# JuliaQuantumControl/GRAPE.jl

Hardware: AMD Instinct MI355X
Metric: GRAPE gradient evals/sec (N=64, 1000 steps, 128 traj) (higher is better)
Workload: dtype f64

## Files before the change

grape.jl_amd/api.py:

```python
from __future__ import annotations

import ctypes as C
import os
import subprocess
import sys

import numpy as np

_HERE = os.path.dirname(os.path.abspath(__file__))
_CSRC = os.path.join(_HERE, "csrc")
_LIBNAME = "libgrape_hip.so"

J_T_SM, J_T_SS, J_T_RE = 0, 1, 2
GRAD_GRADGEN, GRAD_TAYLOR = 0, 1
PROP_EXP, PROP_SERIES = 0, 1
ABI_VERSION = 7

STATUS = {0: "GRAPE_OK", -1: "GRAPE_ERR_INVALID", -2: "GRAPE_ERR_HIP", -3: "GRAPE_ERR_CHI_NORM",
          -4: "GRAPE_ERR_SINGULAR", -5: "GRAPE_ERR_TAYLOR", -6: "GRAPE_ERR_NO_CONTROLS", -7: "GRAPE_ERR_AGAIN",
          -8: "GRAPE_ERR_HOST"}

EXPORTS = ["grape_create", "grape_destroy", "grape_eval", "grape_forward", "grape_backward",
           "grape_forward_device", "grape_backward_device", "grape_check", "grape_get_propagator",
           "grape_get_tau_grads", "grape_get_storage", "grape_get_timings", "grape_reset_timings", "grape_get_work", "grape_get_cert_table", "grape_get_seg_table",
           "grape_last_error", "grape_abi_version", "grape_set_fused_sweeps", "grape_get_sums", "grape_backward_xi",
           "grape_get_final_states", "grape_backward_chi",
           "grape_get_time_gradient", "grape_set_tlist", "grape_eval_batch", "grape_get_batch_info", "grape_create_open",
           "grape_hvp", "grape_get_hvp_info", "grape_open_time_gradient", "grape_open_hvp", "grape_get_open_hvp_info",
           "grape_open_eval_batch", "grape_get_open_batch_info", "grape_open_set_running_cost", "grape_open_backward_xi",
           "grape_hvp_forward", "grape_hvp_backward", "grape_hvp_backward_chi",
           "grape_open_hvp_forward", "grape_open_hvp_backward", "grape_open_hvp_backward_chi",
           "grape_expect", "grape_get_expect_info"]


class GrapeHipError(RuntimeError):
    def __init__(self, code, msg):
        super().__init__(f"{STATUS.get(code, code)}: {msg}")
        self.code = code


class _Problem(C.Structure):
    _fields_ = [("abi_version", C.c_int32), ("N", C.c_int32), ("L", C.c_int32), ("K", C.c_int32),
                ("K_total", C.c_int32), ("N_T", C.c_int32), ("functional", C.c_int32),
                ("gradient_method", C.c_int32), ("hc_per_traj", C.c_int32), ("device", C.c_int32),
                ("tlist", C.c_void_p), ("H0", C.c_void_p), ("Hc", C.c_void_p), ("shape", C.c_void_p),
                ("psi0", C.c_void_p), ("target", C.c_void_p), ("weights", C.c_void_p),
                ("chi_min_norm", C.c_double), ("taylor_max_order", C.c_int32),
                ("taylor_tolerance", C.c_double),
                ("Dpen", C.c_void_p), ("dpen_per_traj", C.c_int32), ("lambda_b", C.c_double),
                ("prop_method", C.c_int32), ("prop_tolerance", C.c_double),
                ("ndev", C.c_int32), ("devices", C.c_void_p), ("taylor_no_check", C.c_int32)]


class _Lindblad(C.Structure):
    _fields_ = [("J", C.c_int32), ("cops_per_traj", C.c_int32), ("cops", C.c_void_p)]


def library_path() -> str:
    return os.path.join(_CSRC, _LIBNAME)


def build_asm(verbose: bool = False, workdir: str | None = None) -> str:
    asm_dir = os.path.join(_CSRC, "asm")
    work = workdir or asm_dir
    kernels = (("gen_t16.py", "expm_t16_asm"), ("gen_t16p.py", "expm_t16p_asm"), ("gen_t16p.py", "expm_t16p4_asm"), ("gen_t18g.py", "expm_t18g_asm"), ("gen_t18gp.py", "expm_t18gp_asm"), ("gen_d3.py", "deriv3_asm"), ("gen_d3s.py", "deriv3s_asm"), ("gen_d3s.py", "deriv3g_asm"),
               ("gen_lg.py", "lg_gemm_asm"), ("gen_d4.py", "deriv4_asm_128"), ("gen_d4.py", "deriv4_asm_256"))
    co_path, emb_s, emb_o = os.path.join(work, "grape_asm.co"), os.path.join(work, "asm_embed.S"), os.path.join(work, "asm_embed.o")
    llvm = "/opt/rocm/lib/llvm/bin"
    cmds, objs = [], []
    for gen_py, name in kernels:
        s_path, o_path = os.path.join(work, name + ".s"), os.path.join(work, name + ".o")
        gen = subprocess.run([sys.executable, os.path.join(asm_dir, gen_py), s_path], capture_output=True, text=True)
        if verbose or gen.returncode:
            print(gen.stdout, gen.stderr)
        if gen.returncode:
            raise RuntimeError(gen_py + " failed")
        cmds.append([os.path.join(llvm, "clang"), "-x", "assembler", "-target", "amdgcn-amd-amdhsa", "-mcpu=gfx950", "-c", s_path, "-o", o_path])
        objs.append(o_path)
    cmds.append([os.path.join(llvm, "ld.lld"), "-shared"] + objs + ["-o", co_path])
    with open(emb_s, "w") as f:
        f.write('\t.section .rodata\n\t.globl grape_asm_co_start\n\t.globl grape_asm_co_end\n\t.p2align 12\n'
                'grape_asm_co_start:\n\t.incbin "grape_asm.co"\ngrape_asm_co_end:\n\t.byte 0\n'
                '\t.section .note.GNU-stack,"",@progbits\n')
    cmds.append(["gcc", "-c", "-fPIC", "asm_embed.S", "-o", "asm_embed.o"])
    for c in cmds:
        res = subprocess.run(c, capture_output=True, text=True, cwd=work)
        if verbose or res.returncode:
            print(" ".join(c), res.stdout, res.stderr)
        if res.returncode:
            raise RuntimeError("assembling the gfx950 kernels failed")
    return emb_o


def _sources():
    srcs = [os.path.join(_CSRC, f) for f in ("grape_hip.hip", "grape_t18.hip", "grape_kernels.hip.h", "grape_large.hip.h",
                                             "grape_series.hip.h", "grape_cheby.hip.h", "grape_t18.hip.h", "grape_t18_coeffs.h",
                                             "grape_deriv3.hip.h", "grape_timegrad.hip.h", "grape_batch.hip.h", "grape_lindblad.hip.h", "grape_lindblad_tg.hip.h", "grape_hvp.hip.h", "grape_hvp_split.hip.h", "grape_lindblad_hvp.hip.h", "grape_lindblad_hvp_split.hip.h", "grape_lindblad_batch.hip.h", "grape_lindblad_rc.hip.h", "grape_devmem.h", "grape_cert.hip.h", "grape_expect.hip.h", "grape_econ_coeffs.h", os.path.join("asm", "gen_t16.py"), os.path.join("asm", "gen_t16p.py"), os.path.join("asm", "gen_t18g.py"), os.path.join("asm", "gen_t18gp.py"), os.path.join("asm", "gen_d3.py"), os.path.join("asm", "gen_d3s.py"), os.path.join("asm", "gen_lg.py"), os.path.join("asm", "gen_d4.py"), os.path.join("asm", "gcn.py"))]
    return srcs, os.path.join(_HERE, "..", "include", "grape_hip.h")


def _up_to_date(out: str) -> bool:
    srcs, hdr = _sources()
    return os.path.exists(out) and all(os.path.getmtime(out) >= os.path.getmtime(s) for s in srcs + [hdr])


def build_library(force: bool = False, verbose: bool = False, extra_flags=(), out: str | None = None) -> str:
    import fcntl
    import shutil
    import tempfile
    out = out or library_path()
    if not force and _up_to_date(out):
        return out
    srcs, _ = _sources()
    with open(os.path.join(_CSRC, ".build.lock"), "w") as lockf:
        fcntl.flock(lockf, fcntl.LOCK_EX)
        if not force and _up_to_date(out):
            return out
        work = tempfile.mkdtemp(prefix="_build_", dir=_CSRC)
        procs = []
        try:
            base = ["hipcc", "--offload-arch=gfx950", "-O3", "-std=c++17", "-fPIC", "-Wno-unused-value"] + list(extra_flags)
            objs = [os.path.join(work, "grape_hip.o"), os.path.join(work, "grape_t18.o")]
            cmds = [base + ["-cuid=grapehip0", "-c", srcs[0], "-o", objs[0]],
                    base + ["-cuid=grapehip1", "-mllvm", "-amdgpu-mfma-vgpr-form", "-c", srcs[1], "-o", objs[1]]]
            procs = [subprocess.Popen(c, stdout=subprocess.PIPE, stderr=subprocess.STDOUT, text=True) for c in cmds]
            objs.append(build_asm(verbose, workdir=work))
            outs = [p.communicate()[0] for p in procs]
            if verbose or any(p.returncode for p in procs):
                print("\n".join(outs))
            if any(p.returncode for p in procs):
                raise RuntimeError("hipcc failed building " + out)
            tmp_so = os.path.join(work, _LIBNAME)
            res = subprocess.run(["hipcc", "--offload-arch=gfx950", "-shared", "-fPIC"] + objs + ["-o", tmp_so], capture_output=True, text=True)
            if verbose or res.returncode:
                print(res.stdout, res.stderr)
            if res.returncode:
                raise RuntimeError("hipcc failed linking " + out)
            asm_dir = os.path.join(_CSRC, "asm")
            for f in os.listdir(work):
                if f.endswith(".s") or f.endswith(".co"):
                    os.replace(os.path.join(work, f), os.path.join(asm_dir, f))
            os.replace(tmp_so, out)
        finally:
            for p in procs:
                if p.poll() is None:
                    p.kill()
                    p.communicate()
            shutil.rmtree(work, ignore_errors=True)
    return out

# ... 311 lines not shown
        nv = 1 if d.ndim == 2 else d.shape[0]
        out = np.empty((nv, self.L * self.N_T))
        self._chk(self._lib.grape_hvp_backward_chi(self._h, nv, chi.ctypes.data, d.ctypes.data, out.ctypes.data))
        return out[0] if d.ndim == 2 else out

    def set_tlist(self, tlist):
        t = np.ascontiguousarray(tlist, dtype=np.float64)
        if t.shape != (self.N_T + 1,):
            raise ValueError(f"tlist must have N_T + 1 = {self.N_T + 1} points, got {t.shape}")
        self._chk(self._lib.grape_set_tlist(self._h, t.ctypes.data))
        self._tlist = t

    def forward_device(self, d_pulsevals_ptr, d_out_ptr, stream=0):
        self._chk(self._lib.grape_forward_device(self._h, d_pulsevals_ptr, d_out_ptr, stream))

    def backward_device(self, d_f_ptr, d_G_ptr, stream=0):
        self._chk(self._lib.grape_backward_device(self._h, d_f_ptr, d_G_ptr, stream))

    def set_fused_sweeps(self, on=True):
        return bool(self._lib.grape_set_fused_sweeps(self._h, int(bool(on))))

    def check(self, stream=0):
        self._chk(self._lib.grape_check(self._h, stream))

    def propagator(self, k, n):
        out = np.empty((self.N, self.N), dtype=np.complex128)
        self._chk(self._lib.grape_get_propagator(self._h, k, n, out.ctypes.data))
        return out.T.copy()

    def tau_grads(self):
        out = np.empty((self.K, self.L, self.N_T), dtype=np.complex128)
        self._chk(self._lib.grape_get_tau_grads(self._h, out.ctypes.data))
        return out

    def storage(self, which=0):
        out = np.empty((self.K, self.N_T + 1, self.N), dtype=np.complex128)
        self._chk(self._lib.grape_get_storage(self._h, which, out.ctypes.data))
        return out

    def timings(self):
        ms = np.full(8, -1.0)
        self._lib.grape_get_timings(self._h, ms.ctypes.data, 8)
        out = dict(zip(["expm", "forward", "backward", "deriv", "reduce", "total"], ms[:6].tolist()))
        if ms[6] >= 0.0:
            out["host_enqueue"] = float(ms[6])
        if ms[7] >= 0.0:
            out["gradient_allreduce_us"] = float(ms[7]) * 1e3
        return out

    def reset_timings(self):
        self._chk(self._lib.grape_reset_timings(self._h))

    def work(self):
        w = np.zeros(21)
        self._lib.grape_get_work(self._h, w.ctypes.data, 21)
        return dict(cells=w[0], squarings=w[1], flop_expm=w[2], flop_deriv=w[3], deriv_orders=w[4],
                    pivoted_cells=w[5], expm_cells=w[6], series_terms=w[7], series_steps=w[8],
                    t18_mfma_flop=w[9], t18_squarings=w[10], t18_cells=w[11], matrix_free_fallback=w[12], t16_cells=w[13],
                    asm_kernel=w[14], asm_deriv_kernel=w[15], asm_blocked_products=w[16],
                    walk_steps=w[17], scan_block=w[18], t16_certified=w[19], seg_certified=w[20])

    def cert_table(self):
        dims = np.zeros(3, np.int32)
        self._chk(self._lib.grape_get_cert_table(self._h, dims.ctypes.data, None, None))
        KC, n8, n6 = (int(x) for x in dims)
        coef, exps = np.zeros((KC, n8 + n6)), np.zeros(n8 + n6, np.int32)
        if n8 + n6:
            self._chk(self._lib.grape_get_cert_table(self._h, dims.ctypes.data, coef.ctypes.data, exps.ctypes.data))
        ex = np.stack([(exps >> (4 * l)) & 15 for l in range(self.L)], axis=1) if n8 + n6 else np.zeros((0, self.L), np.int32)
        return coef[:, :n8], coef[:, n8:], ex

    def seg_table(self):
        dims = np.zeros(4, np.int32)
        self._chk(self._lib.grape_get_seg_table(self._h, dims.ctypes.data, None, None))
        KC, n4, n8, n12 = (int(x) for x in dims)
        nt = n4 + n8 + n12
        coef, exps = np.zeros((KC, nt)), np.zeros(nt, np.int32)
        if nt:
            self._chk(self._lib.grape_get_seg_table(self._h, dims.ctypes.data, coef.ctypes.data, exps.ctypes.data))
        ex = np.stack([(exps >> (4 * l)) & 15 for l in range(self.L)], axis=1) if nt else np.zeros((0, self.L), np.int32)
        return coef[:, :n4], coef[:, n4:n4 + n8], coef[:, n4 + n8:], ex


def liouvillian(H, cops=()):
    H = np.asarray(H, dtype=np.complex128)
    d = H.shape[0]
    if H.shape != (d, d):
        raise ValueError(f"H must be [d, d], got {H.shape}")
    eye = np.eye(d)
    heff = H.copy()
    for A in cops:
        A = np.asarray(A, dtype=np.complex128)
        heff = heff - 0.5j * (A.conj().T @ A)
    out = np.kron(eye, heff) - np.kron(heff.conj(), eye)
    for A in cops:
        A = np.asarray(A, dtype=np.complex128)
        out = out + 1j * np.kron(A.conj(), A)
    return out


class GrapeHipOpen(GrapeHip):

    def __init__(self, H0, Hc, cops, tlist, rho0, target, weights=None, functional=J_T_SM, shape=None, K_total=None,
                 device=0, chi_min_norm=0.0, prop_tolerance=0.0):
        self._lib = load_library()
        H0 = np.asarray(H0)
        if H0.ndim != 3 or H0.shape[1] != H0.shape[2]:
            raise ValueError(f"H0 must be [K, d, d], got {H0.shape}")
        K, N = H0.shape[0], H0.shape[1]
        Hc = np.asarray(Hc)
        per_traj = Hc.ndim == 4
        if Hc.ndim not in (3, 4) or Hc.shape[-2:] != (N, N) or (per_traj and Hc.shape[0] != K):
            raise ValueError(f"Hc must be [L, d, d] or [K, L, d, d] with d = {N}, K = {K}, got {Hc.shape}")
# ... 194 lines not shown
```

grape.jl_amd/csrc/asm/gen_t16.py:

```python
import os
import re
import struct
import sys

sys.path.insert(0, os.path.dirname(os.path.abspath(__file__)))
from gcn import Prog, Reg, V, A, S, VCC, EXEC, Neg, Abs, kernel_text
from gcn import HZ_MFMA_TO_VALU as gcn_wait_valu, HZ_MFMA_TO_MEM as gcn_wait_mem

NT = 4
NP = 64
LDB = (3 * NP + 2) * 8
PLB = NP * 8
TROW = 16 * LDB
PLANES = NP * LDB
E1 = PLANES
EXH = 256 * 8 + 128
EXW = 2 * EXH
E2 = E1 + 4 * EXW
RED = E2 + 4 * EXW
XS0 = RED + 16 * 8
XS1 = XS0 + 1024
LDS_BYTES = XS1 + 1024
KERNARG = 136
SQ_MASK = 0xFF
CERT_BIT = 0x100

HERE = os.path.dirname(os.path.abspath(__file__))


def t16_coeffs():
    txt = open(os.path.join(HERE, "..", "grape_t18_coeffs.h")).read()
    c = {}
    for m in re.finditer(r"#define\s+T16_(C\d+|THETA)\s+([-+0-9.eE]+)", txt):
        c[m.group(1)] = float(m.group(2))
    assert len(c) == 17, c
    return c


def dbits(x):
    b = struct.unpack("<Q", struct.pack("<d", x))[0]
    return b & 0xFFFFFFFF, b >> 32


def pcol(j):
    return (j >> 1) + 8 * (j & 1)


def qrow(i):
    return 4 * (i & 3) + (i >> 2)


TILES = [(0, 0), (0, 1), (0, 2), (0, 3), (1, 1), (1, 2), (1, 3), (2, 2), (2, 3), (3, 3)]


class Pool:

# ... 391 lines not shown
            self.ssel(self.s_tmp[0], 16 * j0 * LDB + 16 * i0 * 8, 16 * j1 * LDB + 16 * i1 * 8)
            self.ssel(self.s_tmp[1], 16 * i0 * LDB + 16 * j0 * 8, 16 * i1 * LDB + 16 * j1 * 8)
            p.valu("v_add_u32", va, self.s_tmp[0], self.v_CP)
            p.valu("v_add_u32", vm, self.s_tmp[1], self.v_CM)
            cstep = (8 if self.PCOL_PERM else 1) * LDB
            for e in range(2):
                p.ds_write(64, va, ar.d(e), e * cstep)
                p.ds_write(64, va, ai.d(e), e * cstep + PLB)
                p.ds_write(64, va, sm.d(e), e * cstep + 2 * PLB)
            d0, d1 = i0 == j0, i1 == j1
            if not (d0 and d1):
                nar, ms = sr, si
                p.valu("v_mul_f64", nar.d(0), ar.d(0), -1.0)
                p.valu("v_mul_f64", nar.d(1), ar.d(1), -1.0)
                p.valu("v_add_f64", ms.d(0), ai.d(0), Neg(ar.d(0)))
                p.valu("v_add_f64", ms.d(1), ai.d(1), Neg(ar.d(1)))
                if d0 or d1:
                    p.salu("s_mov_b64", self.s_save, EXEC)
                    p.s_cmp("s_cmp_lt_u32", self.s_wave, 2)
                    lab = f"L_mirror_{u}_{len(p.ins)}"
                    p.s_branch("s_cbranch_scc1" if d0 else "s_cbranch_scc0", lab)
                for e in range(2):
                    p.ds_write(64, vm, nar.d(e), 32 * e)
                    p.ds_write(64, vm, ai.d(e), 32 * e + PLB)
                    p.ds_write(64, vm, ms.d(e), 32 * e + 2 * PLB)
                if d0 or d1:
                    p.label(lab)
            if fill:
                fill(u)
        for t in (ta, tb, tc):
            self.vp.free(t)

    def product(self, Q, B, half_last=False, init=None, hook=None, bload=None, fused=None):
        p = self.p
        NS = len(Q)
        started = set(init or ())

        def nslots(sk):
            return NS - 1 if (half_last and 2 * sk >= NT) else NS

        def rd(pl, so, sk, r):
            p.tag = "fragment"
            p.ds_read(64, self.aop[pl][so], self.v_AA[so][sk], self.KSTEP * r * LDB + pl * PLB)
            p.tag = ""

        def mma(so, pl, a, b):
            acc = Q[so][pl]
            c = acc if (so, pl) in started else 0
            started.add((so, pl))
            p.mfma(acc, a, b, c)

        sk0 = 0
        if fused:
            assert NS == 4 and not half_last and not bload

            def rdk(pl, so, r):
                p.tag = "fragment"
                p.ds_read(64, self.aop[pl][r], self.v_AA[so][0], self.KSTEP * r * LDB + pl * PLB)
                p.tag = ""

            fused["valu"](0)
            for st in fused["stores"](0):
                st()
            if fused.get("after_first"):
                fused["after_first"]()
            for r in range(4):
                for pl in range(3):
                    rdk(pl, 0, r)
            for so in range(4):
                gaps = [[] for _ in range(12)]
                if so < 3:
                    fused["valu"](so + 1)
                    pend = list(fused["stores"](so + 1))
                    for q, st in enumerate(pend):
                        gaps[4 * (q // 2) + (q % 2)].append(st)
                    last = {pl: (4 * pl + 1 if pend else 0) for pl in range(3)}
                    for r in range(4):
                        for pl in range(3):
                            gaps[max(last[pl], 3 * r + pl)].append(lambda pl=pl, r=r: rdk(pl, so + 1, r))
                j = 0
                for r in range(4):
                    for pl in range(3):
                        mma(so, pl, self.aop[pl][r], B[pl][0].d(r))
                        for f in gaps[j]:
                            f()
                        j += 1
            if fused.get("post"):
                fused["post"]()
            p.s_barrier()
            sk0 = 1
        for pl in range(3):
            for so in range(nslots(sk0)):
                rd(pl, so, sk0, 0)
            if bload:
                bload(pl, sk0, 0)
        for sk in range(sk0, 4):
            for r in range(4):
                ns = nslots(sk)
                more = not (sk == 3 and r == 3)
                nsk, nr = (sk, r + 1) if r < 3 else (sk + 1, 0)
                nsn = nslots(nsk) if more else 0
                for pl in range(3):
                    for so in range(ns):
                        mma(so, pl, self.aop[pl][so], B[pl][sk].d(r))
                        if hook and pl == 0 and so == 0:
                            hook(sk, r)
                    for so in range(nsn):
                        rd(pl, so, nsk, nr)
                    if bload and more:
                        bload(pl, nsk, nr)

    def plane_stores(self, sl, xr, xi, xs):
        if self.opts.get("nostore"):
            return []
        a = self.v_SA[sl]

        def st(h, pl, x):
            self.p.tag = "strip store"
            self.p.ds_write(128, a, x.sub(4 * h, 4), 16 * h + pl * PLB)
            self.p.tag = ""
        return [lambda h=h, pl=pl, x=x: st(h, pl, x) for pl, x in enumerate((xr, xi, xs)) for h in range(2)]

    def interleave(self, streams):
        streams = [list(s) for s in streams]
        if self.opts.get("serial"):
            for s in streams:
                for f in s:
                    f()
            return
        while any(streams):
            for s in streams:
                if s:
                    s.pop(0)()

    def acc_read(self, dst, src):
        if self.opts.get("noacc"):
            self.p.valu("v_mov_b32", dst.sub(0), dst.sub(0))
            self.p.valu("v_mov_b32", dst.sub(1), dst.sub(1))
            return
        self.p.valu("v_accvgpr_read_b32", dst.sub(0), src.sub(0))
        self.p.valu("v_accvgpr_read_b32", dst.sub(1), src.sub(1))

    def acc_write(self, dst, src):
        if self.opts.get("noacc"):
            self.p.valu("v_mov_b32", src.sub(0), src.sub(0))
            self.p.valu("v_mov_b32", src.sub(1), src.sub(1))
            return
        self.p.valu("v_accvgpr_write_b32", dst.sub(0), src.sub(0))
        self.p.valu("v_accvgpr_write_b32", dst.sub(1), src.sub(1))

    def wave_reduce(self, x, tmp, op):
        p = self.p
        for ctrl, rm in (("quad_perm:[1,0,3,2]", 0xF), ("quad_perm:[2,3,0,1]", 0xF), ("row_half_mirror", 0xF), ("row_mirror", 0xF),
                         ("row_bcast:15", 0xA), ("row_bcast:31", 0xC)):
            if rm != 0xF:
                p.valu("v_mov_b32", tmp.sub(0), 0)
                p.valu("v_mov_b32", tmp.sub(1), 0 if op == "v_add_f64" else 0xFFF00000)
            p.dpp_mov(tmp.sub(0), x.sub(0), ctrl, row_mask=rm)
            p.dpp_mov(tmp.sub(1), x.sub(1), ctrl, row_mask=rm)
            p.valu(op, x, x, tmp)

    def cell(self):
        p, c = self.p, self.s_c
        vp, ap = self.vp, self.ap
        Qt = [[V(8 * self.QT[3 * so + j], 8) for j in range(3)] for so in range(4)]
        for t in self.QT:
            vp.free_tiles.remove(t)
        Uprev = V(8 * self.UT, 64)
        for t in range(self.UT, self.UT + 8):
            vp.free_tiles.remove(t)

        self.stamp(0)
        self.As_re, self.As_im, self.As_sm = ap.alloc(4), ap.alloc(4), ap.alloc(4)
        As = (self.As_re, self.As_im, self.As_sm)

        def hook_store(sk, r):
            p.salu("s_mov_b64", self.s_save, EXEC)
            p.s_cmp("s_cmp_lg_u32", self.s_pm, 0)
            p.salu("s_cselect_b64", EXEC, -1, 0)
            p.global_store(4, self.v_UO[r], Uprev.sub(16 * sk + 4 * r, 4), self.s_ub[sk], nt=self.nt_u)
            p.salu("s_mov_b64", EXEC, self.s_save)

        def bload_A(pl, sk, r):
            if r % 2 == 0:
                p.tag = "strip load"
                p.ds_read(128, As[pl].sub(8 * sk + 2 * r, 4), self.v_SA[sk], 8 * r + pl * PLB)
                p.tag = ""

        B_As = [[S_.sub(8 * sl, 8) for sl in range(4)] for S_ in As]
        self.product(Qt[:3], B_As, half_last=True, hook=hook_store, bload=bload_A)
        ap.free(self.As_sm)
        vp.free(Uprev)
        self.stamp(1)
        As_re, As_im = self.As_re, self.As_im

        def A_(sl, r):
            return As_re.sub(8 * sl, 8).d(r), As_im.sub(8 * sl, 8).d(r)

        def in_place_y(sl_list):
            streams = []
            for sl in sl_list:
                for r in range(4):
                    p1, p2, p3 = (Qt[sl][j].d(r) for j in range(3))
                    streams.append([lambda p3=p3, p1=p1: p.valu("v_add_f64", p3, p3, Neg(p1)),
                                    lambda p1=p1, p2=p2: p.valu("v_add_f64", p1, p1, Neg(p2)),
                                    lambda p3=p3, p2=p2: p.valu("v_add_f64", p3, p3, Neg(p2))])
            for g in range(0, len(streams), 4):
                self.interleave(streams[g:g + 4])

        A2re, A2im, A2sm = [vp.alloc() for _ in range(4)], [vp.alloc() for _ in range(4)], [vp.alloc() for _ in range(4)]
        streams = []
        for sl in range(3):
            for r in range(4):
                p1, p2, p3 = (Qt[sl][j].d(r) for j in range(3))
                re_, im_ = A2re[sl].d(r), A2im[sl].d(r)
                streams.append([lambda re_=re_, p1=p1, p2=p2: p.valu("v_add_f64", re_, p1, Neg(p2)),
                                lambda im_=im_, p3=p3, p1=p1: p.valu("v_add_f64", im_, p3, Neg(p1)),
                                lambda im_=im_, p2=p2: p.valu("v_add_f64", im_, im_, Neg(p2))])
        for g in range(0, len(streams), 4):
            self.interleave(streams[g:g + 4])
        for r in range(4):
            p.ds_write(64, self.v_EW2, A2re[2].d(r), 128 * r)
            p.ds_write(64, self.v_EW2, A2im[2].d(r), EXH + 128 * r)
            p.ds_write(64, self.v_EW1, A2re[1].d(r), 128 * r)
            p.ds_write(64, self.v_EW1, A2im[1].d(r), EXH + 128 * r)
        p.s_waitcnt(lgkm=0)
        p.s_barrier()
        self.advance()
        self.cell_bases_issue(self.s_nkc, self.s_nn, self.s_ncell)
        txr, txi = vp.alloc(), vp.alloc()
        for h in range(2):
            p.ds_read(128, txr.sub(4 * h, 4), self.v_ER, 16 * h)
            p.ds_read(128, txi.sub(4 * h, 4), self.v_ER, EXH + 16 * h)
            p.ds_read(128, A2re[3].sub(4 * h, 4), self.v_ER, (E2 - E1) + 16 * h)
            p.ds_read(128, A2im[3].sub(4 * h, 4), self.v_ER, (E2 - E1) + EXH + 16 * h)
        self.stamp(2)
        tt = [vp.alloc(), vp.alloc()]

        def valu2(sl):
            if sl == 2:
                for r in range(4):
                    p.valu("v_add_f64", A2re[2].d(r), A2re[2].d(r), txr.d(r))
                    p.valu("v_add_f64", A2im[2].d(r), A2im[2].d(r), Neg(txi.d(r)))
                for r in range(4):
                    p.valu("v_mul_f64", A2im[3].d(r), A2im[3].d(r), -1.0)
                vp.free(txr)
                vp.free(txi)
            streams = []
            for r in range(4):
                xr, xi, xs = tt[0].d(r), tt[1].d(r), Qt[sl][1].d(r)
                a2r, a2i = A2re[sl].d(r), A2im[sl].d(r)
                ar_, ai_ = A_(sl, r)
                streams.append([lambda xr=xr, ar_=ar_: self.acc_read(xr, ar_),
                                lambda xi=xi, ai_=ai_: self.acc_read(xi, ai_),
                                lambda xr=xr: p.valu("v_mul_f64", xr, c[2], xr),
                                lambda xi=xi: p.valu("v_mul_f64", xi, c[2], xi),
                                lambda xr=xr, a2r=a2r: p.valu("v_fma_f64", xr, c[1], a2r, xr),
                                lambda xi=xi, a2i=a2i: p.valu("v_fma_f64", xi, c[1], a2i, xi),
                                lambda xs=xs, xr=xr, xi=xi: p.valu("v_add_f64", xs, xr, xi),
                                lambda r=r, a2r=a2r, a2i=a2i: p.valu("v_add_f64", A2sm[sl].d(r), a2r, a2i)])
            self.interleave(streams)

        self.product(Qt, [A2re, A2im, A2sm], fused={"valu": valu2, "stores": lambda sl: self.plane_stores(sl, tt[0], tt[1], Qt[sl][1])})
        for t in tt + A2sm:
            vp.free(t)
        self.cell_bases_finish(self.s_nkc)
        self.stamp(3)
        uid = len(p.ins)
        L_cert, L_cert2, L_ones, L_vdone = f"L_cert_{uid}", f"L_cert2_{uid}", f"L_ones_{uid}", f"L_vdone_{uid}"
        p.salu("s_and_b32", self.s_tmp[0], self.s_scur, CERT_BIT)
        p.s_branch("s_cbranch_scc1", L_cert)
        facc, gacc, cacc = vp.alloc(), vp.alloc(), vp.alloc()
        for acc in (facc, gacc, cacc):
            for j in range(8):
                p.valu("v_mov_b32", acc.sub(j), 0)
        streams = []
        for sl in range(4):
            for r in range(4):
                k = len(streams) % 4
                p1, p2, p3 = (Qt[sl][j].d(r) for j in range(3))
                a2r, a2i = A2re[sl].d(r), A2im[sl].d(r)
                f, g_, cs = facc.d(k), gacc.d(k), cacc.d(k)
                streams.append([
                    lambda p3=p3, p1=p1: p.valu("v_add_f64", p3, p3, Neg(p1)),
                    lambda p1=p1, p2=p2: p.valu("v_add_f64", p1, p1, Neg(p2)),
                    lambda p3=p3, p2=p2: p.valu("v_add_f64", p3, p3, Neg(p2)),
                    lambda cs=cs, a2r=a2r: p.valu("v_add_f64", cs, cs, Abs(a2r)),
                    lambda f=f, p1=p1: p.valu("v_fma_f64", f, p1, p1, f),
                    lambda g_=g_, a2r=a2r, p1=p1: p.valu("v_fma_f64", g_, a2r, p1, g_),
                    lambda cs=cs, a2i=a2i: p.valu("v_add_f64", cs, cs, Abs(a2i)),
                    lambda f=f, p3=p3: p.valu("v_fma_f64", f, p3, p3, f),
                    lambda g_=g_, a2i=a2i, p3=p3: p.valu("v_fma_f64", g_, a2i, p3, g_)])
        for g in range(0, 16, 4):
            self.interleave(streams[g:g + 4])
        f, g_, cs = facc.d(0), gacc.d(0), cacc.d(0)
        for k in range(1, 4):
            p.valu("v_add_f64", f, f, facc.d(k))
            p.valu("v_add_f64", g_, g_, gacc.d(k))
            p.valu("v_add_f64", cs, cs, cacc.d(k))
        ones, ct = cacc.d(1), vp.alloc(1)
        lo, hi = dbits(1.0)
        p.valu("v_mov_b32", ones.sub(0), lo)
        p.valu("v_mov_b32", ones.sub(1), hi)
        p.label(L_ones)
        p.mfma(ct, ones, cs, 0)
        p.salu("s_and_b32", self.s_tmp[0], self.s_scur, CERT_BIT)
        p.s_branch("s_cbranch_scc1", L_cert2)
        tmp = cacc.d(2)
        self.wave_reduce(f, tmp, "v_add_f64")
        self.wave_reduce(g_, tmp, "v_add_f64")
        mx = cacc.d(3)
        p.valu("v_mov_b64", mx, ct.d(0))
        for ctrl in ("quad_perm:[1,0,3,2]", "quad_perm:[2,3,0,1]", "row_half_mirror", "row_mirror"):
            p.dpp_mov(tmp.sub(0), mx.sub(0), ctrl)
            p.dpp_mov(tmp.sub(1), mx.sub(1), ctrl)
            p.valu("v_max_f64", mx, mx, tmp)
# ... 15 lines not shown
        vtf, vtg, vt2, vz = vp.alloc(), vp.alloc(), vp.alloc(), vp.alloc()
        p.valu("v_mov_b32", vz.sub(0), RED)
        for h in range(2):
            p.ds_read(128, vtf.sub(4 * h, 4), vz.sub(0), 16 * h)
            p.ds_read(128, vtg.sub(4 * h, 4), vz.sub(0), 32 + 16 * h)
            p.ds_read(128, vt2.sub(4 * h, 4), vz.sub(0), 64 + 16 * h)
        F, G, N2 = vtf.d(0), vtg.d(0), vt2.d(0)
        for k in range(1, 4):
            p.valu("v_add_f64", F, F, vtf.d(k))
            p.valu("v_add_f64", G, G, vtg.d(k))
            p.valu("v_max_f64", N2, N2, vt2.d(k))
        th = self.c["THETA"]
        c1, c2 = self.c["C1"], self.c["C2"]
        k0, k1, k2 = S(58, 2), S(60, 2), S(62, 2)
        self.smov64(k0, -1.0 / c1)
        p.valu("v_mul_f64", G, G, k0)
        self.smov64(k1, c2 * c2)
        p.valu("v_fma_f64", F, Neg(G), k1, F)
        self.smov64(k2, (1.0 + 1e-9) / (c1 * c1))
        p.valu("v_mul_f64", F, F, k2)
        self.smov64(k0, th ** 8)
        p.v_cmp("v_cmp_le_f64", S(58, 2), F, k0)
        p.v_cmp("v_cmp_ge_f64", S(60, 2), G, 0)
        p.salu("s_and_b64", S(58, 2), S(58, 2), S(60, 2))
        self.smov64(k2, th * th / (1.0 + 1e-9))
        p.v_cmp("v_cmp_le_f64", S(60, 2), N2, k2)
        p.salu("s_or_b64", S(58, 2), S(58, 2), S(60, 2))
        p.salu("s_and_b32", self.s_prop, self.s_prop, 1)
        p.s_cmp("s_cmp_eq_u64", S(58, 2), 0)
        p.salu("s_cselect_b32", self.s_tmp[4], 2, 0)
        p.salu("s_or_b32", self.s_prop, self.s_prop, self.s_tmp[4])
        p.valu("v_cndmask_b32", vz.sub(1), 1, 0, S(58, 2))
        p.salu("s_lshl_b32", self.s_tmp[2], self.s_cell, 2)
        p.valu("v_mov_b32", vz.sub(2), self.s_tmp[2])
        p.salu("s_mov_b64", self.s_save, EXEC)
        p.s_cmp("s_cmp_eq_u32", self.s_wave, 0)
        p.salu("s_cselect_b32", self.s_tmp[4], 1, 0)
        p.salu("s_mov_b32", self.s_tmp[5], 0)
        p.salu("s_mov_b64", EXEC, S(self.s_tmp[4].idx, 2))
        p.global_store(1, vz.sub(2), vz.sub(1), self.s_verdict)
        p.salu("s_mov_b64", EXEC, self.s_save)
        for t in (vtf, vtg, vt2, vz):
            vp.free(t)
        p.s_branch("s_branch", L_vdone)
        p.label(L_cert)
        p.nop(gcn_wait_valu)
        in_place_y(range(4))
        p.s_branch("s_branch", L_ones)
        p.label(L_cert2)
        p.nop(gcn_wait_mem)
        p.s_waitcnt(lgkm=0)
        p.s_barrier()
        p.salu("s_and_b32", self.s_prop, self.s_prop, 1)
        p.label(L_vdone)
        self.A2p_re, self.A2p_im = ap.alloc(4), ap.alloc(4)
        Bre, Bim, Bsm = [None] * 4, [None] * 4, [None] * 4
        tt = [vp.alloc(), vp.alloc()]

        def valu3(sl):
            Bre[sl], Bim[sl], Bsm[sl] = vp.alloc(), vp.alloc(), vp.alloc()
            streams = []
            for r in range(4):
                y0r, xs, y0i = (Qt[sl][j].d(r) for j in range(3))
                a2r, a2i = A2re[sl].d(r), A2im[sl].d(r)
                xr, xi = tt[0].d(r), tt[1].d(r)
                br, bi, bs = Bre[sl].d(r), Bim[sl].d(r), Bsm[sl].d(r)
                ar_, ai_ = A_(sl, r)
                pr, pi_ = self.A2p_re.sub(8 * sl, 8).d(r), self.A2p_im.sub(8 * sl, 8).d(r)
                streams.append([
                    lambda xr=xr, ar_=ar_: self.acc_read(xr, ar_),
                    lambda xi=xi, ai_=ai_: self.acc_read(xi, ai_),
                    lambda pr=pr, a2r=a2r: self.acc_write(pr, a2r),
                    lambda pi_=pi_, a2i=a2i: self.acc_write(pi_, a2i),
                    lambda br=br, a2r=a2r, y0r=y0r: p.valu("v_fma_f64", br, c[5], a2r, y0r),
                    lambda bi=bi, a2i=a2i, y0i=y0i: p.valu("v_fma_f64", bi, c[5], a2i, y0i),
                    lambda xr=xr: p.valu("v_mul_f64", xr, c[4], xr),
                    lambda xi=xi: p.valu("v_mul_f64", xi, c[4], xi),
                    lambda xr=xr, a2r=a2r: p.valu("v_fma_f64", xr, c[3], a2r, xr),
                    lambda xi=xi, a2i=a2i: p.valu("v_fma_f64", xi, c[3], a2i, xi),
                    lambda xr=xr, y0r=y0r: p.valu("v_add_f64", xr, xr, y0r),
                    lambda xi=xi, y0i=y0i: p.valu("v_add_f64", xi, xi, y0i),
                    lambda bs=bs, br=br, bi=bi: p.valu("v_add_f64", bs, br, bi),
                    lambda xs=xs, xr=xr, xi=xi: p.valu("v_add_f64", xs, xr, xi),
                    lambda y0r=y0r: p.valu("v_mul_f64", y0r, c[6], y0r),
                    lambda y0i=y0i: p.valu("v_mul_f64", y0i, c[6], y0i),
                    lambda y0r=y0r, a2r=a2r: p.valu("v_fma_f64", y0r, c[7], a2r, y0r),
                    lambda y0i=y0i, a2i=a2i: p.valu("v_fma_f64", y0i, c[7], a2i, y0i),
                    lambda y0i=y0i, y0r=y0r: p.valu("v_add_f64", y0i, y0i, y0r)])
            self.interleave(streams)
            vp.free(A2re[sl])
            vp.free(A2im[sl])

        init13 = {(so, j) for so in range(4) for j in (0, 2)}
        self.stamp(5)
        self.product(Qt, [Bre, Bim, Bsm], init=init13,
                     fused={"valu": valu3, "stores": lambda sl: self.plane_stores(sl, tt[0], tt[1], Qt[sl][1])})
        for t in tt:
            vp.free(t)
        self.stamp(6)
        in_place_y(range(4))
        p.s_barrier()
        self.stamp(7)
        self.stamp(8)
        k16 = S(58, 2)
        self.smov64(k16, self.c["C16"])
        tt = [vp.alloc() for _ in range(4)]

        def valu4(sl):
            streams = []
            for r in range(4):
                y1r, xi, y1i = (Qt[sl][j].d(r) for j in range(3))
                br, bi, xr = Bre[sl].d(r), Bim[sl].d(r), Bsm[sl].d(r)
                asr, asi, a2r, a2i = tt[0].d(r), tt[1].d(r), tt[2].d(r), tt[3].d(r)
                ar_, ai_ = A_(sl, r)
                pr, pi_ = self.A2p_re.sub(8 * sl, 8).d(r), self.A2p_im.sub(8 * sl, 8).d(r)
                st = [
                    lambda asr=asr, ar_=ar_: self.acc_read(asr, ar_),
                    lambda asi=asi, ai_=ai_: self.acc_read(asi, ai_),
                    lambda a2r=a2r, pr=pr: self.acc_read(a2r, pr),
                    lambda a2i=a2i, pi_=pi_: self.acc_read(a2i, pi_),
                    lambda br=br, a2r=a2r: p.valu("v_fma_f64", br, c[5], Neg(a2r), br),
                    lambda bi=bi, a2i=a2i: p.valu("v_fma_f64", bi, c[5], Neg(a2i), bi),
                    lambda xr=xr, a2r=a2r, y1r=y1r: p.valu("v_fma_f64", xr, c[8], a2r, y1r),
                    lambda xi=xi, a2i=a2i, y1i=y1i: p.valu("v_fma_f64", xi, c[8], a2i, y1i),
                    lambda xr=xr, asr=asr: p.valu("v_fma_f64", xr, c[9], asr, xr),
                    lambda xi=xi, asi=asi: p.valu("v_fma_f64", xi, c[9], asi, xi),
                    lambda a2r=a2r: p.valu("v_mul_f64", a2r, c[14], a2r),
                    lambda a2i=a2i: p.valu("v_mul_f64", a2i, c[14], a2i),
                    lambda a2r=a2r, asr=asr: p.valu("v_fma_f64", a2r, c[15], asr, a2r),
                    lambda a2i=a2i, asi=asi: p.valu("v_fma_f64", a2i, c[15], asi, a2i),
                    lambda a2r=a2r, br=br: p.valu("v_fma_f64", a2r, c[13], br, a2r),
                    lambda a2i=a2i, bi=bi: p.valu("v_fma_f64", a2i, c[13], bi, a2i),
                    lambda a2r=a2r, y1r=y1r: p.valu("v_fma_f64", a2r, c[12], y1r, a2r),
                    lambda a2i=a2i, y1i=y1i: p.valu("v_fma_f64", a2i, c[12], y1i, a2i),
                    lambda br=br, y1r=y1r: p.valu("v_fma_f64", br, c[10], br, y1r),
                    lambda bi=bi, y1i=y1i: p.valu("v_fma_f64", bi, c[10], bi, y1i),
                    lambda br=br, asr=asr: p.valu("v_fma_f64", br, c[11], asr, br),
                    lambda bi=bi, asi=asi: p.valu("v_fma_f64", bi, c[11], asi, bi),
                    lambda asr=asr, xr=xr, xi=xi: p.valu("v_add_f64", asr, xr, xi),
                ]
                if sl == 0:
                    def diag(a2r=a2r, r=r):
                        p.salu("s_mov_b64", self.s_save, EXEC)
                        p.salu("s_mov_b64", EXEC, self.s_dmask[r])
                        p.valu("v_add_f64", a2r, a2r, k16)
                        p.salu("s_mov_b64", EXEC, self.s_save)
                    st.append(diag)
                st += [
                    lambda y1r=y1r, a2r=a2r: p.valu("v_mov_b64", y1r, a2r),
                    lambda y1i=y1i, a2r=a2r, a2i=a2i: p.valu("v_add_f64", y1i, a2r, a2i),
                ]
                streams.append(st)
            self.interleave(streams)

        def bsm(sl_list):
            for sl in sl_list:
                for r in range(4):
                    p.valu("v_add_f64", Bsm[sl].d(r), Bre[sl].d(r), Bim[sl].d(r))
# ... 376 lines not shown
```

grape.jl_amd/csrc/grape_hip.hip:

```cpp
#include "../../include/grape_hip.h"
#include "grape_kernels.hip.h"
#include "grape_t18_coeffs.h"
#include "grape_econ_coeffs.h"
#include "grape_large.hip.h"
#include "grape_series.hip.h"
#include "grape_cheby.hip.h"
#include "grape_timegrad.hip.h"
#include "grape_lindblad.hip.h"
#include "grape_lindblad_tg.hip.h"
#include "grape_hvp.hip.h"
#include "grape_hvp_split.hip.h"
#include "grape_lindblad_hvp.hip.h"
#include "grape_lindblad_hvp_split.hip.h"
#include "grape_lindblad_batch.hip.h"
#include "grape_lindblad_rc.hip.h"
#include "grape_devmem.h"
#include "grape_cert.hip.h"
#include "grape_expect.hip.h"

#include <rccl/rccl.h>
#include <dlfcn.h>
#include <mutex>

#include <algorithm>
// ... 42 lines not shown
struct OpenCtx;

struct grape_handle {
    grape_problem p{};
    int N = 0, NP = 0, NT = 0, L = 0, K = 0, K_total = 0, N_T = 0;
    int device = 0;
    hipStream_t stream = nullptr;
    double *d_H0f = nullptr, *d_Hcf = nullptr, *d_H0t = nullptr, *d_Hct = nullptr;
    double *d_H0p = nullptr, *d_Hcp = nullptr, *d_vecs = nullptr;
    double *d_H0q = nullptr, *d_Hcq = nullptr, *d_park2 = nullptr;
    double *d_H0q3 = nullptr, *d_Hcq3 = nullptr, *d_H0p3 = nullptr, *d_Hcp3 = nullptr;
    int deriv4_blocks = 0;
    double *d_park3 = nullptr;
    int deriv3_blocks = 0, deriv3_wpt = 0;
    bool deriv3_h0g = false;
    bool deriv3_general = false;
    int deriv2 = 0, deriv2_maxm = 0;
    bool deriv_stream = false;
    bool deriv_stream_never = false;
    int deriv_blocks = 0;
    bool large = false;
    int chunk = 0;
    double *d_lg[9] = {nullptr, nullptr, nullptr, nullptr, nullptr, nullptr, nullptr, nullptr, nullptr};
    double *d_dinv = nullptr;
    int *d_scell = nullptr;
    double *d_colpart = nullptr;
    bool lg_form2 = false;
    double *d_normpart = nullptr;
    double *d_dts = nullptr, *d_shape = nullptr, *d_weights = nullptr;
    double2 *d_psi0 = nullptr, *d_target = nullptr;
    double *d_eps = nullptr;
    double2 *d_U = nullptr, *d_fw = nullptr, *d_bw = nullptr, *d_tg = nullptr;
    double *d_ret = nullptr;
    double *d_out = nullptr;
    double *d_f = nullptr, *d_G = nullptr, *d_rho = nullptr;
    int *d_flags = nullptr;
    int *d_cellflag = nullptr;
    int KC = 0;
    bool herm = false;
    bool herm_ctrl = false;
    bool t18 = false;
    bool t18_small = true;
    bool t16 = true;
    double *d_gram = nullptr;
    int *d_celllist = nullptr;
    double *d_cert = nullptr;
    int *d_cert_exp = nullptr;
    int cert_n8 = 0, cert_n6 = 0;
    double *d_seg = nullptr;
    double *d_seg8 = nullptr;
    int *d_seg_exp = nullptr;
    int seg_n8 = 0, seg_n4 = 0, seg_n12 = 0, seg8_stride = 0, seg_exp_off = 0;
    int *d_segplan = nullptr;
    bool asm16 = false;
    bool asm16p = false;
    double *d_dte = nullptr;
    bool asm18gp = false;
    bool asm18g = false;
    int *d_wgtab = nullptr, *d_prog = nullptr, *d_splan = nullptr;
    double2 *d_xinit = nullptr;
    int asm_blocks = 0;
    int last_walk_fuse = 0;
    bool asm_sq = true;
    int asm_walk = 0;
    bool foreign_stream = false;
    bool credit_pending = false;
    std::vector<double> bal;
    std::vector<double> bal_stage_chi, bal_stage_xi;
    double *d_Sf = nullptr;
    bool expm_persist = true;
    int expm_lds_pad_kb = 0;
    bool test_hooks = false;
    bool lg_asm = true;
    bool deriv3_asm = true;
    bool taylor_check = true;
    bool no_target = false;
    std::vector<int> cls;
    int *d_cls = nullptr, *d_rep = nullptr;
    int coop_S = 0;
    int *d_xcc_sw = nullptr;
    int coop_rpw = 0, coop_nw = 0;
    double2 *d_Dt = nullptr, *d_xi = nullptr;
    double *d_wq = nullptr, *d_gb = nullptr;
    bool have_gb = false;
    const double2 *xi_user = nullptr;
    double lambda_user = 0.0;
    unsigned long long *d_stats = nullptr;
    double *h_pin = nullptr;
    double *h_get = nullptr;
    DeviceBufs mem;
    size_t h_pin_doubles = 0;
    Phase ph[kRing][kPhases]{};
    long n_fwd = 0, n_bwd = 0;
    std::string err;
    bool have_forward = false, in_eval = false;
    double chi_min_norm = 1e-100, taylor_tol = 1e-16;
    int taylor_max_order = 100;
    bool fuse = false;
    bool fuse_on = true;
    bool want_bw = true;
    bool bw_done = false;
    bool bw_unit = false;
    bool z_valid = false;
    double *d_inv_tnorm = nullptr, *d_ones = nullptr;
    double2 *d_z = nullptr;
    bool scan16 = false;
// ... 136 lines not shown
}
hipError_t stream_fill(void *p, int byte_value, size_t bytes, hipStream_t s) {
    hipStreamCaptureStatus st = hipStreamCaptureStatusNone;
    if (bytes % 4 != 0 || ((size_t)p & 3) != 0 || hipStreamIsCapturing(s, &st) != hipSuccess || st != hipStreamCaptureStatusActive)
        return hipMemsetAsync(p, byte_value, bytes, s);
    const size_t n = bytes / 4;
    if (n == 0) return hipSuccess;
    const unsigned v = 0x01010101u * (unsigned)(byte_value & 0xFF);
    hipLaunchKernelGGL(fill_words_kernel, dim3((unsigned)std::min<size_t>((n + 255) / 256, 1024)), dim3(256), 0, s, (unsigned *)p, v, n);
    return hipGetLastError();
}

size_t expm_lds_bytes(int NT) {
    const int total = NT == 1 ? ExpmLds<1>::TOTAL : NT == 2 ? ExpmLds<2>::TOTAL : NT == 3 ? ExpmLds<3>::TOTAL : ExpmLds<4>::TOTAL;
    return sizeof(double) * (size_t)total;
}

template <int NT>
hipError_t launch_expm(const ExpmArgs &a, bool herm, hipStream_t s, int persistent_blocks = 0, int lds_pad_kb = 0) {
    static LdsLimit lim_fast, lim_piv, lim_herm, lim_pers, lim_persh;
    const size_t lds = expm_lds_bytes(NT) + (size_t)lds_pad_kb * 1024;
    int dev = 0;
    hipGetDevice(&dev);
    {
        hipError_t e = lim_fast.ensure((const void *)expm_pade_kernel<NT, false>, dev, lds);
        if (e == hipSuccess) e = lim_piv.ensure((const void *)expm_pade_kernel<NT, true>, dev, lds);
        if (e == hipSuccess && NT >= 3) e = lim_herm.ensure((const void *)expm_pade_kernel<NT, false, NT >= 3>, dev, lds);
        if (e != hipSuccess) return e;
    }
    hipError_t e = stream_fill(a.cellflag, 0, (size_t)a.K * a.N_T * sizeof(int), s);
    if (e != hipSuccess) return e;
    if (NT == 4 && persistent_blocks > 0) {
        hipError_t ep = lim_pers.ensure((const void *)expm_persistent_kernel<NT, false>, dev, lds);
        if (ep == hipSuccess) ep = lim_persh.ensure((const void *)expm_persistent_kernel<NT, NT == 4>, dev, lds);
        if (ep != hipSuccess) return ep;
        if (herm) hipLaunchKernelGGL((expm_persistent_kernel<NT, NT == 4>), dim3(persistent_blocks), dim3(NT * 64), lds, s, a);
        else hipLaunchKernelGGL((expm_persistent_kernel<NT, false>), dim3(persistent_blocks), dim3(NT * 64), lds, s, a);
    } else
    if (herm && NT >= 3)
        hipLaunchKernelGGL((expm_pade_kernel<NT, false, NT >= 3>), dim3(a.K * a.N_T), dim3(NT * 64), lds, s, a);
    else
        hipLaunchKernelGGL((expm_pade_kernel<NT, false>), dim3(a.K * a.N_T), dim3(NT * 64), lds, s, a);
    hipLaunchKernelGGL((expm_pade_kernel<NT, true>), dim3(std::min(a.K * a.N_T, 1024)), dim3(NT * 64), lds, s, a);
    return hipGetLastError();
}

extern "C" int grape_t18_launch(int NT, int herm, int t16, const void *args, size_t args_size, void *stream, int blocks);
extern "C" const double *grape_econ_pairs(void);
extern "C" int grape_t16p_asm_launch(const void *args, size_t args_size, int *verdict, void *stream, int blocks,
                                     const void *const *walk, int fuse, int K, const double *dte);
extern "C" int grape_t18g_asm_launch(const void *args, size_t args_size, int *verdict, void *stream, int blocks,
                                     const void *const *walk, int fuse, int K, const double *dte);
extern "C" int grape_t16_asm_launch(const void *args, size_t args_size, int *verdict, void *stream, int blocks,
                                    const void *const *walk, int fuse, int K);
extern "C" int grape_t18_batch_launch(int herm, const void *args, size_t args_size, const void *strides, size_t strides_size,
                                      int sets, void *stream, int blocks);
extern "C" void grape_t16_walks(int KC, int N_T, int nblk, int *tab);
extern "C" int grape_t16_credit_launch(const void *args, size_t args_size, void *stream);
static bool deriv3_fits(int NT, int L, bool h0_general = false) {
    const size_t tile = (size_t)2 * 16 * 17 * sizeof(double), mat = (size_t)(NT * (NT + 1) / 2) * tile;
    if (h0_general) return NT >= 3 && NT <= 4 && L >= 1 && L <= 2 && (size_t)NT * NT * tile + (size_t)L * mat <= 160 * 1024;
    return L >= 1 && L <= 8 && (size_t)(1 + L) * mat <= 160 * 1024;
}
extern "C" int grape_deriv3_launch(int NT, const void *d2args, size_t d2size, const double *H0f, const double *Hcf, int wpt,
                                   int skip_if_flagged, int h0_general, int use_asm, void *stream, int blocks);
extern "C" int grape_lg_asm_launch(const void *k, size_t size, unsigned blocks, void *stream);
extern "C" int grape_deriv4_launch(int NP, const void *d2args, size_t d2size, const double *H0q3, const double *Hcq3, const double *H0p3,
                                   const double *Hcp3, void *stream, int blocks);
#ifdef GRAPE_DIAG
extern "C" void grape_t18_set_stamps(unsigned long long *d_stamps, void *stream);
#endif

template <int CPL>
hipError_t launch_coop(const SweepArgs &a, bool backward, int S, int rpw, int nw, hipStream_t s) {
    hipError_t e;
    if (a.xcc) {
        e = hipMemsetAsync(a.xcc, 0xFF, (size_t)a.K * 32 * sizeof(int), s);
        if (e != hipSuccess) return e;
    }
    e = hipMemsetAsync((void *)a.store, 0xFF, (size_t)a.K * (a.N_T + 1) * 64 * CPL * sizeof(double2), s);
    if (e != hipSuccess) return e;
    const dim3 grid(8 * ((a.K + 7) / 8) * S), block(64 * nw);
#define COOP_CASE(NW_, RPW_)                                                                                          \
    if (nw == NW_ && rpw == RPW_) {                                                                                   \
        if (backward) hipLaunchKernelGGL((sweep_coop_kernel<CPL, RPW_, NW_, true>), grid, block, 0, s, a, S);         \
        else hipLaunchKernelGGL((sweep_coop_kernel<CPL, RPW_, NW_, false>), grid, block, 0, s, a, S);                 \
        return hipGetLastError();                                                                                     \
    }
    COOP_CASE(4, 1) COOP_CASE(8, 1) COOP_CASE(16, 1) COOP_CASE(16, 2) COOP_CASE(16, 4)
#undef COOP_CASE
    return hipErrorInvalidValue;
}

static bool g_sweep_wg32 = false;
template <int NP>
hipError_t launch_sweep(const SweepArgs &a, bool backward, hipStream_t s);
template <int NP>
hipError_t launch_sweep_pair(const SweepArgs &af, const SweepArgs &ab, hipStream_t s);

template <int NT>
hipError_t launch_scan_block(const ScanArgs &sa, hipStream_t s) {
    static LdsLimit lim;
    constexpr int NP = 16 * NT;
    const size_t lds = (size_t)2 * 2 * NP * (NP + 2) * sizeof(double);
    int dev = 0;
    hipGetDevice(&dev);
    hipError_t e = lim.ensure((const void *)scan_block_kernel<NT>, dev, lds);
// ... 2372 lines not shown
                const double t = std::ceil((double)h->KC * NBq / slots) * Bk * t1 + (NBq + Bk) * t2;
                if (t < best_t) { best_t = t; best = Bk; }
            }
            if (const char *envb = getenv("GRAPE_SCAN16_BK")) best = std::max(2, atoi(envb));
            h->scan_Bk = std::min(best, N_T);
            h->scan_NB = (N_T + h->scan_Bk - 1) / h->scan_Bk;
            CCHK(h->mem.alloc(&h->d_scanF, (size_t)h->KC * h->scan_NB * NP * NP));
            CCHK(h->mem.alloc(&h->d_scan_fw, (size_t)K * (h->scan_NB + 1) * NP));
            CCHK(h->mem.alloc(&h->d_scan_bw, (size_t)K * (h->scan_NB + 1) * NP));
            h->scan16 = true;
        }
    }
    CCHK(h->mem.alloc(&h->d_tg, (size_t)K * L * N_T));
    CCHK(h->mem.alloc(&h->d_ret, (size_t)2 * K + 8 + (size_t)L * N_T + 4 + (size_t)GRAPE_STAT_SHARDS * GRAPE_STAT_SLOTS));
    h->d_out = h->d_ret;
    h->d_G = h->d_ret + (size_t)2 * K + 8;
    h->d_flags = (int *)(h->d_G + (size_t)L * N_T);
    h->d_stats = (unsigned long long *)(h->d_G + (size_t)L * N_T + 4);
    CCHK(h->mem.alloc(&h->d_f, 2)); CCHK(h->mem.alloc(&h->d_rho, (size_t)K));
    CCHK(h->mem.alloc(&h->d_cellflag, (size_t)K * N_T));
    bool sf_per_cell_ok = false;
    const char *envp16 = getenv("GRAPE_EXPM_ASM16P");
    const bool p_direct = p->hc_per_traj && (h->herm ? L <= 4 : L <= 2) && !(envp16 && atoi(envp16) == 0);
    if (p->hc_per_traj && !p_direct && h->t18 && !h->large && !h->series && h->NT == 4) {
        size_t free_b = 0, total_b = 0;
        CCHK(hipMemGetInfo(&free_b, &total_b));
        const char *envs = getenv("GRAPE_SF_PER_CELL");
        sf_per_cell_ok = !(envs && atoi(envs) == 0) && 2.0 * (double)h->KC * N_T * NP * NP * 16.0 + 8e9 < (double)free_b;
    }
    const bool sf_shape_ok = !p->hc_per_traj || p_direct || sf_per_cell_ok;
    h->asm16 = h->asm16 && h->t16 && h->t18 && h->herm && !h->large && !h->series && h->NT == 4 && sf_shape_ok && (long)K * N_T < (1L << 28);
    h->asm18g = h->asm18g && h->t18 && !h->herm && !h->large && !h->series && h->NT == 4 && sf_shape_ok && (long)K * N_T < (1L << 28);
    h->asm16p = h->asm16 && p_direct;
    h->asm18gp = h->asm18g && p_direct;
    {
        const char *enve = getenv("GRAPE_DERIV_ECON");
        const bool lg_ok = h->large && h->t18 && h->herm && !h->series;
        const bool t16c_ok = h->t16 && h->t18 && h->herm && !h->large && !h->series && (h->NT >= 3 || (h->NT == 2 && h->t18_small));
        h->deriv_econ = (h->asm16 || lg_ok || t16c_ok) && p->gradient_method == GRAPE_GRAD_GRADGEN && h->taylor_tol >= 1e-16 && h->d_batchflag &&
                        !(enve && atoi(enve) == 0);
        if (h->deriv_econ) h->d_econ_pairs = grape_econ_pairs();
        if (h->deriv_econ && !h->d_econ_pairs) h->deriv_econ = false;
        if (h->deriv_econ && lg_ok) {
            CCHK(h->mem.alloc(&h->d_celldeg, (size_t)h->KC * N_T));
            CCHK(hipMemset(h->d_celldeg, 0, (size_t)h->KC * N_T * sizeof(int)));
        }
    }
    if (h->asm16p || h->asm18gp) CCHK(h->mem.alloc(&h->d_dte, (size_t)(L <= 2 ? 4 : 8) * N_T));
    if (h->t18 && !h->large && !h->series && ((L > 2 && !p->hc_per_traj) || (h->asm16 && !h->asm16p) || (h->asm18g && !h->asm18gp)) && (h->NT >= 3 || h->t18_small))
        CCHK(h->mem.alloc(&h->d_Sf, (size_t)(p->hc_per_traj ? (size_t)h->KC * N_T : (size_t)N_T) * 2 * NP * NP));
    if (h->asm16 || h->asm18g) {
        const long ncell = (long)h->KC * N_T;
        h->asm_blocks = (int)std::max<long>(1, std::min<long>(h->num_cus, ncell));
        std::vector<int> tab((size_t)4 * h->asm_blocks);
        grape_t16_walks(h->KC, N_T, h->asm_blocks, tab.data());
        CCHK(h->mem.alloc(&h->d_wgtab, tab.size()));
        CCHK(h->mem.alloc(&h->d_splan, (size_t)ncell));
        CCHK(hipMemset(h->d_splan, 0, (size_t)ncell * sizeof(int)));
        CCHK(hipMemcpy(h->d_wgtab, tab.data(), tab.size() * sizeof(int), hipMemcpyHostToDevice));
        const char *envw = getenv("GRAPE_EXPM_WALK"), *envq = getenv("GRAPE_EXPM_SQ");
        h->asm_sq = !(envq && atoi(envq) == 0);
        h->asm_walk = h->KC == K ? (envw ? atoi(envw) & 3 : 3) : 0;
        if (h->scan16) h->asm_walk = 0;
        if (h->asm_walk) {
            std::vector<double> xi((size_t)2 * K * 64 * 2, 0.0);
            for (int k = 0; k < K; ++k) {
                double n2 = 0.0;
                for (int i = 0; i < 2 * N; ++i) n2 += p->target[(size_t)k * 2 * N + i] * p->target[(size_t)k * 2 * N + i];
                const double itn = n2 > 0.0 ? 1.0 / std::sqrt(n2) : 0.0;
                for (int i = 0; i < N; ++i) {
                    xi[2 * ((size_t)k * 64 + i)] = p->psi0[2 * ((size_t)k * N + i)];
                    xi[2 * ((size_t)k * 64 + i) + 1] = p->psi0[2 * ((size_t)k * N + i) + 1];
                    xi[2 * ((size_t)(K + k) * 64 + i)] = p->target[2 * ((size_t)k * N + i)] * itn;
                    xi[2 * ((size_t)(K + k) * 64 + i) + 1] = -p->target[2 * ((size_t)k * N + i) + 1] * itn;
                }
            }
            CCHK(h->mem.alloc(&h->d_xinit, (size_t)2 * K * 64));
            CCHK(hipMemcpy(h->d_xinit, xi.data(), xi.size() * 8, hipMemcpyHostToDevice));
            CCHK(h->mem.alloc(&h->d_prog, (size_t)2 * K));
            CCHK(hipMemset(h->d_prog, 0, (size_t)2 * K * sizeof(int)));
        }
    }
    if (h->t16 && h->t18 && h->herm && !h->large && !h->series && (h->NT >= 3 || (h->NT == 2 && h->t18_small))) {
        CCHK(h->mem.alloc(&h->d_celllist, (size_t)K * N_T));
        const int M = L + 1, KCn = h->KC;
        const int GS = M * M + M;
        std::vector<double> gram((size_t)KCn * GS);
        std::vector<int> repk(KCn, -1);
        auto shape_factor = [&](const double *op, double fro2) {
            if (!(fro2 > 0.0)) return 1.0;
            std::vector<double> a2((size_t)2 * N * N), a4((size_t)2 * N * N);
            auto square = [&](const double *a, std::vector<double> &c) {
                std::fill(c.begin(), c.end(), 0.0);
                for (int j = 0; j < N; ++j)
                    for (int k = 0; k < N; ++k) {
                        const double br = a[2 * ((size_t)j * N + k)], bi = a[2 * ((size_t)j * N + k) + 1];
                        const double *ak = a + 2 * (size_t)k * N;
                        double *cj = &c[2 * (size_t)j * N];
                        for (int i = 0; i < N; ++i) {
                            cj[2 * i] += ak[2 * i] * br - ak[2 * i + 1] * bi;
                            cj[2 * i + 1] += ak[2 * i] * bi + ak[2 * i + 1] * br;
                        }
                    }
            };
            square(op, a2);
            square(a2.data(), a4);
            double m8 = 0.0;
            for (double x : a4) m8 += x * x;
            const double s8 = std::pow(m8, 0.125), semi = std::pow(3.5, 0.125) * 2.0 * std::sqrt(fro2 / (double)N);
            const double kap = s8 / semi;
            return std::isfinite(kap) && kap > 0.0 ? kap : 1.0;
        };
        std::vector<double> kap_shared((size_t)L, -1.0);
        for (int k = K - 1; k >= 0; --k) repk[h->cls.empty() ? k : h->cls[k]] = k;
        const size_t nn2 = (size_t)2 * N * N;
        for (int kc = 0; kc < KCn; ++kc) {
            const int k = repk[kc] < 0 ? kc : repk[kc];
            auto op = [&](int a) { return a == 0 ? p->H0 + (size_t)k * nn2 : p->Hc + ((size_t)(p->hc_per_traj ? k : 0) * L + (a - 1)) * nn2; };
            for (int a = 0; a < M; ++a)
                for (int b = a; b < M; ++b) {
                    const double *x = op(a), *y = op(b);
                    double sum = 0.;
                    for (size_t i = 0; i < nn2; ++i) sum += x[i] * y[i];
                    gram[(size_t)kc * GS + (size_t)a * M + b] = gram[(size_t)kc * GS + (size_t)b * M + a] = sum;
                }
        }
        if (!p->hc_per_traj)
            for (int l = 0; l < L; ++l) kap_shared[l] = shape_factor(p->Hc + (size_t)l * nn2, gram[(size_t)(1 + l) * M + (1 + l)]);
        parallel_for(KCn, [&](int kc) {
            const int k = repk[kc] < 0 ? kc : repk[kc];
            for (int a = 0; a < M; ++a) {
                const double fro2 = gram[(size_t)kc * GS + (size_t)a * M + a];
                const double *o = a == 0 ? p->H0 + (size_t)k * nn2 : p->Hc + ((size_t)(p->hc_per_traj ? k : 0) * L + (a - 1)) * nn2;
                gram[(size_t)kc * GS + (size_t)M * M + a] = (a > 0 && !p->hc_per_traj) ? kap_shared[a - 1] : shape_factor(o, fro2);
            }
        });
        CCHK(h->mem.alloc(&h->d_gram, gram.size()));
        CCHK(hipMemcpy(h->d_gram, gram.data(), gram.size() * 8, hipMemcpyHostToDevice));
        const char *envc = getenv("GRAPE_EXPM_CERT"), *envg = getenv("GRAPE_DERIV_SEG");
        static_assert(T16_PLAN_LMAX == GRAPE_CERT_LMAX, "power table of t16_plan_kernel");
        const bool want_cert = h->asm16 && L >= 1 && L <= GRAPE_CERT_LMAX && !(envc && atoi(envc) == 0);
        const bool want_seg = h->asm16 && h->deriv_econ && L >= 1 && L <= 2 && !(envg && atoi(envg) == 0);
        if (want_cert || want_seg) {
            const CertPlan pl(L, want_seg);
            const int nt = pl.n8 + pl.n6, ns = pl.n4 + pl.n12;
            if (want_cert) {
                h->cert_n8 = pl.n8; h->cert_n6 = pl.n6;
                CCHK(h->mem.alloc(&h->d_cert, (size_t)KCn * nt));
                CCHK(h->mem.alloc(&h->d_cert_exp, (size_t)nt));
                CCHK(hipMemcpy(h->d_cert_exp, pl.exps.data(), (size_t)nt * sizeof(int), hipMemcpyHostToDevice));
            }
            if (want_seg) {
                h->seg_n8 = pl.n8; h->seg_n4 = pl.n4; h->seg_n12 = pl.n12; h->seg_exp_off = nt;
                CCHK(h->mem.alloc(&h->d_seg, (size_t)KCn * ns));
                CCHK(h->mem.alloc(&h->d_seg_exp, pl.exps.size()));
                CCHK(hipMemcpy(h->d_seg_exp, pl.exps.data(), pl.exps.size() * sizeof(int), hipMemcpyHostToDevice));
                if (want_cert) { h->d_seg8 = h->d_cert; h->seg8_stride = nt; }
                else { CCHK(h->mem.alloc(&h->d_seg8, (size_t)KCn * pl.n8)); h->seg8_stride = pl.n8; }
                CCHK(h->mem.alloc(&h->d_segplan, (size_t)KCn * N_T));
                CCHK(hipMemset(h->d_segplan, 0, (size_t)KCn * N_T * sizeof(int)));
            }
            DeviceBufs tmp;
            int *d_job[8] = {nullptr, nullptr, nullptr, nullptr, nullptr, nullptr, nullptr, nullptr};
            const std::vector<int> *job[8] = {&pl.mm2.row, &pl.mm2.pair, &pl.mm34.row, &pl.mm34.pair, &pl.tr.row, &pl.tr.pair, &pl.mm6.row, &pl.mm6.pair};
            for (int i = 0; i < 8; ++i) {
                CCHK(tmp.alloc(&d_job[i], std::max<size_t>(1, job[i]->size())));
                CCHK(hipMemcpy(d_job[i], job[i]->data(), job[i]->size() * sizeof(int), hipMemcpyHostToDevice));
            }
            const size_t per_class = (size_t)pl.nmat * N * N;
            const int chunk = (int)std::max<size_t>(1, std::min<size_t>((size_t)KCn, ((size_t)64 << 20) / (per_class * sizeof(double2))));
            double2 *d_scr = nullptr;
            CCHK(tmp.alloc(&d_scr, per_class * chunk));
            for (int kc0 = 0; kc0 < KCn; kc0 += chunk) {
                const unsigned nc = (unsigned)std::min(chunk, KCn - kc0);
                hipLaunchKernelGGL(cert_load_kernel, dim3((unsigned)pl.M, nc), dim3(256), 0, 0, (const double *)h->d_H0f, (const double *)h->d_Hcf,
                                   (const int *)h->d_rep, kc0, p->hc_per_traj ? 1 : 0, L, N, NP, pl.nmat, d_scr);
                hipLaunchKernelGGL(cert_mm_kernel, dim3((unsigned)pl.n2, nc), dim3(256), 0, 0, d_scr, pl.nmat, N, pl.M, (const int *)d_job[0], (const int *)d_job[1]);
                hipLaunchKernelGGL(cert_mm_kernel, dim3((unsigned)(pl.n3 + pl.n4), nc), dim3(256), 0, 0, d_scr, pl.nmat, N, pl.M + pl.n2, (const int *)d_job[2],
                                   (const int *)d_job[3]);
                if (want_cert)
                    hipLaunchKernelGGL(cert_trace_kernel, dim3((unsigned)nt, nc), dim3(256), 0, 0, (const double2 *)d_scr, pl.nmat, N, (const int *)d_job[4],
                                       (const int *)d_job[5], nt, h->d_cert + (size_t)kc0 * nt);
                else
                    hipLaunchKernelGGL(cert_trace_kernel, dim3((unsigned)pl.n8, nc), dim3(256), 0, 0, (const double2 *)d_scr, pl.nmat, N, (const int *)d_job[4],
                                       (const int *)d_job[5], pl.n8, h->d_seg8 + (size_t)kc0 * pl.n8);
                if (want_seg) {
                    hipLaunchKernelGGL(cert_mm_kernel, dim3((unsigned)pl.n6, nc), dim3(256), 0, 0, d_scr, pl.nmat, N, pl.M + pl.n2 + pl.n3 + pl.n4,
                                       (const int *)d_job[6], (const int *)d_job[7]);
                    hipLaunchKernelGGL(cert_trace_kernel, dim3((unsigned)ns, nc), dim3(256), 0, 0, (const double2 *)d_scr, pl.nmat, N,
                                       (const int *)d_job[4] + nt, (const int *)d_job[5], ns, h->d_seg + (size_t)kc0 * ns);
                }
                CCHK(hipGetLastError());
            }
            CCHK(hipDeviceSynchronize());
        }
    }
    if (h->large && h->series) {
        const int per_xcd = std::max(1, h->num_cus / 8), S = h->NP / 16;
        if (per_xcd < S) {
            h->err = "prop_method = GRAPE_PROP_SERIES with N > 64 needs NP / 16 co-resident workgroups per XCD";
            return fail(GRAPE_ERR_INVALID);
        }
        h->cheby_S = S;
        h->cheby_pair = h->fuse && per_xcd >= 2 * S;
        if (!h->cheby_pair) h->fuse = false;
        h->cheby_round = 8 * std::max(1, per_xcd / ((h->cheby_pair ? 2 : 1) * S));
        CCHK(h->mem.alloc(&h->d_xch, (size_t)2 * K * 4 * NP));
        CCHK(h->mem.alloc(&h->d_xcc, (size_t)2 * K * 32));
    }
    if (h->large && !h->series) {
        hipDeviceProp_t prop;
        CCHK(hipGetDeviceProperties(&prop, h->device));
        const int per_xcd = std::max(1, prop.multiProcessorCount / 8), groups = (K + 7) / 8;
        int S = 1;
        while (S * 2 * groups <= per_xcd && h->NP / (S * 2) >= 4) S *= 2;
        const int R = h->NP / S;
        const char *env = getenv("GRAPE_SWEEP_COOP");
        if (S >= 2 && R <= 64 && !(env && atoi(env) == 0)) {
            h->coop_S = S;
            h->coop_nw = R >= 16 ? 16 : R;
            h->coop_rpw = R / h->coop_nw;
            CCHK(h->mem.alloc(&h->d_xcc_sw, (size_t)2 * K * 32));
        }
    }
    CCHK(hipMemset(h->d_flags, 0, 8 * sizeof(int)));
    CCHK(hipMemset(h->d_stats, 0, (size_t)GRAPE_STAT_SHARDS * GRAPE_STAT_SLOTS * sizeof(unsigned long long)));
    CCHK(hipMemset(h->d_fw, 0, (size_t)K * (N_T + 1) * NP * 16));
    CCHK(hipMemset(h->d_bw, 0, (size_t)K * (N_T + 1) * NP * 16));
    CCHK(hipMemset(h->d_tg, 0, (size_t)K * L * N_T * 16));
    h->h_pin_doubles = (size_t)2 * L * N_T + 2 * K + 16;
    if (p->Dpen && p->lambda_b != 0.0) {
        h->have_gb = true;
        const int Kd = p->dpen_per_traj ? K : 1;
        std::vector<double> dt_((size_t)Kd * pp * 2, 0.0);
        for (int kd = 0; kd < Kd; ++kd)
            for (int j = 0; j < N; ++j)
                for (int i = 0; i < N; ++i) {
                    dt_[2 * ((size_t)kd * pp + (size_t)j * NP + i)] = p->Dpen[2 * ((size_t)kd * nn + (size_t)j * N + i)];
                    dt_[2 * ((size_t)kd * pp + (size_t)j * NP + i) + 1] = p->Dpen[2 * ((size_t)kd * nn + (size_t)j * N + i) + 1];
                }
        CCHK(h->mem.alloc(&h->d_Dt, (size_t)Kd * pp));
        CCHK(hipMemcpy(h->d_Dt, dt_.data(), dt_.size() * 8, hipMemcpyHostToDevice));
        std::vector<double> wq(N_T + 1);
// ... 24 lines not shown
int grape_forward_device(grape_handle *h, const double *d_pulsevals, double *d_out, void *stream_) try {
    if (h && h->open) return open_refuse(h, "grape_forward_device");
    if (!h || !d_pulsevals || !d_out) return GRAPE_ERR_INVALID;
    if (!h->shards.empty()) { h->err = "device-pointer entry points need a single-device handle (ndev <= 1)"; return GRAPE_ERR_INVALID; }
    hipStream_t s = (hipStream_t)stream_;
    h->foreign_stream = s != h->stream;
    HIPCHK(h, hipSetDevice(h->device));
    (void)hipGetLastError();
    HIPCHK(h, stream_fill(h->d_flags, 0, 8 * sizeof(int) + (size_t)GRAPE_STAT_SHARDS * GRAPE_STAT_SLOTS * sizeof(unsigned long long), s));
    if (d_pulsevals != h->d_eps)
        HIPCHK(h, hipMemcpyAsync(h->d_eps, d_pulsevals, (size_t)h->L * h->N_T * 8, hipMemcpyDeviceToDevice, s));
    ExpmArgs ea{};
    ea.H0f = h->d_H0f; ea.Hcf = h->d_Hcf; ea.eps = h->d_eps; ea.shape = h->d_shape; ea.dts = h->d_dts;
    ea.U = h->d_U; ea.flags = h->d_flags; ea.stats = h->d_stats; ea.cellflag = h->d_cellflag;
    ea.K = h->KC; ea.rep = h->d_rep; ea.L = h->L; ea.N_T = h->N_T; ea.hc_per_traj = h->p.hc_per_traj;
    ea.n1 = h->d_n1; ea.n1_k = h->K;
#ifdef GRAPE_DIAG
    ea.ablate = getenv("GRAPE_DIAG_ABLATE") ? atoi(getenv("GRAPE_DIAG_ABLATE")) : 0;
    static unsigned long long *d_stamps = nullptr;
    if (getenv("GRAPE_DIAG_STAMPS")) {
        if (!d_stamps) hipMalloc((void **)&d_stamps, (size_t)h->K * h->N_T * 32 * 8);
        hipMemsetAsync(d_stamps, 0, (size_t)h->K * h->N_T * 32 * 8, s);
    }
    ea.stamps = d_stamps;
    hipMemcpyToSymbolAsync(HIP_SYMBOL(g_diag_slot_base), &d_stamps, sizeof(d_stamps), 0, hipMemcpyHostToDevice, s);
    grape_t18_set_stamps(d_stamps, (void *)s);
#endif
    hipError_t e = hipSuccess;
    int walk_fuse = 0;
    if (!h->series) {
        phase_begin(h, 0, s);
        if (h->large) {
            e = h->t18 ? expm_large_t18(h, s) : expm_large(h, s);
        } else {
            const long ncell = (long)ea.K * ea.N_T;
            const int per_cu = h->NT == 1 ? 10 : h->NT == 2 ? 4 : 1;
            const int t18_blocks = 8 * (int)std::max<long>(1, std::min<long>((long)(h->num_cus / 8) * per_cu, (ncell + 7) / 8));
            if (h->t18 && (h->NT >= 3 || h->t18_small)) {
                if (h->d_Sf) {
                    CtrlSumArgs ca{};
                    ca.Hcf = h->d_Hcf; ca.eps = h->d_eps; ca.shape = h->d_shape; ca.Sf = h->d_Sf;
                    ca.L = h->L; ca.N_T = h->N_T; ca.pp2 = 2 * h->NP * h->NP;
                    ca.per_traj = h->p.hc_per_traj ? 1 : 0; ca.rep = h->d_rep;
                    hipLaunchKernelGGL(ctrl_sum_kernel, dim3((unsigned)((ca.per_traj ? h->KC : 1) * h->N_T), std::max(1, ca.pp2 / 2 / 2048)), dim3(256), 0, s, ca);
                    HIPCHK(h, hipGetLastError());
                    ea.Sf = h->d_Sf;
                }
                const bool t16 = h->d_celllist != nullptr;
                ea.cell_list = h->d_celllist; ea.listed = 0;
                if (t16) {
                    T16PlanArgs pa{};
                    pa.gram = h->d_gram; pa.eps = h->d_eps; pa.shape = h->d_shape; pa.dts = h->d_dts; pa.flags = h->d_flags;
                    pa.KC = h->KC; pa.L = h->L; pa.N_T = h->N_T; pa.N = h->N;
                    pa.splan = (h->asm16 && (h->asm_sq || h->d_cert)) ? h->d_splan : nullptr;
                    pa.sq_on = h->asm_sq ? 1 : 0;
                    pa.cert = h->d_cert; pa.cert_exp = h->d_cert_exp; pa.n8 = h->cert_n8; pa.n6 = h->cert_n6;
                    pa.verdict = h->d_cellflag;
                    pa.seg = h->d_seg; pa.seg8 = h->d_seg8; pa.seg8_stride = h->seg8_stride; pa.seg8_exp = h->d_seg_exp;
                    pa.seg_exp = h->d_seg_exp ? h->d_seg_exp + h->seg_exp_off : nullptr;
                    pa.s8 = h->seg_n8; pa.n4 = h->seg_n4; pa.n12 = h->seg_n12; pa.segplan = h->d_segplan;
                    const unsigned plan_blocks = (unsigned)(h->KC * ((h->N_T + T16_PLAN_TPB - 1) / T16_PLAN_TPB));
                    const size_t plan_lds = t16_plan_lds(pa);
                    switch (plan_lds ? h->L : 0) {
                        case 1: hipLaunchKernelGGL(t16_plan_kernel<1>, dim3(plan_blocks), dim3(T16_PLAN_TPB), plan_lds, s, pa); break;
                        case 2: hipLaunchKernelGGL(t16_plan_kernel<2>, dim3(plan_blocks), dim3(T16_PLAN_TPB), plan_lds, s, pa); break;
                        case 3: hipLaunchKernelGGL(t16_plan_kernel<3>, dim3(plan_blocks), dim3(T16_PLAN_TPB), plan_lds, s, pa); break;
                        case 4: hipLaunchKernelGGL(t16_plan_kernel<4>, dim3(plan_blocks), dim3(T16_PLAN_TPB), plan_lds, s, pa); break;
                        default: hipLaunchKernelGGL(t16_plan_kernel<0>, dim3(plan_blocks), dim3(T16_PLAN_TPB), 0, s, pa); break;
                    }
                    HIPCHK(h, hipGetLastError());
                }
                const int blocks16 = (t16 && h->NT == 3) ? 8 * (int)std::max<long>(1, std::min<long>((long)(h->num_cus / 8) * 2, (ncell + 7) / 8)) : t18_blocks;
                h->credit_pending = false;
                if (h->asm18g) {
                    walk_fuse = h->asm_walk & (1 | ((h->fuse && h->fuse_on && h->want_bw) ? 2 : 0));
                    if (walk_fuse) HIPCHK(h, stream_fill(h->d_prog, 0, (size_t)2 * h->K * sizeof(int), s));
                    const void *walk[6] = {h->d_wgtab, h->d_xinit, h->d_fw, h->d_bw, h->d_prog, h->d_splan};
                    if (h->asm18gp) {
                        hipLaunchKernelGGL(dte_kernel, dim3((unsigned)((h->N_T + 255) / 256)), dim3(256), 0, s, (const double *)h->d_eps,
                                           (const double *)h->d_shape, (const double *)h->d_dts, h->L, h->N_T, 2, h->d_dte);
                        HIPCHK(h, hipGetLastError());
                    }
                    e = (hipError_t)grape_t18g_asm_launch(&ea, sizeof(ea), h->d_cellflag, (void *)s, h->asm_blocks, walk, walk_fuse, h->K,
                                                          h->asm18gp ? h->d_dte : nullptr);
                    h->credit_pending = !h->asm18gp;
                }
                else if (t16 && h->asm16p) {
                    walk_fuse = h->asm_walk & (1 | ((h->fuse && h->fuse_on && h->want_bw) ? 2 : 0));
                    if (walk_fuse) HIPCHK(h, stream_fill(h->d_prog, 0, (size_t)2 * h->K * sizeof(int), s));
                    hipLaunchKernelGGL(dte_kernel, dim3((unsigned)((h->N_T + 255) / 256)), dim3(256), 0, s, (const double *)h->d_eps,
                                       (const double *)h->d_shape, (const double *)h->d_dts, h->L, h->N_T, h->L <= 2 ? 2 : 4, h->d_dte);
                    HIPCHK(h, hipGetLastError());
                    const void *walk[6] = {h->d_wgtab, h->d_xinit, h->d_fw, h->d_bw, h->d_prog, h->d_splan};
                    e = (hipError_t)grape_t16p_asm_launch(&ea, sizeof(ea), h->d_cellflag, (void *)s, h->asm_blocks, walk, walk_fuse, h->K, h->d_dte);
                }
                else if (t16 && h->asm16) {
                    walk_fuse = h->asm_walk & (1 | ((h->fuse && h->fuse_on && h->want_bw) ? 2 : 0));
                    if (walk_fuse) HIPCHK(h, stream_fill(h->d_prog, 0, (size_t)2 * h->K * sizeof(int), s));
                    const void *walk[6] = {h->d_wgtab, h->d_xinit, h->d_fw, h->d_bw, h->d_prog, h->d_splan};
                    e = (hipError_t)grape_t16_asm_launch(&ea, sizeof(ea), h->d_cellflag, (void *)s, h->asm_blocks, walk, walk_fuse, h->K);
                    h->credit_pending = true;
                }
                else
                    e = (hipError_t)grape_t18_launch(h->NT, h->herm ? 1 : 0, t16 ? 1 : 0, &ea, sizeof(ea), (void *)s, blocks16);
                if (t16 && e == hipSuccess) {
                    ea.listed = 1;
                    e = (hipError_t)grape_t18_launch(h->NT, 1, 0, &ea, sizeof(ea), (void *)s, t18_blocks);
                }
            } else
            switch (h->NT) {
                case 1: e = launch_expm<1>(ea, h->herm, s, 0, h->expm_lds_pad_kb); break;
                case 2: e = launch_expm<2>(ea, h->herm, s, 0, h->expm_lds_pad_kb); break;
                case 3: e = launch_expm<3>(ea, h->herm, s, 0, h->expm_lds_pad_kb); break;
                default: {
                    const int nb = 8 * (h->num_cus / 8);
                    const bool persist = h->expm_persist && nb >= 8 && (long)ea.K * ea.N_T >= 4L * nb;
                    e = launch_expm<4>(ea, h->herm, s, persist ? nb : 0, h->expm_lds_pad_kb);
                    break;
                }
            }
        }
        HIPCHK(h, e);
        if (h->deriv_econ) {
            DerivEconArgs ec{};
            ec.verdict = h->d_cellflag; ec.splan = h->d_splan; ec.cls = h->d_cls; ec.flags = h->d_flags;
            ec.cell_deg = h->large ? h->d_celldeg : nullptr;
            ec.deg0 = ECON_DEG[ECON_VERDICT_SET]; ec.deg1 = ECON_DEG[ECON_NSETS - 1];
            ec.segplan = h->large ? nullptr : h->d_segplan; ec.deg_seg = ECON_DEG[0];
            static_assert(ECON_NSETS == 5, "segments 1.11 (three-moment certificate), 1.36 (verdict), 1.6, 2.0 (blocked path), 2.72 (one planned squaring)");
            ec.K = h->K; ec.KC = h->KC; ec.N_T = h->N_T; ec.batches_per_k = (h->N_T + 15) / 16;
            ec.nbatch_total = h->K * ec.batches_per_k; ec.batch_econ = h->d_batchflag + ec.nbatch_total;
            hipLaunchKernelGGL(deriv_econ_kernel, dim3((unsigned)((ec.nbatch_total + 255) / 256)), dim3(256), 0, s, ec);
            HIPCHK(h, hipGetLastError());
        }
        phase_end(h, 0, s);
    }
#ifdef GRAPE_DIAG
    if (ea.stamps) {
        hipStreamSynchronize(s);
        const size_t nb = (size_t)h->KC * h->N_T;
        std::vector<unsigned long long> st(nb * 32);
        hipMemcpy(st.data(), ea.stamps, nb * 32 * 8, hipMemcpyDeviceToHost);
        auto avg = [&](int i1, int i0) {
            double sum = 0;
            size_t cnt = 0;
            for (size_t b = 0; b < nb; ++b)
                if (st[b * 32 + i1] && st[b * 32 + i0]) { sum += (double)(st[b * 32 + i1] - st[b * 32 + i0]); ++cnt; }
            return cnt ? sum / cnt : 0.0;
        };
        if (h->t18 && h->NT >= 3) {
            const char *tn[] = {"form A (+norm)", "A2 = A A + half exchange", "A3 = A A2", "store A3, norm A2, barrier", "A6 = A3 A3",
                                "A6 exchanges + norms", "scaling, B1 -> X, barrier", "A9 = B1 B5", "+B4, B3+A9 -> X, B2", "p = B2 + (B3+A9) A9",
                                "squarings", "store U", "end barrier"};
            for (int j = 0; j < 13; ++j) fprintf(stderr, "  stamp %-28s %9.0f cycles\n", tn[j], avg(j + 1, j));
            fprintf(stderr, "  stamp %-28s %9.0f cycles\n", "TOTAL per cell", avg(13, 0));
        } else {
        const char *pn[] = {"form A", "norm", "A2", "A4,A6 (+store A2)", "store A6 + combos", "dual", "U=A*T"};
// ... 961 lines not shown
            double cm[kPhases];
            cnt = grape_get_timings(h->shards[g], cm, n < kPhases ? n : kPhases);
            if (cnt < 0) return multi_fail(h, h->shards[g], cnt);
            for (int i = 0; i < cnt; ++i) ms[i] = g == 0 ? cm[i] : std::max(ms[i], cm[i]);
        }
        if (n > kPhases) { ms[kPhases] = h->host_enqueue_calls ? 2.0 * h->host_enqueue_ms / h->host_enqueue_calls : -1.0; cnt = kPhases + 1; }
        if (n > kPhases + 1) { ms[kPhases + 1] = (h->use_rccl && h->allreduce_calls) ? h->allreduce_ms / h->allreduce_calls : -1.0; cnt = kPhases + 2; }
        return cnt;
    }
    HIPCHK(h, hipSetDevice(h->device));
    HIPCHK(h, hipDeviceSynchronize());
    int cnt = 0;
    for (int i = 0; i < kPhases && i < n; ++i, ++cnt) {
        double sum = 0.0;
        int used = 0;
        for (int r = 0; r < kRing; ++r) {
            float t = 0.f;
            Phase &p = h->ph[r][i];
            if (p.used && hipEventElapsedTime(&t, p.e0, p.e1) == hipSuccess) { sum += t; ++used; }
        }
        ms[i] = used ? sum / used : -1.0;
    }
    return cnt;
}
GRAPE_BARRIER(h ? &h->err : &g_create_error)

int grape_reset_timings(grape_handle *h) try {
    if (!h) return GRAPE_ERR_INVALID;
    if (h->open) { h->open->ms_fwd = h->open->ms_bwd = 0.0; h->open->n_fwd = h->open->n_bwd = 0; return GRAPE_OK; }
    if (!h->shards.empty()) {
        for (grape_handle *c : h->shards) {
            const int rc = grape_reset_timings(c);
            if (rc) return multi_fail(h, c, rc);
        }
        h->host_enqueue_ms = 0.0;
        h->allreduce_ms = 0.0; h->allreduce_calls = 0;
        h->host_enqueue_calls = 0;
        return GRAPE_OK;
    }
    HIPCHK(h, hipSetDevice(h->device));
    HIPCHK(h, hipDeviceSynchronize());
    for (auto &ring : h->ph)
        for (auto &p : ring) p.used = false;
    h->n_fwd = h->n_bwd = 0;
    h->n_eval = 0;
    return GRAPE_OK;
}
GRAPE_BARRIER(h ? &h->err : &g_create_error)

int grape_get_work(grape_handle *h, double *out, int n) try {
    if (!h || !out || n < 4) return GRAPE_ERR_INVALID;
    if (h->open) return open_work(h, out, n);
    if (!h->shards.empty()) {
        const int m = n < 21 ? n : 21;
        std::fill(out, out + m, 0.0);
        for (grape_handle *c : h->shards) {
            double cw[21] = {0.};
            const int rc = grape_get_work(c, cw, m);
            if (rc < 0) return multi_fail(h, c, rc);
            for (int i = 0; i < m; ++i) out[i] = (i == 15 || i == 16 || i == 18) ? cw[i] : out[i] + cw[i];
        }
        if (m > 14 && out[14] > 0.0) out[14] = h->shards[0]->asm16p ? 3.0 : h->shards[0]->asm18gp ? 4.0 : h->shards[0]->asm18g ? 2.0 : 1.0;
        return 4;
    }
    HIPCHK(h, hipSetDevice(h->device));
    if (h->foreign_stream) HIPCHK(h, hipDeviceSynchronize());
    if (h->credit_pending) {
        ExpmArgs ea{};
        ea.H0f = h->d_H0f; ea.Hcf = h->d_Hcf; ea.eps = h->d_eps; ea.shape = h->d_shape; ea.dts = h->d_dts;
        ea.flags = h->d_flags; ea.stats = h->d_stats; ea.Sf = h->d_Sf;
        ea.K = h->KC; ea.rep = h->d_rep; ea.L = h->L; ea.N_T = h->N_T; ea.hc_per_traj = h->p.hc_per_traj;
        ea.n1 = h->d_n1; ea.n1_k = h->K;
        HIPCHK(h, (hipError_t)grape_t16_credit_launch(&ea, sizeof(ea), (void *)h->stream));
        HIPCHK(h, hipStreamSynchronize(h->stream));
        h->credit_pending = false;
    }
    unsigned long long sh[GRAPE_STAT_SHARDS * GRAPE_STAT_SLOTS], st[GRAPE_STAT_SLOTS] = {0};
    { const int rc_ = getter_fetch(h, sh, h->d_stats, sizeof(sh)); if (rc_) return rc_; }
    for (int q = 0; q < GRAPE_STAT_SHARDS; ++q)
        for (int i = 0; i < GRAPE_STAT_SLOTS; ++i) st[i] += sh[q * GRAPE_STAT_SLOTS + i];
    const double N3 = (double)h->N * h->N * h->N, N2 = (double)h->N * h->N;
    const double cells = (double)h->K * h->N_T, ecells = (double)h->KC * h->N_T;
    const double gemms = 2.0 * st[3] + 3.0 * st[4] + 4.0 * st[5] + 5.0 * st[6] + 6.0 * st[7];
    out[0] = cells;
    out[1] = (double)st[0];
    out[2] = (gemms + (double)st[0]) * 8.0 * N3 + ecells * (32.0 / 3.0) * N3;
    out[3] = (double)st[8] * (1.0 + 2.0 * h->L) * 8.0 * N2;
    if (n > 4) out[4] = (double)st[8];
    if (n > 5) out[5] = (double)st[9];
    if (n > 6) out[6] = h->series ? 0.0 : ecells;
    if (n > 7) out[7] = (double)st[10];
    if (n > 8) out[8] = (double)st[11];
    if (n > 9) out[9] = (double)st[12] * 2048.0;
    if (n > 10) out[10] = (double)st[13];
    if (n > 11) out[11] = (double)st[14];
    if (n > 12) out[12] = h->u_fallback ? 1.0 : 0.0;
    if (n > 13) out[13] = (double)st[15];
    if (n > 14) out[14] = h->asm16p ? 3.0 : h->asm16 ? 1.0 : h->asm18gp ? 4.0 : h->asm18g ? 2.0 : 0.0;
    if (n > 15) {
        double kind = 0.0;
        if (!h->series && h->d_park3 && h->NT == 4) {
            if (h->deriv3_general) kind = 3.0;
            else if (h->L > 2) kind = 2.0;
            else if (!h->deriv3_h0g && h->deriv3_asm) kind = 1.0;
        } else if (!h->series && h->deriv4_blocks) kind = 4.0;
        out[15] = kind;
    }
    if (n > 16) out[16] = (h->large && !h->series && h->t18 && h->lg_asm) ? 1.0 : 0.0;
    if (n > 17) {
        double carried = 0.0;
        if (h->last_walk_fuse && h->d_prog) {
            std::vector<int> prog((size_t)2 * h->K);
            { const int rc_ = getter_fetch(h, prog.data(), h->d_prog, prog.size() * sizeof(int)); if (rc_) return rc_; }
            for (int k = 0; k < h->K; ++k) {
                if (h->last_walk_fuse & 1) carried += prog[(size_t)k];
                if (h->last_walk_fuse & 2) carried += prog[(size_t)h->K + k];
            }
        }
        out[17] = carried;
    }
    if (n > 18) out[18] = h->scan16 ? (double)h->scan_Bk : 0.0;
    if (n > 19) {
        double certified = 0.0, seg = 0.0;
        const bool want_seg = n > 20 && h->d_segplan && h->deriv_econ;
        if ((h->d_cert || want_seg) && h->d_splan && !h->series) {
            const size_t ncell = (size_t)h->KC * h->N_T;
            std::vector<int> plan(ncell);
            int fl[8];
            { const int rc_ = getter_fetch(h, plan.data(), h->d_splan, ncell * sizeof(int)); if (rc_) return rc_; }
            { const int rc_ = getter_fetch(h, fl, h->d_flags, sizeof(fl)); if (rc_) return rc_; }
            const bool tried = !(4L * fl[6] > (long)ncell);
            if (tried && h->d_cert)
                for (int w : plan) certified += (w & T16_PLAN_CERT) ? 1.0 : 0.0;
            if (tried && want_seg) {
                std::vector<int> sp(ncell), verdict(ncell);
                { const int rc_ = getter_fetch(h, sp.data(), h->d_segplan, ncell * sizeof(int)); if (rc_) return rc_; }
                { const int rc_ = getter_fetch(h, verdict.data(), h->d_cellflag, ncell * sizeof(int)); if (rc_) return rc_; }
                for (int k = 0; k < h->K; ++k) {
                    const size_t c0 = (size_t)(h->cls.empty() ? k : h->cls[k]) * h->N_T;
                    for (int i = 0; i < h->N_T; ++i)
                        seg += (sp[c0 + i] && verdict[c0 + i] == 0 && (plan[c0 + i] & T16_PLAN_SQ_MASK) == 0) ? 1.0 : 0.0;
                }
            }
        }
        out[19] = certified;
        if (n > 20) out[20] = seg;
    }
    return 4;
}
GRAPE_BARRIER(h ? &h->err : &g_create_error)

int grape_get_cert_table(grape_handle *h, int *dims, double *coef, int *exps) try {
    if (!h || !dims) return GRAPE_ERR_INVALID;
    if (h->open || !h->shards.empty()) {
        h->err = "grape_get_cert_table: a closed handle on one device";
        return GRAPE_ERR_INVALID;
    }
    const int nt = h->cert_n8 + h->cert_n6;
    dims[0] = h->KC; dims[1] = h->cert_n8; dims[2] = h->cert_n6;
    if (!h->d_cert || !nt) { dims[1] = dims[2] = 0; return GRAPE_OK; }
    HIPCHK(h, hipSetDevice(h->device));
    if (coef) HIPCHK(h, hipMemcpy(coef, h->d_cert, (size_t)h->KC * nt * sizeof(double), hipMemcpyDeviceToHost));
    if (exps) HIPCHK(h, hipMemcpy(exps, h->d_cert_exp, (size_t)nt * sizeof(int), hipMemcpyDeviceToHost));
    return GRAPE_OK;
}
GRAPE_BARRIER(h ? &h->err : &g_create_error)

int grape_get_seg_table(grape_handle *h, int *dims, double *coef, int *exps) try {
    if (!h || !dims) return GRAPE_ERR_INVALID;
    if (h->open || !h->shards.empty()) {
        h->err = "grape_get_seg_table: a closed handle on one device";
        return GRAPE_ERR_INVALID;
    }
    const int n4 = h->seg_n4, n8 = h->seg_n8, n12 = h->seg_n12, nt = n4 + n8 + n12;
    dims[0] = h->KC; dims[1] = n4; dims[2] = n8; dims[3] = n12;
    if (!h->d_seg || !nt) { dims[1] = dims[2] = dims[3] = 0; return GRAPE_OK; }
    HIPCHK(h, hipSetDevice(h->device));
    if (coef) {
        HIPCHK(h, hipMemcpy2D(coef, (size_t)nt * sizeof(double), h->d_seg, (size_t)(n4 + n12) * sizeof(double), (size_t)n4 * sizeof(double),
                              (size_t)h->KC, hipMemcpyDeviceToHost));
        HIPCHK(h, hipMemcpy2D(coef + n4, (size_t)nt * sizeof(double), h->d_seg8, (size_t)h->seg8_stride * sizeof(double), (size_t)n8 * sizeof(double),
                              (size_t)h->KC, hipMemcpyDeviceToHost));
        HIPCHK(h, hipMemcpy2D(coef + n4 + n8, (size_t)nt * sizeof(double), h->d_seg + n4, (size_t)(n4 + n12) * sizeof(double), (size_t)n12 * sizeof(double),
                              (size_t)h->KC, hipMemcpyDeviceToHost));
    }
    if (exps) {
        HIPCHK(h, hipMemcpy(exps, h->d_seg_exp + h->seg_exp_off, (size_t)n4 * sizeof(int), hipMemcpyDeviceToHost));
        HIPCHK(h, hipMemcpy(exps + n4, h->d_seg_exp, (size_t)n8 * sizeof(int), hipMemcpyDeviceToHost));
        HIPCHK(h, hipMemcpy(exps + n4 + n8, h->d_seg_exp + h->seg_exp_off + n4, (size_t)n12 * sizeof(int), hipMemcpyDeviceToHost));
    }
    return GRAPE_OK;
}
GRAPE_BARRIER(h ? &h->err : &g_create_error)

int grape_get_time_gradient(grape_handle *h, double *dJdt) try {
    if (h && h->open) return open_refuse(h, "grape_get_time_gradient");
    if (!h || !dJdt) return GRAPE_ERR_INVALID;
    const int N_T = h->N_T;
    if (!h->shards.empty()) {
// ... 986 lines not shown
```

grape.jl_amd/csrc/grape_kernels.hip.h:

```cpp
#pragma once
#include <hip/hip_runtime.h>
#include <stdint.h>

#include "grape_t18_coeffs.h"
#include "grape_econ_coeffs.h"

typedef double d4 __attribute__((ext_vector_type(4)));

#define MFMA64(a, b, c) __builtin_amdgcn_mfma_f64_16x16x4f64((a), (b), (c), 0, 0, 0)

__device__ __constant__ double c_pade3[4] = {120., 60., 12., 1.};
__device__ __constant__ double c_pade5[6] = {30240., 15120., 3360., 420., 30., 1.};
__device__ __constant__ double c_pade7[8] = {17297280., 8648640., 1995840., 277200., 25200., 1512., 56., 1.};
__device__ __constant__ double c_pade9[10] = {17643225600., 8821612800., 2075673600., 302702400.,
                                              30270240., 2162160., 110880., 3960., 90., 1.};
#define B13_0 64764752532480000.
#define B13_1 32382376266240000.
#define B13_2 7771770303897600.
#define B13_3 1187353796428800.
#define B13_4 129060195264000.
#define B13_5 10559470521600.
#define B13_6 670442572800.
#define B13_7 33522128640.
#define B13_8 1323241920.
#define B13_9 40840800.
#define B13_10 960960.
#define B13_11 16380.
#define B13_12 182.
#define B13_13 1.

#define GRAPE_STAT_SHARDS 64
#define GRAPE_STAT_SLOTS 16
__device__ __forceinline__ void stat_add(unsigned long long *stats, int idx, unsigned long long v) {
    atomicAdd(&stats[(size_t)(blockIdx.x & (GRAPE_STAT_SHARDS - 1)) * GRAPE_STAT_SLOTS + idx], v);
}

struct ExpmArgs {
    const double *H0f;
    const double *Hcf;
    const double *eps;
    const double *shape;
    const double *dts;
    double2 *U;
    int *flags;
    unsigned long long *stats;
    int K, L, N_T, hc_per_traj;
    const int *rep;
    int *cellflag;
    const double *n1;
    int n1_k;
    int *cell_list;
    int listed;
    const double *Sf;
#ifdef GRAPE_DIAG
    int ablate;
    unsigned long long *stamps;
#endif
};

#define T16_PLAN_R 1.15
#define T16_PLAN_RS 1.11
#define T16_PLAN_SMAX 3
struct T16PlanArgs {
    const double *gram;
    const double *eps, *shape, *dts;
    int *flags;
    int KC, L, N_T, N;
    int *splan;
    int sq_on;
    const double *cert;
    const int *cert_exp;
    int n8, n6;
    int *verdict;
    const double *seg;
    const double *seg8;
    const int *seg_exp;
    const int *seg8_exp;
    int seg8_stride, s8, n4, n12;
    int *segplan;
};
#define T16_PLAN_SQ_MASK 0xFF
#define T16_PLAN_CERT 0x100
#define T16_PLAN_TPB 128
#define T16_PLAN_LMAX 4
#define T16_PLAN_PMAX 12
typedef double T16PlanPowers[T16_PLAN_PMAX + 1][T16_PLAN_TPB];
template <int LT>
__device__ __forceinline__ void t16_trace_poly(const double *t, const int *ex, const int n, const T16PlanPowers *pw, double &p, double &S) {
    const int tid = threadIdx.x;
    double sp = 0., sa = 0.;
    for (int i0 = 0; i0 < n; i0 += 8) {
        unsigned x[8];
        double c[8], mono[8];
#pragma unroll
        for (int u = 0; u < 8; ++u) {
            const int i = min(i0 + u, n - 1);
            x[u] = (unsigned)ex[i];
            c[u] = i0 + u < n ? t[i] : 0.0;
        }
#pragma unroll
        for (int u = 0; u < 8; ++u) {
            mono[u] = pw[0][x[u] & 15u][tid];
#pragma unroll
            for (int l = 1; l < LT; ++l) mono[u] *= pw[l][(x[u] >> (4 * l)) & 15u][tid];
        }
#pragma unroll
        for (int u = 0; u < 8; ++u) {
            sp += c[u] * mono[u];
            sa += fabs(c[u]) * fabs(mono[u]);
        }
    }
    p = sp; S = sa;
}
__device__ __forceinline__ bool t16_certified(const double p8, const double S8, const double p6, const double dt, const int sq) {
    const double dt2 = dt * dt, dt8 = (dt2 * dt2) * (dt2 * dt2);
    constexpr double th2 = T16_THETA * T16_THETA, th8 = (th2 * th2) * (th2 * th2);
    const double lhs = (p8 + 0x1p-30 * S8) * dt8 * (1.0 + 1e-6), rhs = ldexp(th8, 8 * sq);
    return lhs <= rhs && p6 >= 0.0;
}
__device__ __forceinline__ bool t16_seg_certified(const double p4, const double S4, const double p8, const double S8, const double p12,
                                                  const double S12, const double dt) {
    constexpr double th = ECON_SEG_THETA, th2 = th * th, th4 = th2 * th2, th8 = th4 * th4, th12 = th8 * th4;
    const double dt2 = dt * dt, dt4 = dt2 * dt2, dt8 = dt4 * dt4, dt12 = dt8 * dt4;
    const double m4lo = (p4 - 0x1p-30 * S4) * dt4, m4hi = (p4 + 0x1p-30 * S4) * dt4;
    const double m8lo = (p8 - 0x1p-30 * S8) * dt8, m8hi = (p8 + 0x1p-30 * S8) * dt8;
    const double m12hi = (p12 + 0x1p-30 * S12) * dt12;
    if (m4hi * (1.0 + 1e-6) <= th4) return true;
    if (!(m8hi * (1.0 + 1e-6) < th4 * m4lo)) return false;
    const double lo = m8lo - th8, hi = m8hi - th8;
    const double gap = lo > 0.0 ? lo : hi < 0.0 ? -hi : 0.0;
    const double lhs = (m12hi - th12) * (m4hi - th4);
    return (lhs > 0.0 ? lhs * (1.0 + 1e-6) : lhs) < gap * gap;
}
struct T16PlanLds {
    int nc, n8own, ns;
    __host__ __device__ explicit T16PlanLds(const T16PlanArgs &a)
        : nc(a.cert ? a.n8 + a.n6 : 0), n8own((a.seg && !a.cert) ? a.s8 : 0), ns(a.seg ? a.n4 + a.n12 : 0) {}
    __host__ __device__ int entries() const { return nc + n8own + ns; }
};
__host__ __device__ inline size_t t16_plan_lds(const T16PlanArgs &a) {
    if (!(a.cert || a.seg) || a.L > T16_PLAN_LMAX) return 0;
    return (size_t)a.L * sizeof(T16PlanPowers) + (size_t)T16PlanLds(a).entries() * (sizeof(double) + sizeof(int));
}
template <int LT>
__global__ void __launch_bounds__(T16_PLAN_TPB) t16_plan_kernel(T16PlanArgs a) {
    extern __shared__ __attribute__((aligned(16))) double plan_sm[];
    const int tid = threadIdx.x, nbx = (a.N_T + T16_PLAN_TPB - 1) / T16_PLAN_TPB;
    const int kc = blockIdx.x / nbx, n = (blockIdx.x - kc * nbx) * T16_PLAN_TPB + tid;
    constexpr bool tables = LT > 0;
    T16PlanPowers *pw = (T16PlanPowers *)plan_sm;
    const T16PlanLds ly(a);
    const int nc = ly.nc, n8own = ly.n8own, ns = ly.ns;
    double *tt = plan_sm + (size_t)LT * (T16_PLAN_PMAX + 1) * T16_PLAN_TPB;
    int *tx = (int *)(tt + ly.entries());
    if (tables) {
        for (int i = tid; i < nc; i += T16_PLAN_TPB) { tt[i] = a.cert[(size_t)kc * nc + i]; tx[i] = a.cert_exp[i]; }
        for (int i = tid; i < n8own; i += T16_PLAN_TPB) { tt[nc + i] = a.seg8[(size_t)kc * a.seg8_stride + i]; tx[nc + i] = a.seg8_exp[i]; }
        for (int i = tid; i < ns; i += T16_PLAN_TPB) { tt[nc + n8own + i] = a.seg[(size_t)kc * ns + i]; tx[nc + n8own + i] = a.seg_exp[i]; }
        __syncthreads();
    }
    bool out = false;
    if (n < a.N_T) {
        const int cell = kc * a.N_T + n, M = a.L + 1;
        const double *G = a.gram + (size_t)kc * (M * M + M), *kap = G + M * M;
        double e[9];
        e[0] = 1.0;
        for (int l = 0; l < a.L; ++l) e[1 + l] = a.eps[(size_t)l * a.N_T + n] * (a.shape ? a.shape[(size_t)l * a.N_T + n] : 1.0);
        double m2 = 0., wk = 0., w = 0.;
        for (int i = 0; i < M; ++i) {
            for (int j = 0; j < M; ++j) m2 += e[i] * e[j] * G[i * M + j];
            const double wi = fabs(e[i]) * sqrt(fmax(G[i * M + i], 0.0));
            w += wi; wk += wi * kap[i];
        }
        const double dt = a.dts[n];
        const double r = 2.0 * fabs(dt) * sqrt(fmax(m2, 0.0) / (double)a.N) * (w > 0.0 ? wk / w : 1.0);
        out = !(r <= T16_PLAN_R);
        int sq = 0;
        if (a.splan && out && a.sq_on) {
            double rs = r;
            while (sq < T16_PLAN_SMAX && !(rs <= T16_PLAN_RS)) { rs *= 0.5; ++sq; }
            out = !(rs <= T16_PLAN_RS);
            if (out) sq = 0;
        }
        if (tables)
            for (int l = 0; l < LT; ++l) {
                double x = 1.0;
                for (int j = 0; j <= T16_PLAN_PMAX; ++j, x *= e[1 + l]) pw[l][j][tid] = x;
            }
        double p8 = 0., S8 = 0.;
        const bool have8 = a.splan && a.cert;
        if (a.splan) {
            bool cert = false;
            if (tables && a.cert) {
                double p6, S6;
                t16_trace_poly<LT>(tt, tx, a.n8, pw, p8, S8);
                t16_trace_poly<LT>(tt + a.n8, tx + a.n8, a.n6, pw, p6, S6);
                cert = t16_certified(p8, S8, p6, dt, sq);
            }
            if (cert) a.verdict[cell] = 0;
            a.splan[cell] = sq | (cert ? T16_PLAN_CERT : 0);
        }
        if (tables && a.seg) {
            bool seg = false;
            if (sq == 0) {
                const double *t = tt + nc + n8own;
                const int *x = tx + nc + n8own;
                double p4, S4, p12, S12;
                if (!have8) t16_trace_poly<LT>(a.cert ? tt : tt + nc, a.cert ? tx : tx + nc, a.s8, pw, p8, S8);
                t16_trace_poly<LT>(t, x, a.n4, pw, p4, S4);
                t16_trace_poly<LT>(t + a.n4, x + a.n4, a.n12, pw, p12, S12);
                seg = t16_seg_certified(p4, S4, p8, S8, p12, S12, dt);
            }
            a.segplan[cell] = seg ? 1 : 0;
        }
    }
    const unsigned long long m = __ballot(out);
    if ((threadIdx.x & 63) == 0 && m) atomicAdd(&a.flags[6], (int)__popcll(m));
}
__device__ __forceinline__ bool t16_skipped(const int *flags, const int ncell) { return 4L * flags[6] > (long)ncell; }

struct CtrlSumArgs {
    const double *Hcf, *eps, *shape;
    double *Sf;
    int L, N_T, pp2;
    int per_traj;
    const int *rep;
};
__device__ __forceinline__ void ctrl_sum_body(CtrlSumArgs a) {
    const int blk = blockIdx.x, kc = a.per_traj ? blk / a.N_T : 0, n = blk - kc * a.N_T;
    if (a.per_traj) a.Hcf += (size_t)(a.rep ? a.rep[kc] : kc) * a.L * a.pp2;
    double e[8];
    for (int l = 0; l < a.L; ++l) e[l] = a.eps[(size_t)l * a.N_T + n] * (a.shape ? a.shape[(size_t)l * a.N_T + n] : 1.0);
    double2 *dst = (double2 *)(a.Sf + (size_t)blk * a.pp2);
#pragma unroll 4
    for (int i = blockIdx.y * blockDim.x + threadIdx.x; i < a.pp2 / 2; i += gridDim.y * blockDim.x) {
        double2 acc = make_double2(0., 0.);
        for (int l = 0; l < a.L; ++l) {
            const double2 h = ((const double2 *)(a.Hcf + (size_t)l * a.pp2))[i];
            acc.x = fma(e[l], h.x, acc.x); acc.y = fma(e[l], h.y, acc.y);
        }
        dst[i] = acc;
    }
}
__global__ void __launch_bounds__(256) ctrl_sum_kernel(CtrlSumArgs a) { ctrl_sum_body(a); }

__global__ void __launch_bounds__(256) dte_kernel(const double *eps, const double *shape, const double *dts, int L, int N_T, int slots, double *out) {
    const int n = blockIdx.x * blockDim.x + threadIdx.x;
    if (n >= N_T) return;
    double *row = out + (size_t)2 * slots * n;
    row[0] = dts[n];
    for (int l = 0; l < 2 * slots - 1; ++l)
        row[1 + l] = l < L ? eps[(size_t)l * N_T + n] * (shape ? shape[(size_t)l * N_T + n] : 1.0) : 0.0;
}

template <int NT>
struct Strip {
    d4 re[NT];
    d4 im[NT];
};

template <int NT>
__device__ __forceinline__ void strip_zero(Strip<NT> &s) {
#pragma unroll
    for (int t = 0; t < NT; ++t) {
        s.re[t] = (d4){0., 0., 0., 0.};
        s.im[t] = (d4){0., 0., 0., 0.};
    }
// ... 3512 lines not shown
```

grape.jl_amd/csrc/grape_t18.hip:

```cpp
#include <hip/hip_runtime.h>
#include <stdint.h>
#include <string.h>
#include <type_traits>
#include <mutex>
#include <vector>
#include <stdlib.h>
#include <stdio.h>
namespace {
#include "grape_t18.hip.h"
#define GRAPE_BATCH_T18_UNIT
#include "grape_batch.hip.h"
#include "grape_deriv3.hip.h"
#include "grape_econ_coeffs.h"

template <int NT, bool SYM, bool CHEB, bool T16 = false>
hipError_t launch(const ExpmArgs &a, hipStream_t s, int blocks) {
    static size_t lds_set[64] = {0};
    const size_t lds = sizeof(double) * (size_t)T18Lds<NT>::TOTAL;
    int dev = 0;
    hipGetDevice(&dev);
    if (lds_set[dev & 63] < lds) {
        hipError_t e = hipFuncSetAttribute((const void *)expm_t18_kernel<NT, SYM, CHEB, T16>, hipFuncAttributeMaxDynamicSharedMemorySize, (int)lds);
        if (e != hipSuccess) return e;
        lds_set[dev & 63] = lds;
// ... 75 lines not shown
    double2 *fw, *bw;
    int *prog;
    int K, s_per_cell;
    const int *splan;
};
static_assert(sizeof(T16AsmArgs) == 136, "argument block of the assembly kernel");

__device__ __forceinline__ double t16_post_norm1(const ExpmArgs &a, const int cell, double *red, const int tid) {
    constexpr int NP = 64;
    const int kc = cell / a.N_T, n = cell - kc * a.N_T, k = a.rep ? a.rep[kc] : kc;
    const double *h0 = a.H0f + (size_t)k * 2 * NP * NP, *sn = a.Sf + (size_t)(a.hc_per_traj ? cell : n) * 2 * NP * NP;
    const double dt = a.dts[n];
    const int j = tid & 63, part = tid >> 6;
    double sum = 0.;
    for (int i = part; i < NP; i += 4) {
        const double xr = dt * (h0[NP * NP + i * NP + j] + sn[NP * NP + i * NP + j]), xi = -dt * (h0[i * NP + j] + sn[i * NP + j]);
        sum += fast_sqrt(xr * xr + xi * xi);
    }
    red[tid] = sum;
    __syncthreads();
    if (tid < 64) {
        double c = red[tid] + red[64 + tid] + red[128 + tid] + red[192 + tid];
#pragma unroll
        for (int off = 32; off >= 1; off >>= 1) c = fmax(c, __shfl_xor(c, off, 64));
        if (tid == 0) red[256] = c;
    }
    __syncthreads();
    const double nA = red[256];
    __syncthreads();
    return nA;
}

__global__ void __launch_bounds__(256) t16_post_kernel(ExpmArgs a, const int *verdict, const int *prog, int nprog, const int *splan) {
    const int tid = threadIdx.x, lane = tid & 63, ncell = a.K * a.N_T;
    if (t16_skipped(a.flags, ncell)) return;
    if (prog && blockIdx.x == 0) {
        unsigned long long steps = 0;
        for (int i = tid; i < nprog; i += 256) steps += (unsigned long long)prog[i];
        for (int off = 32; off >= 1; off >>= 1) steps += __shfl_xor(steps, off, 64);
        if (lane == 0 && steps) stat_add(a.stats, 12, steps * 4ull * 2ull);
    }
    const int cell = blockIdx.x * 256 + tid;
    const bool valid = cell < ncell;
    const bool ok = valid && verdict[cell] == 0;
    if (valid && !ok) a.cell_list[atomicAdd(&a.flags[4], 1)] = cell;
    const unsigned long long m_ok = __ballot(ok), m_valid = __ballot(valid);
    {
        unsigned long long sq = valid ? (unsigned long long)(splan[cell] & T16_PLAN_SQ_MASK) : 0ull;
        unsigned long long sq_ok = ok ? sq : 0ull;
        for (int off = 32; off >= 1; off >>= 1) { sq += __shfl_xor(sq, off, 64); sq_ok += __shfl_xor(sq_ok, off, 64); }
        if (lane == 0 && sq) stat_add(a.stats, 12, sq * 4ull * 192ull);
        if (lane == 0 && sq_ok) stat_add(a.stats, 13, sq_ok);
    }
    if (lane == 0 && m_valid) {
        stat_add(a.stats, 12, (unsigned long long)__popcll(m_valid) * 4ull * (unsigned long long)(T16Count<4>::CELL + 1));
        if (m_ok) {
            stat_add(a.stats, 14, (unsigned long long)__popcll(m_ok));
            stat_add(a.stats, 15, (unsigned long long)__popcll(m_ok));
        }
        atomicAdd(&a.flags[5], (int)__popcll(m_valid));
    }
}

__global__ void __launch_bounds__(256) t16_credit_kernel(ExpmArgs a) {
    __shared__ double red[264];
    __shared__ int todo[256], ntodo;
    __shared__ unsigned long long cnt[8];
    const int tid = threadIdx.x, lane = tid & 63, ncell = a.K * a.N_T;
    if (t16_skipped(a.flags, ncell)) return;
    if (tid < 8) cnt[tid] = 0;
    if (tid == 0) ntodo = 0;
    __syncthreads();
    auto order_of = [](double nA) { return nA > 2.1 ? 4 : nA > 0.95 ? 3 : nA > 0.25 ? 2 : nA > 0.015 ? 1 : 0; };
    auto squarings_of = [](double nA) {
        if (!(nA > 5.4)) return 0;
        const double r = nA / 5.4;
        const int e = ilogb(r);
        return (r == ldexp(1.0, e)) ? e : e + 1;
    };
    const int cell = blockIdx.x * 256 + tid;
    bool cert = false;
    if (cell < ncell) {
        const double bound = expm_norm_bound(a, cell);
        cert = bound > 2.1 && bound <= 5.4;
        if (!cert) todo[atomicAdd(&ntodo, 1)] = cell;
    }
    const unsigned long long m_cert = __ballot(cert);
    if (lane == 0 && m_cert) atomicAdd(&cnt[2 + 4], (unsigned long long)__popcll(m_cert));
    __syncthreads();
    const int nt = ntodo;
    for (int q = 0; q < nt; ++q) {
        const double nA = t16_post_norm1(a, todo[q], red, tid);
        if (tid == 0) {
            const int sj = squarings_of(nA);
            if (sj) { cnt[0] += (unsigned long long)sj; cnt[1] = max(cnt[1], (unsigned long long)sj); }
            cnt[2 + order_of(nA)] += 1ull;
        }
    }
    __syncthreads();
    if (tid == 0) {
        if (cnt[0]) stat_add(a.stats, 0, cnt[0]);
        for (int o = 0; o < 5; ++o)
            if (cnt[2 + o]) stat_add(a.stats, 3 + o, cnt[2 + o]);
        if (cnt[1]) atomicMax(&a.flags[1], (int)cnt[1]);
    }
}

constexpr int D3_INV_TABLE = 2048;
constexpr int D3_PAIRS_OFF = 32768, D3_ECON_OFF = 32768, D3_ECON_TAB_B = 512;
struct AsmModule {
    hipModule_t mod = nullptr;
    hipFunction_t fn = nullptr, fn_d3 = nullptr, fn_d3s = nullptr, fn_lg = nullptr, fn_d3g = nullptr, fn_d4[2] = {nullptr, nullptr};
    hipFunction_t fn_t18g = nullptr, fn_t16p = nullptr, fn_t16p4 = nullptr, fn_t18gp = nullptr;
    double *inv = nullptr;
};
hipError_t asm_function(int dev, hipFunction_t *fn, hipFunction_t *fn_d3 = nullptr, const double **inv = nullptr,
                        hipFunction_t *fn_d3s = nullptr, hipFunction_t *fn_lg = nullptr, hipFunction_t *fn_d3g = nullptr,
                        hipFunction_t *fn_d4 = nullptr, int d4_index = 0, hipFunction_t *fn_t18g = nullptr,
                        hipFunction_t *fn_t16p = nullptr, int t16p_slots = 2) {
    static AsmModule mods[64];
    static std::mutex mtx;
    std::lock_guard<std::mutex> lock(mtx);
    AsmModule &m = mods[dev & 63];
    if (!m.fn) {
        static std::vector<char> override_co;
        const void *image = (const void *)grape_asm_co_start;
        if (const char *path = getenv("GRAPE_ASM_CO")) {
            if (override_co.empty()) {
                if (FILE *f = fopen(path, "rb")) {
                    fseek(f, 0, SEEK_END);
                    const long n = ftell(f);
                    fseek(f, 0, SEEK_SET);
                    if (n > 0) {
                        override_co.resize((size_t)n);
                        if (fread(override_co.data(), 1, (size_t)n, f) != (size_t)n) override_co.clear();
                    }
                    fclose(f);
                }
            }
            if (override_co.empty()) return hipErrorFileNotFound;
            image = override_co.data();
        }
        hipError_t e = hipModuleLoadData(&m.mod, image);
        if (e != hipSuccess) return e;
        e = hipModuleGetFunction(&m.fn_d3, m.mod, "deriv3_asm");
        if (e != hipSuccess) return e;
        e = hipModuleGetFunction(&m.fn_d3s, m.mod, "deriv3s_asm");
        if (e != hipSuccess) return e;
        e = hipModuleGetFunction(&m.fn_lg, m.mod, "lg_gemm_asm");
        if (e != hipSuccess) return e;
        e = hipModuleGetFunction(&m.fn_d3g, m.mod, "deriv3g_asm");
        if (e != hipSuccess) return e;
        e = hipModuleGetFunction(&m.fn_d4[0], m.mod, "deriv4_asm_128");
        if (e != hipSuccess) return e;
        e = hipModuleGetFunction(&m.fn_d4[1], m.mod, "deriv4_asm_256");
        if (e != hipSuccess) return e;
        e = hipModuleGetFunction(&m.fn_t18g, m.mod, "expm_t18g_asm");
        if (e != hipSuccess) return e;
        e = hipModuleGetFunction(&m.fn_t16p, m.mod, "expm_t16p_asm");
        if (e != hipSuccess) return e;
        e = hipModuleGetFunction(&m.fn_t16p4, m.mod, "expm_t16p4_asm");
        if (e != hipSuccess) return e;
        e = hipModuleGetFunction(&m.fn_t18gp, m.mod, "expm_t18gp_asm");
        if (e != hipSuccess) return e;
        static_assert(D3_PAIRS_OFF >= (D3_INV_TABLE + 20) * 8 && D3_ECON_OFF == D3_INV_TABLE * 16 && ECON_MAXDEG - ECON_MINDEG <= 15, "layout of gen_d3.py");
        std::vector<double> tab((D3_PAIRS_OFF + D3_ECON_OFF + 16 * D3_ECON_TAB_B) / 8);
        tab[0] = 0.0;
        for (int i = 1; i < D3_INV_TABLE; ++i) tab[i] = 1.0 / (double)i;
        for (int a = 0; a < D3_INV_TABLE; ++a) tab[D3_PAIRS_OFF / 8 + 2 * a] = tab[D3_PAIRS_OFF / 8 + 2 * a + 1] = 1.0 / (double)(a + 1);
        for (int i = 0; i < ECON_NSETS; ++i)
            for (int a = 0; a < ECON_DEG[i]; ++a)
                for (int j = 0; j < 2; ++j)
                    tab[(D3_PAIRS_OFF + D3_ECON_OFF + (ECON_DEG[i] - ECON_MINDEG) * D3_ECON_TAB_B) / 8 + 2 * a + j] = ECON_TABS[i][a][j];
        int *pt = (int *)(tab.data() + D3_INV_TABLE);
        int np_ = 0;
        for (int ti = 0; ti < 4; ++ti)
            for (int tj = ti; tj < 4; ++tj)
                for (int plane = 0; plane < 2; ++plane)
                    for (int half = 0; half < 2; ++half) pt[np_++] = plane * 64 * 64 * 8 + ti * 16 * 64 * 8 + tj * 16 * 8;
        e = hipMalloc((void **)&m.inv, sizeof(double) * tab.size());
        if (e != hipSuccess) return e;
        e = hipMemcpy(m.inv, tab.data(), sizeof(double) * tab.size(), hipMemcpyHostToDevice);
        if (e != hipSuccess) return e;
        e = hipModuleGetFunction(&m.fn, m.mod, "expm_t16_asm");
        if (e != hipSuccess) return e;
    }
    if (fn) *fn = m.fn;
    if (fn_d3) *fn_d3 = m.fn_d3;
    if (fn_d3s) *fn_d3s = m.fn_d3s;
    if (fn_lg) *fn_lg = m.fn_lg;
    if (fn_d3g) *fn_d3g = m.fn_d3g;
    if (fn_d4) *fn_d4 = m.fn_d4[d4_index & 1];
    if (fn_t18g) *fn_t18g = m.fn_t18g;
    if (fn_t16p) *fn_t16p = t16p_slots == 4 ? m.fn_t16p4 : t16p_slots == 0 ? m.fn_t18gp : m.fn_t16p;
    if (inv) *inv = m.inv;
    return hipSuccess;
}
}

namespace {
struct D3AsmArgs {
    const double *H0f, *Hcf, *eps, *shape, *dts;
    const double2 *fw, *bw;
    const double *rho;
    double2 *tg;
    double *park;
    int *flags;
    unsigned long long *stats;
    const int *batch_flag;
    const double *inv;
    int K, L, N_T, hc_per_traj, wpt, batches_per_k, mcap, slots;
    double tol2;
    int deep, nblocks;
};
static_assert(sizeof(D3AsmArgs) == 160, "argument block of the assembly kernel");

hipError_t launch_d3_asm(const Deriv3Args &g, hipStream_t s, int blocks, bool general) {
    const Deriv2Args &a = g.d;
    if (a.L < 1 || a.L > (general ? 7 : 8) || blocks < 1 || a.maxm + 2 > D3_INV_TABLE) return hipErrorInvalidValue;
    if ((long)a.N_T + 1 >= (1L << 21) || (long)a.K * a.L * a.N_T >= (1L << 27)) return hipErrorInvalidValue;
    int dev = 0;
    hipError_t e = hipGetDevice(&dev);
    if (e != hipSuccess) return e;
    hipFunction_t fn, fn_s, fn_g;
    const double *inv;
    e = asm_function(dev, nullptr, &fn, &inv, &fn_s, nullptr, &fn_g);
    if (e != hipSuccess) return e;
    if (a.L > 2) fn = fn_s;
    if (general) fn = fn_g;
    D3AsmArgs k{};
    k.H0f = g.H0f; k.Hcf = g.Hcf; k.eps = a.eps; k.shape = a.shape; k.dts = a.dts; k.fw = a.fw; k.bw = a.bw; k.rho = a.rho;
    k.tg = a.tg; k.park = a.park; k.flags = a.flags; k.stats = a.stats; k.batch_flag = a.batch_flag; k.inv = inv;
    k.K = a.K; k.L = a.L; k.N_T = a.N_T; k.hc_per_traj = a.hc_per_traj; k.wpt = g.wpt; k.batches_per_k = a.batches_per_k;
    k.mcap = a.max_order < a.maxm ? a.max_order : a.maxm;
    k.slots = a.maxm + 1;
    k.tol2 = a.tol * a.tol;
    k.deep = (a.deep_redo && a.max_order > k.mcap) ? 1 : 0;
    if (a.batch_econ && !general && a.batch_flag && k.mcap >= ECON_MAXDEG) k.deep |= 2;
    k.nblocks = blocks;
    size_t size = sizeof(k);
    void *cfg[] = {HIP_LAUNCH_PARAM_BUFFER_POINTER, &k, HIP_LAUNCH_PARAM_BUFFER_SIZE, &size, HIP_LAUNCH_PARAM_END};
    return hipModuleLaunchKernel(fn, (unsigned)blocks, 1, 1, 256, 1, 1, 0, s, nullptr, cfg);
}
}

extern "C" const double *grape_econ_pairs(void) {
    int dev = 0;
// ... 28 lines not shown
    Deriv2Args a;
    memcpy(&a, d2args, sizeof(a));
    if (a.L < 1 || a.L > 8 || a.gpark || a.maxm + 2 > D3_INV_TABLE || !H0q3 || !Hcq3 || !H0p3 || !Hcp3) return (int)hipErrorInvalidValue;
    if ((long)a.N_T + 1 >= (1L << 19) || (long)a.K * a.L * a.N_T >= (1L << 27) || a.nbatch_total >= (1 << 24)) return (int)hipErrorInvalidValue;
    int dev = 0;
    hipError_t e = hipGetDevice(&dev);
    if (e != hipSuccess) return (int)e;
    hipFunction_t fn;
    const double *inv;
    e = asm_function(dev, nullptr, nullptr, &inv, nullptr, nullptr, nullptr, &fn, NP == 256);
    if (e != hipSuccess) return (int)e;
    D4AsmArgs k{};
    k.H0q = H0q3; k.Hcq = Hcq3; k.H0p = H0p3; k.Hcp = Hcp3; k.eps = a.eps; k.shape = a.shape; k.dts = a.dts; k.fw = a.fw; k.bw = a.bw;
    k.rho = a.rho; k.tg = a.tg; k.park = a.park; k.flags = a.flags; k.stats = a.stats; k.batch_flag = a.batch_flag; k.inv = inv;
    k.K = a.K; k.L = a.L; k.N_T = a.N_T; k.hc_per_traj = a.hc_per_traj; k.nbatch_total = a.nbatch_total; k.batches_per_k = a.batches_per_k;
    k.mcap = a.max_order < a.maxm ? a.max_order : a.maxm;
    k.slots = a.maxm + 1;
    k.tol2 = a.tol * a.tol;
    k.deep = (a.batch_econ && a.batch_flag && k.mcap >= ECON_MAXDEG) ? 2 : 0;
    k.nblocks = blocks;
    size_t size = sizeof(k);
    void *cfg[] = {HIP_LAUNCH_PARAM_BUFFER_POINTER, &k, HIP_LAUNCH_PARAM_BUFFER_SIZE, &size, HIP_LAUNCH_PARAM_END};
    return (int)hipModuleLaunchKernel(fn, (unsigned)blocks, 1, 1, 256, 1, 1, 0, (hipStream_t)stream, nullptr, cfg);
}

extern "C" int grape_lg_asm_launch(const void *k, size_t size, unsigned blocks, void *stream) {
    if (size != 416 || blocks == 0) return (int)hipErrorInvalidValue;
    int dev = 0;
    hipError_t e = hipGetDevice(&dev);
    if (e != hipSuccess) return (int)e;
    hipFunction_t fn;
    e = asm_function(dev, nullptr, nullptr, nullptr, nullptr, &fn);
    if (e != hipSuccess) return (int)e;
    unsigned char buf[416];
    memcpy(buf, k, sizeof(buf));
    size_t sz = sizeof(buf);
    void *cfg[] = {HIP_LAUNCH_PARAM_BUFFER_POINTER, buf, HIP_LAUNCH_PARAM_BUFFER_SIZE, &sz, HIP_LAUNCH_PARAM_END};
    return (int)hipModuleLaunchKernel(fn, blocks, 1, 1, 256, 1, 1, 0, (hipStream_t)stream, nullptr, cfg);
}

extern "C" void grape_t16_walks(int KC, int N_T, int nblk, int *tab) {
    const long ncell = (long)KC * N_T;
    for (int b = 0; b < nblk; ++b) {
        const long lo = b * ncell / nblk, hi = (b + 1) * ncell / nblk;
        int *e = tab + 4 * b;
        e[3] = 0;
        if (hi == lo) { e[0] = 0; e[1] = 0; e[2] = 1; }
        else if (lo % N_T == 0 || hi % N_T != 0) { e[0] = (int)lo; e[1] = (int)(hi - lo); e[2] = 1; }
        else { e[0] = (int)(hi - 1); e[1] = (int)(hi - lo); e[2] = -1; }
    }
}

extern "C" int grape_t16_asm_launch(const void *args, size_t args_size, int *verdict, void *stream, int blocks,
                                    const void *const *walk, int fuse, int K) {
    if (args_size != sizeof(ExpmArgs)) return (int)hipErrorInvalidValue;
    ExpmArgs a;
    memcpy(&a, args, sizeof(a));
    if (!a.Sf || !verdict || blocks < 1 || !walk || !walk[0] || !walk[5]) return (int)hipErrorInvalidValue;
    if (fuse && (!walk[1] || !walk[2] || !walk[3] || !walk[4] || a.rep || K != a.K)) return (int)hipErrorInvalidValue;
    const long ncell = (long)a.K * a.N_T;
    if (ncell <= 0 || ncell >= (1L << 28)) return (int)hipErrorInvalidValue;
    int dev = 0;
    hipError_t e = hipGetDevice(&dev);
    if (e != hipSuccess) return (int)e;
    hipFunction_t fn;
    e = asm_function(dev, &fn);
    if (e != hipSuccess) return (int)e;
    T16AsmArgs k{};
    k.H0f = a.H0f; k.Sf = a.Sf; k.dts = a.dts; k.U = a.U; k.verdict = verdict; k.rep = a.rep;
    k.KC = a.K; k.N_T = a.N_T; k.nblk = blocks; k.flags = a.flags;
    k.fuse = fuse; k.wgtab = (const int *)walk[0]; k.xinit = (const double2 *)walk[1]; k.fw = (double2 *)walk[2];
    k.bw = (double2 *)walk[3]; k.prog = (int *)walk[4]; k.K = K; k.splan = (const int *)walk[5];
    k.s_per_cell = a.hc_per_traj ? 1 : 0;
    size_t size = sizeof(k);
    void *cfg[] = {HIP_LAUNCH_PARAM_BUFFER_POINTER, &k, HIP_LAUNCH_PARAM_BUFFER_SIZE, &size, HIP_LAUNCH_PARAM_END};
    hipStream_t s = (hipStream_t)stream;
    e = hipModuleLaunchKernel(fn, (unsigned)blocks, 1, 1, 256, 1, 1, 0, s, nullptr, cfg);
    if (e != hipSuccess) return (int)e;
    hipLaunchKernelGGL(t16_post_kernel, dim3((unsigned)((ncell + 255) / 256)), dim3(256), 0, s, a, (const int *)verdict,
                       fuse ? (const int *)walk[4] : (const int *)nullptr, 2 * K, (const int *)walk[5]);
    return (int)hipGetLastError();
}

extern "C" int grape_t16p_asm_launch(const void *args, size_t args_size, int *verdict, void *stream, int blocks,
                                     const void *const *walk, int fuse, int K, const double *dte) {
    if (args_size != sizeof(ExpmArgs)) return (int)hipErrorInvalidValue;
    ExpmArgs a;
    memcpy(&a, args, sizeof(a));
    if (!a.hc_per_traj || a.L < 1 || a.L > 4 || !dte || !verdict || blocks < 1 || !walk || !walk[0] || !walk[5]) return (int)hipErrorInvalidValue;
    if (fuse && (!walk[1] || !walk[2] || !walk[3] || !walk[4] || a.rep || K != a.K)) return (int)hipErrorInvalidValue;
    const long ncell = (long)a.K * a.N_T;
    if (ncell <= 0 || ncell >= (1L << 28)) return (int)hipErrorInvalidValue;
    int dev = 0;
    hipError_t e = hipGetDevice(&dev);
    if (e != hipSuccess) return (int)e;
    hipFunction_t fn;
    e = asm_function(dev, nullptr, nullptr, nullptr, nullptr, nullptr, nullptr, nullptr, 0, nullptr, &fn, a.L <= 2 ? 2 : 4);
    if (e != hipSuccess) return (int)e;
    T16AsmArgs k{};
    k.H0f = a.H0f; k.Sf = a.Hcf; k.dts = dte; k.U = a.U; k.verdict = verdict; k.rep = a.rep;
    k.KC = a.K; k.N_T = a.N_T; k.nblk = blocks; k.flags = a.flags;
    k.fuse = fuse; k.wgtab = (const int *)walk[0]; k.xinit = (const double2 *)walk[1]; k.fw = (double2 *)walk[2];
    k.bw = (double2 *)walk[3]; k.prog = (int *)walk[4]; k.K = K; k.splan = (const int *)walk[5];
    k.s_per_cell = a.L;
    size_t size = sizeof(k);
    void *cfg[] = {HIP_LAUNCH_PARAM_BUFFER_POINTER, &k, HIP_LAUNCH_PARAM_BUFFER_SIZE, &size, HIP_LAUNCH_PARAM_END};
    hipStream_t s = (hipStream_t)stream;
    e = hipModuleLaunchKernel(fn, (unsigned)blocks, 1, 1, 256, 1, 1, 0, s, nullptr, cfg);
    if (e != hipSuccess) return (int)e;
    hipLaunchKernelGGL(t16_post_kernel, dim3((unsigned)((ncell + 255) / 256)), dim3(256), 0, s, a, (const int *)verdict,
                       fuse ? (const int *)walk[4] : (const int *)nullptr, 2 * K, (const int *)walk[5]);
    return (int)hipGetLastError();
}

namespace {
__global__ void __launch_bounds__(256) t18g_post_kernel(ExpmArgs a, const int *verdict, const int *prog, int nprog, const int *splan) {
    const int tid = threadIdx.x, lane = tid & 63, ncell = a.K * a.N_T;
    if (prog && blockIdx.x == 0) {
        unsigned long long steps = 0;
        for (int i = tid; i < nprog; i += 256) steps += (unsigned long long)prog[i];
// ... 102 lines not shown
```

grape.jl_amd/csrc/grape_t18.hip.h:

```cpp
#pragma once
#include "grape_kernels.hip.h"

#ifdef T18_STOP
#define T18_STOP_AT(n, Uout, Src) do { if (T18_STOP == (n)) { _Pragma("unroll") for (int t_ = 0; t_ < NT; ++t_) { (Uout).re[t_] = (Src).re[t_ % (sizeof((Src).re) / sizeof((Src).re[0]))]; (Uout).im[t_] = (Src).im[t_ % (sizeof((Src).im) / sizeof((Src).im[0]))]; } s_out = 0; bad = false; return; } } while (0)
#else
#define T18_STOP_AT(n, Uout, Src) do {} while (0)
#endif

#include "grape_t18_coeffs.h"

template <bool HERM> struct T18Coef;
template <> struct T18Coef<true> {
    static constexpr double A1 = T18_A1, A2 = T18_A2, A3 = T18_A3, B1 = T18_B1, B2 = T18_B2, B3 = T18_B3, B6 = T18_B6,
        C0 = T18_C0, C1 = T18_C1, C2 = T18_C2, C3 = T18_C3, C6 = T18_C6, D0 = T18_D0, D1 = T18_D1, D2 = T18_D2, D3 = T18_D3,
        D6 = T18_D6, E2 = T18_E2, E3 = T18_E3, E6 = T18_E6, B0 = T18_B0, THETA = T18_THETA;
};
template <> struct T18Coef<false> {
    static constexpr double A1 = T18T_A1, A2 = T18T_A2, A3 = T18T_A3, B1 = T18T_B1, B2 = T18T_B2, B3 = T18T_B3, B6 = T18T_B6,
        C0 = T18T_C0, C1 = T18T_C1, C2 = T18T_C2, C3 = T18T_C3, C6 = T18T_C6, D0 = T18T_D0, D1 = T18T_D1, D2 = T18T_D2, D3 = T18T_D3,
        D6 = T18T_D6, E2 = T18T_E2, E3 = T18T_E3, E6 = T18T_E6, B0 = T18T_B0, THETA = T18T_THETA;
};

template <int NT>
struct T18Lds {
// ... 497 lines not shown
        B3.im[t] = CF::C1 * As.im[t] + CF::C2 * A2.im[t] + CF::C3 * A3.im[t] + CF::C6 * A6.im[t];
        B2.re[t] = CF::B1 * As.re[t] + CF::B2 * A2.re[t] + CF::B3 * A3.re[t] + CF::B6 * A6.re[t];
        B2.im[t] = CF::B1 * As.im[t] + CF::B2 * A2.im[t] + CF::B3 * A3.im[t] + CF::B6 * A6.im[t];
        if (t == 0) {
#pragma unroll
            for (int r = 0; r < 4; ++r)
                if (4 * r + rgd == cdiag) { b4r[r] += CF::D0; B3.re[0][r] += CF::C0; B2.re[0][r] += CF::B0; }
        }
        q.p1[t] = b4r; q.p2[t] = (d4){0., 0., 0., 0.}; q.p3[t] = b4r + b4i;
    }
    t18_store_slots<LD, NT, NT>(R, U, wave, lane);
    __syncthreads();
    T18_STOP_AT(7, U, B5);
    STAMP(7);
    t18_gemm<LD, NT, NT, false>(q, R, B5, wave, lane, nohook);
    Strip3M<NT> A9;
    t18_combine<NT, NT>(q, A9);
#pragma unroll
    for (int t = 0; t < NT; ++t) A9.sm[t] = A9.re[t] + A9.im[t];
    T18_STOP_AT(8, U, A9);
    STAMP(8);
    __syncthreads();
#pragma unroll
    for (int t = 0; t < NT; ++t) {
        U.re[t] = A9.re[t] + B3.re[t];
        U.im[t] = A9.im[t] + B3.im[t];
        q.p1[t] = B2.re[t]; q.p2[t] = (d4){0., 0., 0., 0.}; q.p3[t] = B2.re[t] + B2.im[t];
    }
    t18_store_slots<LD, NT, NT>(R, U, wave, lane);
    __syncthreads();
    T18_STOP_AT(9, U, A9);
    STAMP(9);
    t18_gemm<LD, NT, NT, false>(q, R, A9, wave, lane, hook_last);
    t18_combine<NT, NT>(q, U);
    STAMP(10);
    for (int it = 0; it < s; ++it) {
        __syncthreads();
        t18_store_slots<LD, NT, NT>(R, U, wave, lane);
#pragma unroll
        for (int t = 0; t < NT; ++t) U.sm[t] = U.re[t] + U.im[t];
        __syncthreads();
        acc3_zero(q);
        t18_gemm<LD, NT, NT, false>(q, R, U, wave, lane, nohook);
        t18_combine<NT, NT>(q, U);
    }
}

template <int NT>
struct T16Count {
    static constexpr int CELL = T18Count<NT>::SQH + 3 * T18Count<NT>::GP;
    static constexpr int CELL_NOSYM = 4 * T18Count<NT>::GP;
};

template <int NT, bool SYM, class HookFirst, class HookLast>
__device__ __forceinline__ bool expm_t16_cell(double *smem, const int wave, const int lane_in, Strip3M<NT> &U, HookFirst hook_first,
                                              HookLast hook_last) {
#define T16_FRESH_LANE(l) int l = lane_in; asm volatile("" : "+v"(l))
    using LY = T18Lds<NT>;
    constexpr int LD = LY::LD, NS = SYM ? NT - 1 : NT;
    constexpr bool HALF = SYM && NT == 4;
    static_assert(!SYM || NT >= 3, "tile symmetry needs at least three tiles per side");
    double *R = smem, *e1 = smem + LY::E1, *e2 = smem + LY::E2, *red = smem + LY::RED;
    const T18NoHook nohook;
    Strip3M<NT> As, A2, Y0;
    int lane = lane_in;
    t18_load_strip<LD, NT>(R, As, wave, lane);
    {
        Acc3<NS> q;
        acc3_zero(q);
        t18_gemm<LD, NS, NT, HALF>(q, R, As, wave, lane, hook_first);
        t18_combine<NS, NT>(q, A2);
    }
    if constexpr (SYM) {
        if constexpr (NT == 4) rot_exch_write<NT, 2>(e1, A2.re[2], A2.im[2], wave, lane, 1.0);
        rot_exch_write<NT>(e2, A2.re[1], A2.im[1], wave, lane, 1.0);
    }
    __syncthreads();
    if constexpr (SYM) {
        if constexpr (NT == 4) t18_exch_add<NT, 2>(e1, A2, wave, lane);
        t18_exch_read_last<NT>(e2, A2, wave, lane);
    }
    Acc3<NT> q;
    { T16_FRESH_LANE(l2); lane = l2; }
#pragma unroll
    for (int t = 0; t < NT; ++t) {
        U.re[t] = T16_C1 * A2.re[t] + T16_C2 * As.re[t];
        U.im[t] = T16_C1 * A2.im[t] + T16_C2 * As.im[t];
        A2.sm[t] = A2.re[t] + A2.im[t];
    }
    t18_store_slots<LD, NT, NT>(R, U, wave, lane);
    __syncthreads();
    acc3_zero(q);
    t18_gemm<LD, NT, NT, false>(q, R, A2, wave, lane, nohook);
    t18_combine<NT, NT>(q, Y0);
    {
        double f = 0., g = 0.;
#pragma unroll
        for (int t = 0; t < NT; ++t)
#pragma unroll
            for (int r = 0; r < 4; ++r) {
                f = fma(Y0.re[t][r], Y0.re[t][r], f); f = fma(Y0.im[t][r], Y0.im[t][r], f);
                g = fma(A2.re[t][r], Y0.re[t][r], g); g = fma(A2.im[t][r], Y0.im[t][r], g);
            }
        f = wave_sum(f);
        g = wave_sum(g);
        const double n2w = t18_colsum_max<NT>(A2);
        if (lane == 0) { red[wave] = f; red[NT + wave] = g; red[2 * NT + wave] = n2w; }
    }
    __syncthreads();
    bool ok;
    {
        double F = red[0], G = red[NT], n2 = red[2 * NT];
#pragma unroll
        for (int w = 1; w < NT; ++w) { F += red[w]; G += red[NT + w]; n2 = fmax(n2, red[2 * NT + w]); }
        const double m6 = -G / T16_C1;
        const double m8 = (F - (T16_C2 * T16_C2) * m6) / (T16_C1 * T16_C1);
        constexpr double th2 = T16_THETA * T16_THETA, th8 = th2 * th2 * th2 * th2;
        ok = (n2 * (1.0 + 1e-9) <= th2) || (m6 >= 0. && m8 * (1.0 + 1e-9) <= th8);
    }
    ok = __builtin_amdgcn_readfirstlane((int)ok) != 0;
    { T16_FRESH_LANE(l3); lane = l3; }
#pragma unroll
    for (int t = 0; t < NT; ++t) {
        U.re[t] = Y0.re[t] + T16_C3 * A2.re[t] + T16_C4 * As.re[t];
        U.im[t] = Y0.im[t] + T16_C3 * A2.im[t] + T16_C4 * As.im[t];
        const d4 vr = T16_C6 * Y0.re[t] + T16_C7 * A2.re[t], vi = T16_C6 * Y0.im[t] + T16_C7 * A2.im[t];
        q.p1[t] = vr; q.p2[t] = (d4){0., 0., 0., 0.}; q.p3[t] = vr + vi;
        Y0.re[t] += T16_C5 * A2.re[t];
        Y0.im[t] += T16_C5 * A2.im[t];
        Y0.sm[t] = Y0.re[t] + Y0.im[t];
    }
    t18_store_slots<LD, NT, NT>(R, U, wave, lane);
    __syncthreads();
    t18_gemm<LD, NT, NT, false>(q, R, Y0, wave, lane, nohook);
    Strip3M<NT> &Y1 = U;
    t18_combine<NT, NT>(q, Y1);
    __syncthreads();
    { T16_FRESH_LANE(l4); lane = l4; }
    {
        const int cdiag = lane & 15, rgd = lane >> 4;
        constexpr int PL = LY::PL;
        double *x = R + (lane >> 4) * LD + 16 * wave + (lane & 15);
#pragma unroll
        for (int t = 0; t < NT; ++t) {
            const d4 y0r = Y0.re[t] - T16_C5 * A2.re[t], y0i = Y0.im[t] - T16_C5 * A2.im[t];
            const d4 xr = Y1.re[t] + T16_C8 * A2.re[t] + T16_C9 * As.re[t], xi = Y1.im[t] + T16_C8 * A2.im[t] + T16_C9 * As.im[t];
            const int tb = (wave + t) % NT;
#pragma unroll
            for (int r = 0; r < 4; ++r) {
                const int o = (16 * tb + 4 * r) * LD;
                x[o] = xr[r]; x[PL + o] = xi[r]; x[2 * PL + o] = xr[r] + xi[r];
            }
            d4 vr = T16_C12 * Y1.re[t] + T16_C13 * y0r + T16_C14 * A2.re[t] + T16_C15 * As.re[t];
            const d4 vi = T16_C12 * Y1.im[t] + T16_C13 * y0i + T16_C14 * A2.im[t] + T16_C15 * As.im[t];
            if (t == 0) {
#pragma unroll
                for (int r = 0; r < 4; ++r)
                    if (4 * r + rgd == cdiag) vr[r] += T16_C16;
            }
            q.p1[t] = vr; q.p2[t] = (d4){0., 0., 0., 0.}; q.p3[t] = vr + vi;
            Y0.re[t] = Y1.re[t] + T16_C10 * y0r + T16_C11 * As.re[t];
            Y0.im[t] = Y1.im[t] + T16_C10 * y0i + T16_C11 * As.im[t];
            Y0.sm[t] = Y0.re[t] + Y0.im[t];
        }
    }
    __syncthreads();
    t18_gemm<LD, NT, NT, false>(q, R, Y0, wave, lane, hook_last);
    t18_combine<NT, NT>(q, U);
    return ok;
#undef T16_FRESH_LANE
}

template <int NT>
__device__ __forceinline__ void t18_store_u(const ExpmArgs &a, const int cell, const int wave, const int lane, const Strip3M<NT> &T) {
    constexpr int NP = 16 * NT;
    double2 *Uc = a.U + (size_t)cell * NP * NP;
    const int col = 16 * wave + (lane & 15), rg = lane >> 4;
#pragma unroll
    for (int sl = 0; sl < NT; ++sl) {
        const int tb = (wave + sl) % NT;
#pragma unroll
        for (int r = 0; r < 4; ++r) Uc[(16 * tb + 4 * r + rg) * NP + col] = make_double2(T.re[sl][r], T.im[sl][r]);
    }
}

template <int NT>
__device__ __forceinline__ void t18_store_u_slot(const ExpmArgs &a, const int cell, const int wave, const int lane, const Strip<NT> &T,
                                                 const int sl) {
    constexpr int NP = 16 * NT;
    const int tb = (wave + sl) % NT;
    double2 *Ut = a.U + ((size_t)cell * NP + 16 * tb) * NP;
    const unsigned loff = (unsigned)((lane >> 4) * NP + 16 * wave + (lane & 15));
#pragma unroll
    for (int r = 0; r < 4; ++r) (Ut + (size_t)(4 * r) * NP)[loff] = make_double2(T.re[sl][r], T.im[sl][r]);
}

template <int NT, bool SYM, bool CHEB, bool T16 = false>
__device__ __forceinline__ void expm_t18_body(const ExpmArgs &a) {
    static_assert(!T16 || CHEB, "the four-product route is a Hermitian-generator route");
    using LY = T18Lds<NT>;
    extern __shared__ __attribute__((aligned(16))) double smem[];
    const int tid0 = threadIdx.x, lane0 = tid0 & 63;
    const int wave = __builtin_amdgcn_readfirstlane(tid0 >> 6);
    const int ncell = a.K * a.N_T;
    const int x = blockIdx.x & 7, per_x = gridDim.x >> 3;
    const int lo = (int)((long)x * ncell / 8), hi = (int)((long)(x + 1) * ncell / 8);
    const bool skip16 = a.cell_list != nullptr && t16_skipped(a.flags, ncell);
    if (T16 && skip16) return;
    const bool listed = a.listed != 0 && !skip16;
    const int step = listed ? (int)gridDim.x : per_x;
    const int end = listed ? min(__builtin_amdgcn_readfirstlane(a.flags[4]), ncell) : hi;
    const int idx0 = listed ? (int)blockIdx.x : lo + ((int)blockIdx.x >> 3);
    auto cell_at = [&](int i) -> int { return listed ? __builtin_amdgcn_readfirstlane(a.cell_list[i]) : i; };
    int st_s = 0, st_max = 0, st_ord[5] = {0, 0, 0, 0, 0}, st_sq = 0, st_cells = 0, st_t16 = 0;
    bool any_bad = false;
    Strip<NT> Uprev;
    strip_zero(Uprev);
    int prev = -1;
    const int first = idx0 < end ? cell_at(idx0) : 0;
    if (idx0 < end) {
        if constexpr (SYM) {
            T18FormA<64 * NT, NT> fa(a, smem, first, tid0);
            fa.issue();
            fa.commit();
        } else {
            t18_form_a_general<64 * NT, NT>(a, smem, first, tid0);
        }
    }
    __syncthreads();
    for (int idx = idx0; idx < end; idx += step) {
        const int cell = cell_at(idx);
        int lane = lane0, tid = tid0;
        asm volatile("" : "+v"(lane), "+v"(tid));
#ifdef GRAPE_DIAG
        if (tid == 0) g_diag_off[blockIdx.x & 1023] = (idx != idx0 + step);
        __syncthreads();
#endif
        STAMP(0);
        int sj = 0, oj = 0;
        if (!listed) {
            const double bound = expm_norm_bound(a, cell);
            double nA = bound;
            if (!(bound > 2.1 && bound <= 5.4)) nA = t18_norm1<NT>(smem, tid);
            if (nA > 5.4) {
                const double r = nA / 5.4;
                const int e = ilogb(r);
                sj = (r == ldexp(1.0, e)) ? e : e + 1;
            }
            oj = nA > 2.1 ? 4 : nA > 0.95 ? 3 : nA > 0.25 ? 2 : nA > 0.015 ? 1 : 0;
        }
        Strip3M<NT> U;
        int s;
        bool bad;
        STAMP(1);
        const bool have_next = idx + step < end;
        const int next = have_next ? cell_at(idx + step) : cell;
        if constexpr (SYM) {
            T18FormA<64 * NT, NT> fa(a, smem, next, tid);
            auto store_prev = [&](int sk, int r) { if (r == 0 && prev >= 0) t18_store_u_slot<NT>(a, prev, wave, lane, Uprev, sk); };
            auto fetch_next = [&](int sk, int r) { if (sk == 1 && r == 0) fa.issue(); };
            if constexpr (T16) {
                s = 0; bad = false;
                const bool ok16 = expm_t16_cell<NT, true>(smem, wave, lane, U, store_prev, fetch_next);
                if (tid == 0 && a.cellflag) a.cellflag[cell] = ok16 ? 0 : 1;
                if (ok16) st_t16 += 1;
                else if (tid == 0) a.cell_list[atomicAdd(&a.flags[4], 1)] = cell;
            } else {
                expm_t18_cell<NT, true, true>(smem, wave, lane, U, s, bad, store_prev, fetch_next);
            }
            STAMP(11);
            __syncthreads();
            STAMP(12);
            if (have_next) fa.commit();
        } else {
            if constexpr (T16) {
                s = 0; bad = false;
                const bool ok16 = expm_t16_cell<NT, false>(smem, wave, lane, U, T18NoHook(), T18NoHook());
                if (tid == 0 && a.cellflag) a.cellflag[cell] = ok16 ? 0 : 1;
                if (ok16) st_t16 += 1;
                else if (tid == 0) a.cell_list[atomicAdd(&a.flags[4], 1)] = cell;
            } else {
                expm_t18_cell<NT, false, CHEB>(smem, wave, lane, U, s, bad, T18NoHook(), T18NoHook());
            }
#pragma unroll
            for (int sl = 0; sl < NT; ++sl) {
                Strip<NT> Us;
                Us.re[sl] = U.re[sl]; Us.im[sl] = U.im[sl];
                t18_store_u_slot<NT>(a, cell, wave, lane, Us, sl);
            }
            __syncthreads();
            if (have_next) t18_form_a_general<64 * NT, NT>(a, smem, next, tid);
        }
        if constexpr (SYM) {
#pragma unroll
            for (int t = 0; t < NT; ++t) { Uprev.re[t] = U.re[t]; Uprev.im[t] = U.im[t]; }
            prev = cell;
        }
        any_bad |= bad;
        st_s += sj; st_max = max(st_max, sj); st_ord[oj] += listed ? 0 : 1;
        st_sq += s; st_cells += 1;
        __syncthreads();
        STAMP(13);
    }
    if (prev >= 0) {
#pragma unroll
        for (int sl = 0; sl < NT; ++sl) t18_store_u_slot<NT>(a, prev, wave, lane0, Uprev, sl);
    }
#ifdef GRAPE_DIAG
    if (tid0 == 0) g_diag_off[blockIdx.x & 1023] = 0;
#endif
    if (tid0 == 0) {
        stat_add(a.stats, 0, (unsigned long long)st_s);
#pragma unroll
        for (int o = 0; o < 5; ++o)
            if (st_ord[o]) stat_add(a.stats, 3 + o, (unsigned long long)st_ord[o]);
        if (st_max > 0) atomicMax(&a.flags[1], st_max);
        unsigned long long mi = (unsigned long long)st_cells * (T16 ? (SYM ? T16Count<NT>::CELL : T16Count<NT>::CELL_NOSYM) : SYM ? T18Count<NT>::CELL : T18Count<NT>::CELL_GENERAL)
                                + (unsigned long long)st_sq * T18Count<NT>::GP;
        if constexpr (T16) {
            stat_add(a.stats, 15, (unsigned long long)st_t16);
            atomicAdd(&a.flags[5], st_cells);
        }
        stat_add(a.stats, 12, (unsigned long long)NT * mi);
        stat_add(a.stats, 13, (unsigned long long)st_sq);
        stat_add(a.stats, 14, (unsigned long long)(T16 ? st_t16 : st_cells));
        if (any_bad) atomicOr(&a.flags[0], 64);
    }
}
template <int NT, bool SYM, bool CHEB, bool T16 = false>
__global__ void __launch_bounds__(NT * 64, (T16 && NT == 3) ? 2 : 1) expm_t18_kernel(ExpmArgs a) { expm_t18_body<NT, SYM, CHEB, T16>(a); }
```

grape.jl_amd/csrc/grape_t18_coeffs.h:

```cpp
#pragma once
#define T18_THETA 2.0
#define T18T_THETA 1.09
#define T18_A1 -0.10036558103014462001
#define T18_A2 -0.007456351650625886579
#define T18_A3 -0.00083091953191006175088
#define T18_B1 -0.14075572409909292308
#define T18_B2 1.0955465096236762141
#define T18_B3 0.29811198744557154804
#define T18_B6 -0.00057207257428924858549
#define T18_C0 -4.7094393853968811891
#define T18_C1 1.7157463766850012865
#define T18_C2 0.073686948027488562391
#define T18_C3 -0.0033650385206633560936
#define T18_C6 0.000033927981037541774044
#define T18_D0 0.0
#define T18_D1 -0.24222749901747747758
#define T18_D2 0.050668391204088569683
#define T18_D3 0.023404567895744140748
#define T18_D6 -0.000010355013205937047443
#define T18_E2 -0.13912895765004587534
#define T18_E3 -0.013910627366173824328
#define T18_E6 -0.000014649629174709440602
#define T18_B0 0.99999999999999999921
#define T18T_A1 -0.10036558103014462001
#define T18T_A2 -0.0080292464824115696008
#define T18T_A3 -0.00089213849804572995564
#define T18T_B1 0.24591022090110863764
#define T18T_B2 1.362667083208190483
#define T18T_B3 0.49892102569169427267
#define T18T_B6 -0.00064092743005853663879
#define T18T_C0 -11.148502971774368372
#define T18T_C1 1.6801581387890619718
#define T18T_C2 0.05717798464788655127
#define T18T_C3 -0.0069821012248805208429
#define T18T_C6 0.000033497501708607053831
#define T18T_D0 0.0
#define T18T_D1 -0.067640451907138190756
#define T18T_D2 0.067596130177045964608
#define T18T_D3 0.029555257042931552743
#define T18T_D6 -0.000013918025751606070112
#define T18T_E2 -0.092336461936711859281
#define T18T_E3 -0.01693649390020817172
#define T18T_E6 -0.00001400867981820361598
#define T18T_B0 1.0

#define T16_THETA 1.36
#define T16_C1 0.0003990485980387312666
#define T16_C2 0.0029228143276988285886
#define T16_C3 -0.0077470178547223424775
#define T16_C4 0.40523011494938120965
#define T16_C5 0.032514297214079020788
#define T16_C6 5.6985532981688705678
#define T16_C7 0.022467770221737013362
#define T16_C8 0.2375283509963317365
#define T16_C9 2.1834336740729687939
#define T16_C10 -5.7548650707099555138
#define T16_C11 -0.024893888233397960765
#define T16_C12 10.136883359859348227
#define T16_C13 -61.008736429296066557
#define T16_C14 0.32660098775353450156
#define T16_C15 0.9999999999999999025
#define T16_C16 0.99999999999999991128
```

Baseline: 55.81.

## Add T16Q expm variant with C2=0 coefficients skipping the guard product

Adds a second degree-16 matrix exponential scheme whose coefficient C2 is zero. This lets certified cells replace the full second product and norm-check reduction with a half-size product. A new assembly kernel generator and a HIP template path select this variant per cell through a plan bit, enabled by default when there are enough cells per block. The trade-off is a smaller validity radius (theta 1.11), so more cells depend on certification, and the kernel code and branching become more complex.

```diff
diff --git a/grape.jl_amd/api.py b/grape.jl_amd/api.py
--- a/grape.jl_amd/api.py
+++ b/grape.jl_amd/api.py
@@ -63,7 +63,7 @@
 def build_asm(verbose: bool = False, workdir: str | None = None) -> str:
     asm_dir = os.path.join(_CSRC, "asm")
     work = workdir or asm_dir
-    kernels = (("gen_t16.py", "expm_t16_asm"), ("gen_t16p.py", "expm_t16p_asm"), ("gen_t16p.py", "expm_t16p4_asm"), ("gen_t18g.py", "expm_t18g_asm"), ("gen_t18gp.py", "expm_t18gp_asm"), ("gen_d3.py", "deriv3_asm"), ("gen_d3s.py", "deriv3s_asm"), ("gen_d3s.py", "deriv3g_asm"),
+    kernels = (("gen_t16.py", "expm_t16_asm"), ("gen_t16q.py", "expm_t16q_asm"), ("gen_t16p.py", "expm_t16p_asm"), ("gen_t16p.py", "expm_t16p4_asm"), ("gen_t18g.py", "expm_t18g_asm"), ("gen_t18gp.py", "expm_t18gp_asm"), ("gen_d3.py", "deriv3_asm"), ("gen_d3s.py", "deriv3s_asm"), ("gen_d3s.py", "deriv3g_asm"),
                ("gen_lg.py", "lg_gemm_asm"), ("gen_d4.py", "deriv4_asm_128"), ("gen_d4.py", "deriv4_asm_256"))
     co_path, emb_s, emb_o = os.path.join(work, "grape_asm.co"), os.path.join(work, "asm_embed.S"), os.path.join(work, "asm_embed.o")
     llvm = "/opt/rocm/lib/llvm/bin"
@@ -95,7 +95,7 @@
 def _sources():
     srcs = [os.path.join(_CSRC, f) for f in ("grape_hip.hip", "grape_t18.hip", "grape_kernels.hip.h", "grape_large.hip.h",
                                              "grape_series.hip.h", "grape_cheby.hip.h", "grape_t18.hip.h", "grape_t18_coeffs.h",
-                                             "grape_deriv3.hip.h", "grape_timegrad.hip.h", "grape_batch.hip.h", "grape_lindblad.hip.h", "grape_lindblad_tg.hip.h", "grape_hvp.hip.h", "grape_hvp_split.hip.h", "grape_lindblad_hvp.hip.h", "grape_lindblad_hvp_split.hip.h", "grape_lindblad_batch.hip.h", "grape_lindblad_rc.hip.h", "grape_devmem.h", "grape_cert.hip.h", "grape_expect.hip.h", "grape_econ_coeffs.h", os.path.join("asm", "gen_t16.py"), os.path.join("asm", "gen_t16p.py"), os.path.join("asm", "gen_t18g.py"), os.path.join("asm", "gen_t18gp.py"), os.path.join("asm", "gen_d3.py"), os.path.join("asm", "gen_d3s.py"), os.path.join("asm", "gen_lg.py"), os.path.join("asm", "gen_d4.py"), os.path.join("asm", "gcn.py"))]
+                                             "grape_deriv3.hip.h", "grape_timegrad.hip.h", "grape_batch.hip.h", "grape_lindblad.hip.h", "grape_lindblad_tg.hip.h", "grape_hvp.hip.h", "grape_hvp_split.hip.h", "grape_lindblad_hvp.hip.h", "grape_lindblad_hvp_split.hip.h", "grape_lindblad_batch.hip.h", "grape_lindblad_rc.hip.h", "grape_devmem.h", "grape_cert.hip.h", "grape_expect.hip.h", "grape_econ_coeffs.h", os.path.join("asm", "gen_t16.py"), os.path.join("asm", "gen_t16q.py"), os.path.join("asm", "gen_t16p.py"), os.path.join("asm", "gen_t18g.py"), os.path.join("asm", "gen_t18gp.py"), os.path.join("asm", "gen_d3.py"), os.path.join("asm", "gen_d3s.py"), os.path.join("asm", "gen_lg.py"), os.path.join("asm", "gen_d4.py"), os.path.join("asm", "gcn.py"))]
     return srcs, os.path.join(_HERE, "..", "include", "grape_hip.h")
 
 
@@ -513,13 +513,13 @@
         self._chk(self._lib.grape_reset_timings(self._h))
 
     def work(self):
-        w = np.zeros(21)
-        self._lib.grape_get_work(self._h, w.ctypes.data, 21)
+        w = np.zeros(22)
+        self._lib.grape_get_work(self._h, w.ctypes.data, 22)
         return dict(cells=w[0], squarings=w[1], flop_expm=w[2], flop_deriv=w[3], deriv_orders=w[4],
                     pivoted_cells=w[5], expm_cells=w[6], series_terms=w[7], series_steps=w[8],
                     t18_mfma_flop=w[9], t18_squarings=w[10], t18_cells=w[11], matrix_free_fallback=w[12], t16_cells=w[13],
                     asm_kernel=w[14], asm_deriv_kernel=w[15], asm_blocked_products=w[16],
-                    walk_steps=w[17], scan_block=w[18], t16_certified=w[19], seg_certified=w[20])
+                    walk_steps=w[17], scan_block=w[18], t16_certified=w[19], seg_certified=w[20], t16q_cells=w[21])
 
     def cert_table(self):
         dims = np.zeros(3, np.int32)
diff --git a/grape.jl_amd/csrc/asm/gen_t16.py b/grape.jl_amd/csrc/asm/gen_t16.py
--- a/grape.jl_amd/csrc/asm/gen_t16.py
+++ b/grape.jl_amd/csrc/asm/gen_t16.py
@@ -2,6 +2,7 @@
 import re
 import struct
 import sys
+from types import SimpleNamespace
 
 sys.path.insert(0, os.path.dirname(os.path.abspath(__file__)))
 from gcn import Prog, Reg, V, A, S, VCC, EXEC, Neg, Abs, kernel_text
@@ -499,7 +500,7 @@
 
         sk0 = 0
         if fused:
-            assert NS == 4 and not half_last and not bload
+            assert not bload and (NS == 4 or (NS == 3 and half_last))
 
             def rdk(pl, so, r):
                 p.tag = "fragment"
@@ -514,7 +515,7 @@
             for r in range(4):
                 for pl in range(3):
                     rdk(pl, 0, r)
-            for so in range(4):
+            for so in range(NS):
                 gaps = [[] for _ in range(12)]
                 if so < 3:
                     fused["valu"](so + 1)
@@ -522,7 +523,7 @@
                     for q, st in enumerate(pend):
                         gaps[4 * (q // 2) + (q % 2)].append(st)
                     last = {pl: (4 * pl + 1 if pend else 0) for pl in range(3)}
-                    for r in range(4):
+                    for r in range(4 if so + 1 < NS else 0):
                         for pl in range(3):
                             gaps[max(last[pl], 3 * r + pl)].append(lambda pl=pl, r=r: rdk(pl, so + 1, r))
                 j = 0
@@ -607,6 +608,18 @@
             p.dpp_mov(tmp.sub(1), x.sub(1), ctrl, row_mask=rm)
             p.valu(op, x, x, tmp)
 
+    def second_product_fork(self, cx):
+        pass
+
+    def second_product_square(self, cx, L_join):
+        pass
+
+    def cell_coeffs(self, q):
+        return None
+
+    def load_c16(self, k16):
+        self.smov64(k16, self.c["C16"])
+
     def cell(self):
         p, c = self.p, self.s_c
         vp, ap = self.vp, self.ap
@@ -673,6 +686,8 @@
             p.ds_write(64, self.v_EW1, A2im[1].d(r), EXH + 128 * r)
         p.s_waitcnt(lgkm=0)
         p.s_barrier()
+        cx = SimpleNamespace(Qt=Qt, A2re=A2re, A2im=A2im, A2sm=A2sm)
+        self.second_product_fork(cx)
         self.advance()
         self.cell_bases_issue(self.s_nkc, self.s_nn, self.s_ncell)
         txr, txi = vp.alloc(), vp.alloc()
@@ -708,7 +723,8 @@
                                 lambda r=r, a2r=a2r, a2i=a2i: p.valu("v_add_f64", A2sm[sl].d(r), a2r, a2i)])
             self.interleave(streams)
 
-        self.product(Qt, [A2re, A2im, A2sm], fused={"valu": valu2, "stores": lambda sl: self.plane_stores(sl, tt[0], tt[1], Qt[sl][1])})
+        self.product(Qt, [A2re, A2im, A2sm], fused={"valu": valu2, "stores": lambda sl: self.plane_stores(sl, tt[0], tt[1], Qt[sl][1]),
+                                                    "post": self.cell_coeffs(False)})
         for t in tt + A2sm:
             vp.free(t)
         self.cell_bases_finish(self.s_nkc)
@@ -830,6 +846,7 @@
         p.s_waitcnt(lgkm=0)
         p.s_barrier()
         p.salu("s_and_b32", self.s_prop, self.s_prop, 1)
+        self.second_product_square(cx, L_vdone)
         p.label(L_vdone)
         self.A2p_re, self.A2p_im = ap.alloc(4), ap.alloc(4)
         Bre, Bim, Bsm = [None] * 4, [None] * 4, [None] * 4
@@ -881,7 +898,7 @@
         self.stamp(7)
         self.stamp(8)
         k16 = S(58, 2)
-        self.smov64(k16, self.c["C16"])
+        self.load_c16(k16)
         tt = [vp.alloc() for _ in range(4)]
 
         def valu4(sl):
diff --git a/grape.jl_amd/csrc/asm/gen_t16q.py b/grape.jl_amd/csrc/asm/gen_t16q.py
--- /dev/null
+++ b/grape.jl_amd/csrc/asm/gen_t16q.py
@@ -0,0 +1,146 @@
+import os
+import re
+import sys
+
+sys.path.insert(0, os.path.dirname(os.path.abspath(__file__)))
+from gcn import S, Neg, kernel_text
+import gen_t16 as g16
+from gen_t16 import E1, E2, EXH, LDS_BYTES, KERNARG
+
+HERE = os.path.dirname(os.path.abspath(__file__))
+Q_BIT = 0x200
+MFMA_Q = 120 + 120 + 2 * 192 + 1
+
+
+def t16q_coeffs():
+    txt = open(os.path.join(HERE, "..", "grape_t18_coeffs.h")).read()
+    c = {}
+    for m in re.finditer(r"#define\s+T16Q_(C\d+|THETA)\s+([-+0-9.eE]+)", txt):
+        c[m.group(1)] = float(m.group(2))
+    assert len(c) == 17 and c["C2"] == 0.0, c
+    return c
+
+
+class GenQ(g16.Gen):
+    def __init__(self, name="expm_t16q_asm", **kw):
+        super().__init__(name=name, **kw)
+        self.cq = t16q_coeffs()
+
+    def cell_coeffs(self, q):
+        c = self.cq if q else self.c
+
+        def load():
+            for i in range(3, 16):
+                self.smov64(self.s_c[i], c[f"C{i}"])
+        return load
+
+    def load_c16(self, k16):
+        p = self.p
+        lo, hi = g16.dbits(self.c["C16"])
+        qlo, qhi = g16.dbits(self.cq["C16"])
+        p.salu("s_and_b32", self.s_tmp[4], self.s_scur, Q_BIT)
+        self.ssel(k16.sub(0), qlo, lo)
+        self.ssel(k16.sub(1), qhi, hi)
+
+    def second_product_fork(self, cx):
+        p = self.p
+        uid = len(p.ins)
+        cx.L_q = f"L_q_{uid}"
+        cx.pool = list(self.vp.free_tiles)
+        p.salu("s_and_b32", self.s_tmp[0], self.s_scur, Q_BIT)
+        p.s_branch("s_cbranch_scc1", cx.L_q)
+
+    def second_product_square(self, cx, L_join):
+        p, vp = self.p, self.vp
+        Qt, A2re, A2im, A2sm = cx.Qt, cx.A2re, cx.A2im, cx.A2sm
+        p.s_branch("s_branch", L_join)
+        p.label(cx.L_q)
+        joined = list(vp.free_tiles)
+        vp.free_tiles[:] = cx.pool
+
+        self.advance()
+        self.cell_bases_issue(self.s_nkc, self.s_nn, self.s_ncell)
+        txr, txi = vp.alloc(), vp.alloc()
+        for h in range(2):
+            p.ds_read(128, txr.sub(4 * h, 4), self.v_ER, 16 * h)
+            p.ds_read(128, txi.sub(4 * h, 4), self.v_ER, EXH + 16 * h)
+            p.ds_read(128, A2re[3].sub(4 * h, 4), self.v_ER, (E2 - E1) + 16 * h)
+            p.ds_read(128, A2im[3].sub(4 * h, 4), self.v_ER, (E2 - E1) + EXH + 16 * h)
+        self.stamp(2)
+        tx1 = (txr, txi)
+
+        def valu(sl):
+            if sl == 2:
+                for r in range(4):
+                    p.valu("v_add_f64", A2re[2].d(r), A2re[2].d(r), tx1[0].d(r))
+                    p.valu("v_add_f64", A2im[2].d(r), A2im[2].d(r), Neg(tx1[1].d(r)))
+                for r in range(4):
+                    p.valu("v_mul_f64", A2im[3].d(r), A2im[3].d(r), -1.0)
+                vp.free(tx1[0])
+                vp.free(tx1[1])
+            for r in range(4):
+                p.valu("v_add_f64", A2sm[sl].d(r), A2re[sl].d(r), A2im[sl].d(r))
+
+        self.product(Qt[:3], [A2re, A2im, A2sm], half_last=True,
+                     fused={"valu": valu, "stores": lambda sl: self.plane_stores(sl, A2re[sl], A2im[sl], A2sm[sl]),
+                            "post": self.cell_coeffs(True)})
+        for t in A2sm:
+            vp.free(t)
+        self.cell_bases_finish(self.s_nkc)
+        self.stamp(3)
+        kq = S(58, 2)
+        self.smov64(kq, self.cq["C1"])
+        streams = []
+        for sl in range(3):
+            for r in range(4):
+                p1, p2, p3 = (Qt[sl][j].d(r) for j in range(3))
+                streams.append([lambda p3=p3, p1=p1: p.valu("v_add_f64", p3, p3, Neg(p1)),
+                                lambda p1=p1, p2=p2: p.valu("v_add_f64", p1, p1, Neg(p2)),
+                                lambda p3=p3, p2=p2: p.valu("v_add_f64", p3, p3, Neg(p2)),
+                                lambda p1=p1: p.valu("v_mul_f64", p1, kq, p1),
+                                lambda p3=p3: p.valu("v_mul_f64", p3, kq, p3)])
+        for g in range(0, len(streams), 4):
+            self.interleave(streams[g:g + 4])
+        for r in range(4):
+            p.ds_write(64, self.v_EW2, Qt[2][0].d(r), 128 * r)
+            p.ds_write(64, self.v_EW2, Qt[2][2].d(r), EXH + 128 * r)
+            p.ds_write(64, self.v_EW1, Qt[1][0].d(r), 128 * r)
+            p.ds_write(64, self.v_EW1, Qt[1][2].d(r), EXH + 128 * r)
+        p.s_waitcnt(lgkm=0)
+        p.s_barrier()
+        txr, txi = vp.alloc(), vp.alloc()
+        for h in range(2):
+            p.ds_read(128, txr.sub(4 * h, 4), self.v_ER, 16 * h)
+            p.ds_read(128, txi.sub(4 * h, 4), self.v_ER, EXH + 16 * h)
+            p.ds_read(128, Qt[3][0].sub(4 * h, 4), self.v_ER, (E2 - E1) + 16 * h)
+            p.ds_read(128, Qt[3][2].sub(4 * h, 4), self.v_ER, (E2 - E1) + EXH + 16 * h)
+        drop = vp.alloc()
+        p.mfma(drop, A2re[0].d(0), A2re[0].d(0), 0)
+        vp.free(drop)
+        for r in range(4):
+            p.valu("v_add_f64", Qt[2][0].d(r), Qt[2][0].d(r), txr.d(r))
+            p.valu("v_add_f64", Qt[2][2].d(r), Qt[2][2].d(r), Neg(txi.d(r)))
+        for r in range(4):
+            p.valu("v_mul_f64", Qt[3][2].d(r), Qt[3][2].d(r), -1.0)
+        vp.free(txr)
+        vp.free(txi)
+        p.salu("s_and_b32", self.s_prop, self.s_prop, 1)
+        self.stamp(4)
+        assert sorted(vp.free_tiles) == sorted(joined), (vp.free_tiles, joined)
+
+
+def generate(path=None, **kw):
+    g = GenQ(**kw)
+    prog = g.build()
+    text = kernel_text(prog, KERNARG, LDS_BYTES)
+    if path:
+        with open(path, "w") as f:
+            f.write(text)
+    return g, prog, text
+
+
+if __name__ == "__main__":
+    out = sys.argv[1] if len(sys.argv) > 1 else os.path.join(HERE, "expm_t16q_asm.s")
+    g, prog, _ = generate(out)
+    print(f"{out}: {len(prog.ins)} lines, {prog.count('mfma')} matrix instructions, {prog.count('valu') + prog.count('dpp')} vector, "
+          f"{prog.count('lds')} LDS, {prog.count('vmem')} global, {prog.auto_nops} wait states inserted")
diff --git a/grape.jl_amd/csrc/grape_hip.hip b/grape.jl_amd/csrc/grape_hip.hip
--- a/grape.jl_amd/csrc/grape_hip.hip
+++ b/grape.jl_amd/csrc/grape_hip.hip
@@ -118,6 +118,11 @@
     int *d_seg_exp = nullptr;
     int seg_n8 = 0, seg_n4 = 0, seg_n12 = 0, seg8_stride = 0, seg_exp_off = 0;
     int *d_segplan = nullptr;
+    double *d_t86 = nullptr, *d_t412 = nullptr;
+    int *d_texp = nullptr;
+    int t_n8 = 0, t_n6 = 0, t_n4 = 0, t_n12 = 0;
+    bool asm16q = false;
+    bool t16q_twin = false;
     bool asm16 = false;
     bool asm16p = false;
     double *d_dte = nullptr;
@@ -360,7 +365,7 @@
 extern "C" int grape_t18g_asm_launch(const void *args, size_t args_size, int *verdict, void *stream, int blocks,
                                      const void *const *walk, int fuse, int K, const double *dte);
 extern "C" int grape_t16_asm_launch(const void *args, size_t args_size, int *verdict, void *stream, int blocks,
-                                    const void *const *walk, int fuse, int K);
+                                    const void *const *walk, int fuse, int K, int q);
 extern "C" int grape_t18_batch_launch(int herm, const void *args, size_t args_size, const void *strides, size_t strides_size,
                                       int sets, void *stream, int blocks);
 extern "C" void grape_t16_walks(int KC, int N_T, int nblk, int *tab);
@@ -2839,6 +2844,11 @@
     if (h->asm16 || h->asm18g) {
         const long ncell = (long)h->KC * N_T;
         h->asm_blocks = (int)std::max<long>(1, std::min<long>(h->num_cus, ncell));
+        {
+            const char *envt = getenv("GRAPE_EXPM_T16Q");
+            const bool eligible = h->asm16 && !h->asm16p && !p->hc_per_traj && L >= 1 && L <= 2;
+            h->asm16q = eligible && (envt ? atoi(envt) != 0 : ncell >= (long)T16Q_MIN_WALK * h->asm_blocks);
+        }
         std::vector<int> tab((size_t)4 * h->asm_blocks);
         grape_t16_walks(h->KC, N_T, h->asm_blocks, tab.data());
         CCHK(h->mem.alloc(&h->d_wgtab, tab.size()));
@@ -2866,6 +2876,16 @@
             CCHK(hipMemcpy(h->d_xinit, xi.data(), xi.size() * 8, hipMemcpyHostToDevice));
             CCHK(h->mem.alloc(&h->d_prog, (size_t)2 * K));
             CCHK(hipMemset(h->d_prog, 0, (size_t)2 * K * sizeof(int)));
+        }
+    }
+    if (!h->asm16 && !h->asm18g && h->t16 && h->t18 && h->herm && !h->large && !h->series && h->NT == 4 && !p->hc_per_traj && L >= 1 && L <= 2 &&
+        (long)K * N_T < (1L << 28)) {
+        const char *envt = getenv("GRAPE_EXPM_T16Q");
+        const long ncell = (long)h->KC * N_T, blocks = std::max<long>(1, std::min<long>(h->num_cus, ncell));
+        h->t16q_twin = envt ? atoi(envt) != 0 : ncell >= (long)T16Q_MIN_WALK * blocks;
+        if (h->t16q_twin) {
+            CCHK(h->mem.alloc(&h->d_splan, (size_t)ncell));
+            CCHK(hipMemset(h->d_splan, 0, (size_t)ncell * sizeof(int)));
         }
     }
     if (h->t16 && h->t18 && h->herm && !h->large && !h->series && (h->NT >= 3 || (h->NT == 2 && h->t18_small))) {
@@ -2928,24 +2948,32 @@
         static_assert(T16_PLAN_LMAX == GRAPE_CERT_LMAX, "power table of t16_plan_kernel");
         const bool want_cert = h->asm16 && L >= 1 && L <= GRAPE_CERT_LMAX && !(envc && atoi(envc) == 0);
         const bool want_seg = h->asm16 && h->deriv_econ && L >= 1 && L <= 2 && !(envg && atoi(envg) == 0);
-        if (want_cert || want_seg) {
-            const CertPlan pl(L, want_seg);
+        const bool want_q = h->asm16q || h->t16q_twin;
+        const bool build_cert = want_cert || want_q, build_seg = want_seg || want_q;
+        if (build_cert || build_seg) {
+            const CertPlan pl(L, build_seg);
             const int nt = pl.n8 + pl.n6, ns = pl.n4 + pl.n12;
+            CCHK(h->mem.alloc(&h->d_texp, pl.exps.size()));
+            CCHK(hipMemcpy(h->d_texp, pl.exps.data(), pl.exps.size() * sizeof(int), hipMemcpyHostToDevice));
+            h->t_n8 = pl.n8; h->t_n6 = pl.n6;
+            if (build_cert) CCHK(h->mem.alloc(&h->d_t86, (size_t)KCn * nt));
+            if (build_seg) {
+                h->t_n4 = pl.n4; h->t_n12 = pl.n12;
+                CCHK(h->mem.alloc(&h->d_t412, (size_t)KCn * ns));
+            }
             if (want_cert) {
                 h->cert_n8 = pl.n8; h->cert_n6 = pl.n6;
-                CCHK(h->mem.alloc(&h->d_cert, (size_t)KCn * nt));
-                CCHK(h->mem.alloc(&h->d_cert_exp, (size_t)nt));
-                CCHK(hipMemcpy(h->d_cert_exp, pl.exps.data(), (size_t)nt * sizeof(int), hipMemcpyHostToDevice));
+                h->d_cert = h->d_t86; h->d_cert_exp = h->d_texp;
             }
             if (want_seg) {
                 h->seg_n8 = pl.n8; h->seg_n4 = pl.n4; h->seg_n12 = pl.n12; h->seg_exp_off = nt;
-                CCHK(h->mem.alloc(&h->d_seg, (size_t)KCn * ns));
-                CCHK(h->mem.alloc(&h->d_seg_exp, pl.exps.size()));
-                CCHK(hipMemcpy(h->d_seg_exp, pl.exps.data(), pl.exps.size() * sizeof(int), hipMemcpyHostToDevice));
-                if (want_cert) { h->d_seg8 = h->d_cert; h->seg8_stride = nt; }
-                else { CCHK(h->mem.alloc(&h->d_seg8, (size_t)KCn * pl.n8)); h->seg8_stride = pl.n8; }
+                h->d_seg = h->d_t412; h->d_seg_exp = h->d_texp;
                 CCHK(h->mem.alloc(&h->d_segplan, (size_t)KCn * N_T));
                 CCHK(hipMemset(h->d_segplan, 0, (size_t)KCn * N_T * sizeof(int)));
+            }
+            if (build_seg) {
+                if (build_cert) { h->d_seg8 = h->d_t86; h->seg8_stride = nt; }
+                else { CCHK(h->mem.alloc(&h->d_seg8, (size_t)KCn * pl.n8)); h->seg8_stride = pl.n8; }
             }
             DeviceBufs tmp;
             int *d_job[8] = {nullptr, nullptr, nullptr, nullptr, nullptr, nullptr, nullptr, nullptr};
@@ -2965,17 +2993,17 @@
                 hipLaunchKernelGGL(cert_mm_kernel, dim3((unsigned)pl.n2, nc), dim3(256), 0, 0, d_scr, pl.nmat, N, pl.M, (const int *)d_job[0], (const int *)d_job[1]);
                 hipLaunchKernelGGL(cert_mm_kernel, dim3((unsigned)(pl.n3 + pl.n4), nc), dim3(256), 0, 0, d_scr, pl.nmat, N, pl.M + pl.n2, (const int *)d_job[2],
                                    (const int *)d_job[3]);
-                if (want_cert)
+                if (build_cert)
                     hipLaunchKernelGGL(cert_trace_kernel, dim3((unsigned)nt, nc), dim3(256), 0, 0, (const double2 *)d_scr, pl.nmat, N, (const int *)d_job[4],
-                                       (const int *)d_job[5], nt, h->d_cert + (size_t)kc0 * nt);
+                                       (const int *)d_job[5], nt, h->d_t86 + (size_t)kc0 * nt);
                 else
                     hipLaunchKernelGGL(cert_trace_kernel, dim3((unsigned)pl.n8, nc), dim3(256), 0, 0, (const double2 *)d_scr, pl.nmat, N, (const int *)d_job[4],
                                        (const int *)d_job[5], pl.n8, h->d_seg8 + (size_t)kc0 * pl.n8);
-                if (want_seg) {
+                if (build_seg) {
                     hipLaunchKernelGGL(cert_mm_kernel, dim3((unsigned)pl.n6, nc), dim3(256), 0, 0, d_scr, pl.nmat, N, pl.M + pl.n2 + pl.n3 + pl.n4,
                                        (const int *)d_job[6], (const int *)d_job[7]);
                     hipLaunchKernelGGL(cert_trace_kernel, dim3((unsigned)ns, nc), dim3(256), 0, 0, (const double2 *)d_scr, pl.nmat, N,
-                                       (const int *)d_job[4] + nt, (const int *)d_job[5], ns, h->d_seg + (size_t)kc0 * ns);
+                                       (const int *)d_job[4] + nt, (const int *)d_job[5], ns, h->d_t412 + (size_t)kc0 * ns);
                 }
                 CCHK(hipGetLastError());
             }
@@ -3106,13 +3134,14 @@
                     T16PlanArgs pa{};
                     pa.gram = h->d_gram; pa.eps = h->d_eps; pa.shape = h->d_shape; pa.dts = h->d_dts; pa.flags = h->d_flags;
                     pa.KC = h->KC; pa.L = h->L; pa.N_T = h->N_T; pa.N = h->N;
-                    pa.splan = (h->asm16 && (h->asm_sq || h->d_cert)) ? h->d_splan : nullptr;
-                    pa.sq_on = h->asm_sq ? 1 : 0;
-                    pa.cert = h->d_cert; pa.cert_exp = h->d_cert_exp; pa.n8 = h->cert_n8; pa.n6 = h->cert_n6;
+                    pa.splan = ((h->asm16 && (h->asm_sq || h->d_cert || h->asm16q)) || h->t16q_twin) ? h->d_splan : nullptr;
+                    pa.sq_on = (h->asm16 && h->asm_sq) ? 1 : 0;
+                    pa.cert = h->d_t86; pa.cert_exp = h->d_t86 ? h->d_texp : nullptr; pa.n8 = h->t_n8; pa.n6 = h->t_n6;
                     pa.verdict = h->d_cellflag;
-                    pa.seg = h->d_seg; pa.seg8 = h->d_seg8; pa.seg8_stride = h->seg8_stride; pa.seg8_exp = h->d_seg_exp;
-                    pa.seg_exp = h->d_seg_exp ? h->d_seg_exp + h->seg_exp_off : nullptr;
-                    pa.s8 = h->seg_n8; pa.n4 = h->seg_n4; pa.n12 = h->seg_n12; pa.segplan = h->d_segplan;
+                    pa.seg = h->d_t412; pa.seg8 = h->d_seg8; pa.seg8_stride = h->seg8_stride; pa.seg8_exp = h->d_t412 ? h->d_texp : nullptr;
+                    pa.seg_exp = h->d_t412 ? h->d_texp + h->t_n8 + h->t_n6 : nullptr;
+                    pa.s8 = h->d_t412 ? h->t_n8 : 0; pa.n4 = h->t_n4; pa.n12 = h->t_n12; pa.segplan = h->d_segplan;
+                    pa.cert_use = h->d_cert ? 1 : 0; pa.seg_use = h->d_seg ? 1 : 0; pa.q_use = (h->asm16q || h->t16q_twin) ? 1 : 0;
                     const unsigned plan_blocks = (unsigned)(h->KC * ((h->N_T + T16_PLAN_TPB - 1) / T16_PLAN_TPB));
                     const size_t plan_lds = t16_plan_lds(pa);
                     switch (plan_lds ? h->L : 0) {
@@ -3152,11 +3181,13 @@
                     walk_fuse = h->asm_walk & (1 | ((h->fuse && h->fuse_on && h->want_bw) ? 2 : 0));
                     if (walk_fuse) HIPCHK(h, stream_fill(h->d_prog, 0, (size_t)2 * h->K * sizeof(int), s));
                     const void *walk[6] = {h->d_wgtab, h->d_xinit, h->d_fw, h->d_bw, h->d_prog, h->d_splan};
-                    e = (hipError_t)grape_t16_asm_launch(&ea, sizeof(ea), h->d_cellflag, (void *)s, h->asm_blocks, walk, walk_fuse, h->K);
+                    e = (hipError_t)grape_t16_asm_launch(&ea, sizeof(ea), h->d_cellflag, (void *)s, h->asm_blocks, walk, walk_fuse, h->K, h->asm16q ? 1 : 0);
                     h->credit_pending = true;
                 }
-                else
+                else {
+                    ea.splan = h->t16q_twin ? h->d_splan : nullptr;
                     e = (hipError_t)grape_t18_launch(h->NT, h->herm ? 1 : 0, t16 ? 1 : 0, &ea, sizeof(ea), (void *)s, blocks16);
+                }
                 if (t16 && e == hipSuccess) {
                     ea.listed = 1;
                     e = (hipError_t)grape_t18_launch(h->NT, 1, 0, &ea, sizeof(ea), (void *)s, t18_blocks);
@@ -4224,10 +4255,10 @@
     if (!h || !out || n < 4) return GRAPE_ERR_INVALID;
     if (h->open) return open_work(h, out, n);
     if (!h->shards.empty()) {
-        const int m = n < 21 ? n : 21;
+        const int m = n < 22 ? n : 22;
         std::fill(out, out + m, 0.0);
         for (grape_handle *c : h->shards) {
-            double cw[21] = {0.};
+            double cw[22] = {0.};
             const int rc = grape_get_work(c, cw, m);
             if (rc < 0) return multi_fail(h, c, rc);
             for (int i = 0; i < m; ++i) out[i] = (i == 15 || i == 16 || i == 18) ? cw[i] : out[i] + cw[i];
@@ -4293,9 +4324,10 @@
     }
     if (n > 18) out[18] = h->scan16 ? (double)h->scan_Bk : 0.0;
     if (n > 19) {
-        double certified = 0.0, seg = 0.0;
+        double certified = 0.0, seg = 0.0, qcells = 0.0;
         const bool want_seg = n > 20 && h->d_segplan && h->deriv_econ;
-        if ((h->d_cert || want_seg) && h->d_splan && !h->series) {
+        const bool want_q = n > 21 && (h->asm16q || h->t16q_twin);
+        if ((h->d_cert || want_seg || want_q) && h->d_splan && !h->series) {
             const size_t ncell = (size_t)h->KC * h->N_T;
             std::vector<int> plan(ncell);
             int fl[8];
@@ -4304,6 +4336,8 @@
             const bool tried = !(4L * fl[6] > (long)ncell);
             if (tried && h->d_cert)
                 for (int w : plan) certified += (w & T16_PLAN_CERT) ? 1.0 : 0.0;
+            if (tried && want_q)
+                for (int w : plan) qcells += (w & T16_PLAN_Q) ? 1.0 : 0.0;
             if (tried && want_seg) {
                 std::vector<int> sp(ncell), verdict(ncell);
                 { const int rc_ = getter_fetch(h, sp.data(), h->d_segplan, ncell * sizeof(int)); if (rc_) return rc_; }
@@ -4317,6 +4351,7 @@
         }
         out[19] = certified;
         if (n > 20) out[20] = seg;
+        if (n > 21) out[21] = qcells;
     }
     return 4;
 }
diff --git a/grape.jl_amd/csrc/grape_kernels.hip.h b/grape.jl_amd/csrc/grape_kernels.hip.h
--- a/grape.jl_amd/csrc/grape_kernels.hip.h
+++ b/grape.jl_amd/csrc/grape_kernels.hip.h
@@ -52,6 +52,7 @@
     int *cell_list;
     int listed;
     const double *Sf;
+    const int *splan;
 #ifdef GRAPE_DIAG
     int ablate;
     unsigned long long *stamps;
@@ -78,9 +79,14 @@
     const int *seg8_exp;
     int seg8_stride, s8, n4, n12;
     int *segplan;
+    int cert_use, seg_use;
+    int q_use;
 };
 #define T16_PLAN_SQ_MASK 0xFF
 #define T16_PLAN_CERT 0x100
+#define T16_PLAN_Q 0x200
+#define T16Q_MIN_WALK 8
+static_assert(T16Q_THETA == ECON_SEG_THETA, "the segment the plan certifies is the one the T16Q_* set was made for");
 #define T16_PLAN_TPB 128
 #define T16_PLAN_LMAX 4
 #define T16_PLAN_PMAX 12
@@ -187,20 +193,22 @@
                 double x = 1.0;
                 for (int j = 0; j <= T16_PLAN_PMAX; ++j, x *= e[1 + l]) pw[l][j][tid] = x;
             }
-        double p8 = 0., S8 = 0.;
-        const bool have8 = a.splan && a.cert;
+        double p8 = 0., S8 = 0., p6 = 0.;
+        const bool q_use = tables && a.q_use && a.splan && a.cert && a.seg;
+        const bool have8 = a.splan && a.cert && (a.cert_use || q_use);
+        int word = sq;
         if (a.splan) {
             bool cert = false;
-            if (tables && a.cert) {
-                double p6, S6;
+            if (tables && have8) {
+                double S6;
                 t16_trace_poly<LT>(tt, tx, a.n8, pw, p8, S8);
                 t16_trace_poly<LT>(tt + a.n8, tx + a.n8, a.n6, pw, p6, S6);
-                cert = t16_certified(p8, S8, p6, dt, sq);
+                cert = a.cert_use && t16_certified(p8, S8, p6, dt, sq);
             }
             if (cert) a.verdict[cell] = 0;
-            a.splan[cell] = sq | (cert ? T16_PLAN_CERT : 0);
-        }
-        if (tables && a.seg) {
+            word |= cert ? T16_PLAN_CERT : 0;
+        }
+        if (tables && a.seg && (a.seg_use || q_use)) {
             bool seg = false;
             if (sq == 0) {
                 const double *t = tt + nc + n8own;
@@ -211,8 +219,13 @@
                 t16_trace_poly<LT>(t + a.n4, x + a.n4, a.n12, pw, p12, S12);
                 seg = t16_seg_certified(p4, S4, p8, S8, p12, S12, dt);
             }
-            a.segplan[cell] = seg ? 1 : 0;
-        }
+            if (a.seg_use) a.segplan[cell] = seg ? 1 : 0;
+            if (q_use && seg && t16_certified(p8, S8, p6, dt, 0)) {
+                a.verdict[cell] = 0;
+                word |= T16_PLAN_Q;
+            }
+        }
+        if (a.splan) a.splan[cell] = word;
     }
     const unsigned long long m = __ballot(out);
     if ((threadIdx.x & 63) == 0 && m) atomicAdd(&a.flags[6], (int)__popcll(m));
diff --git a/grape.jl_amd/csrc/grape_t18.hip b/grape.jl_amd/csrc/grape_t18.hip
--- a/grape.jl_amd/csrc/grape_t18.hip
+++ b/grape.jl_amd/csrc/grape_t18.hip
@@ -151,8 +151,10 @@
         if (lane == 0 && sq) stat_add(a.stats, 12, sq * 4ull * 192ull);
         if (lane == 0 && sq_ok) stat_add(a.stats, 13, sq_ok);
     }
+    const unsigned long long m_q = __ballot(valid && (splan[cell] & T16_PLAN_Q));
     if (lane == 0 && m_valid) {
-        stat_add(a.stats, 12, (unsigned long long)__popcll(m_valid) * 4ull * (unsigned long long)(T16Count<4>::CELL + 1));
+        stat_add(a.stats, 12, (unsigned long long)__popcll(m_valid) * 4ull * (unsigned long long)(T16Count<4>::CELL + 1)
+                                  - (unsigned long long)__popcll(m_q) * 4ull * (unsigned long long)(T18Count<4>::GP - T18Count<4>::SQH));
         if (m_ok) {
             stat_add(a.stats, 14, (unsigned long long)__popcll(m_ok));
             stat_add(a.stats, 15, (unsigned long long)__popcll(m_ok));
@@ -210,13 +212,13 @@
 struct AsmModule {
     hipModule_t mod = nullptr;
     hipFunction_t fn = nullptr, fn_d3 = nullptr, fn_d3s = nullptr, fn_lg = nullptr, fn_d3g = nullptr, fn_d4[2] = {nullptr, nullptr};
-    hipFunction_t fn_t18g = nullptr, fn_t16p = nullptr, fn_t16p4 = nullptr, fn_t18gp = nullptr;
+    hipFunction_t fn_t18g = nullptr, fn_t16p = nullptr, fn_t16p4 = nullptr, fn_t18gp = nullptr, fn_t16q = nullptr;
     double *inv = nullptr;
 };
 hipError_t asm_function(int dev, hipFunction_t *fn, hipFunction_t *fn_d3 = nullptr, const double **inv = nullptr,
                         hipFunction_t *fn_d3s = nullptr, hipFunction_t *fn_lg = nullptr, hipFunction_t *fn_d3g = nullptr,
                         hipFunction_t *fn_d4 = nullptr, int d4_index = 0, hipFunction_t *fn_t18g = nullptr,
-                        hipFunction_t *fn_t16p = nullptr, int t16p_slots = 2) {
+                        hipFunction_t *fn_t16p = nullptr, int t16p_slots = 2, hipFunction_t *fn_t16q = nullptr) {
     static AsmModule mods[64];
     static std::mutex mtx;
     std::lock_guard<std::mutex> lock(mtx);
@@ -262,6 +264,8 @@
         if (e != hipSuccess) return e;
         e = hipModuleGetFunction(&m.fn_t18gp, m.mod, "expm_t18gp_asm");
         if (e != hipSuccess) return e;
+        e = hipModuleGetFunction(&m.fn_t16q, m.mod, "expm_t16q_asm");
+        if (e != hipSuccess) return e;
         static_assert(D3_PAIRS_OFF >= (D3_INV_TABLE + 20) * 8 && D3_ECON_OFF == D3_INV_TABLE * 16 && ECON_MAXDEG - ECON_MINDEG <= 15, "layout of gen_d3.py");
         std::vector<double> tab((D3_PAIRS_OFF + D3_ECON_OFF + 16 * D3_ECON_TAB_B) / 8);
         tab[0] = 0.0;
@@ -292,6 +296,7 @@
     if (fn_d4) *fn_d4 = m.fn_d4[d4_index & 1];
     if (fn_t18g) *fn_t18g = m.fn_t18g;
     if (fn_t16p) *fn_t16p = t16p_slots == 4 ? m.fn_t16p4 : t16p_slots == 0 ? m.fn_t18gp : m.fn_t16p;
+    if (fn_t16q) *fn_t16q = m.fn_t16q;
     if (inv) *inv = m.inv;
     return hipSuccess;
 }
@@ -426,7 +431,7 @@
 }
 
 extern "C" int grape_t16_asm_launch(const void *args, size_t args_size, int *verdict, void *stream, int blocks,
-                                    const void *const *walk, int fuse, int K) {
+                                    const void *const *walk, int fuse, int K, int q) {
     if (args_size != sizeof(ExpmArgs)) return (int)hipErrorInvalidValue;
     ExpmArgs a;
     memcpy(&a, args, sizeof(a));
@@ -437,9 +442,10 @@
     int dev = 0;
     hipError_t e = hipGetDevice(&dev);
     if (e != hipSuccess) return (int)e;
-    hipFunction_t fn;
-    e = asm_function(dev, &fn);
-    if (e != hipSuccess) return (int)e;
+    hipFunction_t fn, fn_q;
+    e = asm_function(dev, &fn, nullptr, nullptr, nullptr, nullptr, nullptr, nullptr, 0, nullptr, nullptr, 2, &fn_q);
+    if (e != hipSuccess) return (int)e;
+    if (q) fn = fn_q;
     T16AsmArgs k{};
     k.H0f = a.H0f; k.Sf = a.Sf; k.dts = a.dts; k.U = a.U; k.verdict = verdict; k.rep = a.rep;
     k.KC = a.K; k.N_T = a.N_T; k.nblk = blocks; k.flags = a.flags;
diff --git a/grape.jl_amd/csrc/grape_t18.hip.h b/grape.jl_amd/csrc/grape_t18.hip.h
--- a/grape.jl_amd/csrc/grape_t18.hip.h
+++ b/grape.jl_amd/csrc/grape_t18.hip.h
@@ -573,7 +573,7 @@
     static constexpr int CELL_NOSYM = 4 * T18Count<NT>::GP;
 };
 
-template <int NT, bool SYM, class HookFirst, class HookLast>
+template <int NT, bool SYM, bool Q = false, class HookFirst, class HookLast>
 __device__ __forceinline__ bool expm_t16_cell(double *smem, const int wave, const int lane_in, Strip3M<NT> &U, HookFirst hook_first,
                                               HookLast hook_last) {
 #define T16_FRESH_LANE(l) int l = lane_in; asm volatile("" : "+v"(l))
@@ -581,6 +581,11 @@
     constexpr int LD = LY::LD, NS = SYM ? NT - 1 : NT;
     constexpr bool HALF = SYM && NT == 4;
     static_assert(!SYM || NT >= 3, "tile symmetry needs at least three tiles per side");
+    static_assert(!Q || (SYM && NT == 4), "the Hermitian-square path is a four-tile path");
+#define T16_K(i) constexpr double K##i = Q ? T16Q_C##i : T16_C##i
+    T16_K(1); T16_K(2); T16_K(3); T16_K(4); T16_K(5); T16_K(6); T16_K(7); T16_K(8); T16_K(9); T16_K(10); T16_K(11); T16_K(12); T16_K(13);
+    T16_K(14); T16_K(15); T16_K(16);
+#undef T16_K
     double *R = smem, *e1 = smem + LY::E1, *e2 = smem + LY::E2, *red = smem + LY::RED;
     const T18NoHook nohook;
     Strip3M<NT> As, A2, Y0;
@@ -603,52 +608,74 @@
     }
     Acc3<NT> q;
     { T16_FRESH_LANE(l2); lane = l2; }
-#pragma unroll
-    for (int t = 0; t < NT; ++t) {
-        U.re[t] = T16_C1 * A2.re[t] + T16_C2 * As.re[t];
-        U.im[t] = T16_C1 * A2.im[t] + T16_C2 * As.im[t];
-        A2.sm[t] = A2.re[t] + A2.im[t];
-    }
-    t18_store_slots<LD, NT, NT>(R, U, wave, lane);
-    __syncthreads();
-    acc3_zero(q);
-    t18_gemm<LD, NT, NT, false>(q, R, A2, wave, lane, nohook);
-    t18_combine<NT, NT>(q, Y0);
-    {
-        double f = 0., g = 0.;
-#pragma unroll
-        for (int t = 0; t < NT; ++t)
-#pragma unroll
-            for (int r = 0; r < 4; ++r) {
-                f = fma(Y0.re[t][r], Y0.re[t][r], f); f = fma(Y0.im[t][r], Y0.im[t][r], f);
-                g = fma(A2.re[t][r], Y0.re[t][r], g); g = fma(A2.im[t][r], Y0.im[t][r], g);
-            }
-        f = wave_sum(f);
-        g = wave_sum(g);
-        const double n2w = t18_colsum_max<NT>(A2);
-        if (lane == 0) { red[wave] = f; red[NT + wave] = g; red[2 * NT + wave] = n2w; }
-    }
-    __syncthreads();
     bool ok;
-    {
-        double F = red[0], G = red[NT], n2 = red[2 * NT];
-#pragma unroll
-        for (int w = 1; w < NT; ++w) { F += red[w]; G += red[NT + w]; n2 = fmax(n2, red[2 * NT + w]); }
-        const double m6 = -G / T16_C1;
-        const double m8 = (F - (T16_C2 * T16_C2) * m6) / (T16_C1 * T16_C1);
-        constexpr double th2 = T16_THETA * T16_THETA, th8 = th2 * th2 * th2 * th2;
-        ok = (n2 * (1.0 + 1e-9) <= th2) || (m6 >= 0. && m8 * (1.0 + 1e-9) <= th8);
+    if constexpr (Q) {
+        (void)K2;
+#pragma unroll
+        for (int t = 0; t < NT; ++t) A2.sm[t] = A2.re[t] + A2.im[t];
+        t18_store_slots<LD, NT, NT>(R, A2, wave, lane);
+        __syncthreads();
+        {
+            Acc3<NS> qh;
+            acc3_zero(qh);
+            t18_gemm<LD, NS, NT, HALF>(qh, R, A2, wave, lane, nohook);
+            t18_combine<NS, NT>(qh, Y0);
+        }
+#pragma unroll
+        for (int t = 0; t < NS; ++t) { Y0.re[t] = K1 * Y0.re[t]; Y0.im[t] = K1 * Y0.im[t]; }
+        rot_exch_write<NT, 2>(e1, Y0.re[2], Y0.im[2], wave, lane, 1.0);
+        rot_exch_write<NT>(e2, Y0.re[1], Y0.im[1], wave, lane, 1.0);
+        __syncthreads();
+        t18_exch_add<NT, 2>(e1, Y0, wave, lane);
+        t18_exch_read_last<NT>(e2, Y0, wave, lane);
+        ok = true;
+    } else {
+#pragma unroll
+        for (int t = 0; t < NT; ++t) {
+            U.re[t] = K1 * A2.re[t] + K2 * As.re[t];
+            U.im[t] = K1 * A2.im[t] + K2 * As.im[t];
+            A2.sm[t] = A2.re[t] + A2.im[t];
+        }
+        t18_store_slots<LD, NT, NT>(R, U, wave, lane);
+        __syncthreads();
+        acc3_zero(q);
+        t18_gemm<LD, NT, NT, false>(q, R, A2, wave, lane, nohook);
+        t18_combine<NT, NT>(q, Y0);
+        {
+            double f = 0., g = 0.;
+#pragma unroll
+            for (int t = 0; t < NT; ++t)
+#pragma unroll
+                for (int r = 0; r < 4; ++r) {
+                    f = fma(Y0.re[t][r], Y0.re[t][r], f); f = fma(Y0.im[t][r], Y0.im[t][r], f);
+                    g = fma(A2.re[t][r], Y0.re[t][r], g); g = fma(A2.im[t][r], Y0.im[t][r], g);
+                }
+            f = wave_sum(f);
+            g = wave_sum(g);
+            const double n2w = t18_colsum_max<NT>(A2);
+            if (lane == 0) { red[wave] = f; red[NT + wave] = g; red[2 * NT + wave] = n2w; }
+        }
+        __syncthreads();
+        {
+            double F = red[0], G = red[NT], n2 = red[2 * NT];
+#pragma unroll
+            for (int w = 1; w < NT; ++w) { F += red[w]; G += red[NT + w]; n2 = fmax(n2, red[2 * NT + w]); }
+            const double m6 = -G / K1;
+            const double m8 = (F - (K2 * K2) * m6) / (K1 * K1);
+            constexpr double th2 = T16_THETA * T16_THETA, th8 = th2 * th2 * th2 * th2;
+            ok = (n2 * (1.0 + 1e-9) <= th2) || (m6 >= 0. && m8 * (1.0 + 1e-9) <= th8);
+        }
     }
     ok = __builtin_amdgcn_readfirstlane((int)ok) != 0;
     { T16_FRESH_LANE(l3); lane = l3; }
 #pragma unroll
     for (int t = 0; t < NT; ++t) {
-        U.re[t] = Y0.re[t] + T16_C3 * A2.re[t] + T16_C4 * As.re[t];
-        U.im[t] = Y0.im[t] + T16_C3 * A2.im[t] + T16_C4 * As.im[t];
-        const d4 vr = T16_C6 * Y0.re[t] + T16_C7 * A2.re[t], vi = T16_C6 * Y0.im[t] + T16_C7 * A2.im[t];
+        U.re[t] = Y0.re[t] + K3 * A2.re[t] + K4 * As.re[t];
+        U.im[t] = Y0.im[t] + K3 * A2.im[t] + K4 * As.im[t];
+        const d4 vr = K6 * Y0.re[t] + K7 * A2.re[t], vi = K6 * Y0.im[t] + K7 * A2.im[t];
         q.p1[t] = vr; q.p2[t] = (d4){0., 0., 0., 0.}; q.p3[t] = vr + vi;
-        Y0.re[t] += T16_C5 * A2.re[t];
-        Y0.im[t] += T16_C5 * A2.im[t];
+        Y0.re[t] += K5 * A2.re[t];
+        Y0.im[t] += K5 * A2.im[t];
         Y0.sm[t] = Y0.re[t] + Y0.im[t];
     }
     t18_store_slots<LD, NT, NT>(R, U, wave, lane);
@@ -664,24 +691,24 @@
         double *x = R + (lane >> 4) * LD + 16 * wave + (lane & 15);
 #pragma unroll
         for (int t = 0; t < NT; ++t) {
-            const d4 y0r = Y0.re[t] - T16_C5 * A2.re[t], y0i = Y0.im[t] - T16_C5 * A2.im[t];
-            const d4 xr = Y1.re[t] + T16_C8 * A2.re[t] + T16_C9 * As.re[t], xi = Y1.im[t] + T16_C8 * A2.im[t] + T16_C9 * As.im[t];
+            const d4 y0r = Y0.re[t] - K5 * A2.re[t], y0i = Y0.im[t] - K5 * A2.im[t];
+            const d4 xr = Y1.re[t] + K8 * A2.re[t] + K9 * As.re[t], xi = Y1.im[t] + K8 * A2.im[t] + K9 * As.im[t];
             const int tb = (wave + t) % NT;
 #pragma unroll
             for (int r = 0; r < 4; ++r) {
                 const int o = (16 * tb + 4 * r) * LD;
                 x[o] = xr[r]; x[PL + o] = xi[r]; x[2 * PL + o] = xr[r] + xi[r];
             }
-            d4 vr = T16_C12 * Y1.re[t] + T16_C13 * y0r + T16_C14 * A2.re[t] + T16_C15 * As.re[t];
-            const d4 vi = T16_C12 * Y1.im[t] + T16_C13 * y0i + T16_C14 * A2.im[t] + T16_C15 * As.im[t];
+            d4 vr = K12 * Y1.re[t] + K13 * y0r + K14 * A2.re[t] + K15 * As.re[t];
+            const d4 vi = K12 * Y1.im[t] + K13 * y0i + K14 * A2.im[t] + K15 * As.im[t];
             if (t == 0) {
 #pragma unroll
                 for (int r = 0; r < 4; ++r)
-                    if (4 * r + rgd == cdiag) vr[r] += T16_C16;
+                    if (4 * r + rgd == cdiag) vr[r] += K16;
             }
             q.p1[t] = vr; q.p2[t] = (d4){0., 0., 0., 0.}; q.p3[t] = vr + vi;
-            Y0.re[t] = Y1.re[t] + T16_C10 * y0r + T16_C11 * As.re[t];
-            Y0.im[t] = Y1.im[t] + T16_C10 * y0i + T16_C11 * As.im[t];
+            Y0.re[t] = Y1.re[t] + K10 * y0r + K11 * As.re[t];
+            Y0.im[t] = Y1.im[t] + K10 * y0i + K11 * As.im[t];
             Y0.sm[t] = Y0.re[t] + Y0.im[t];
         }
     }
@@ -733,7 +760,7 @@
     const int end = listed ? min(__builtin_amdgcn_readfirstlane(a.flags[4]), ncell) : hi;
     const int idx0 = listed ? (int)blockIdx.x : lo + ((int)blockIdx.x >> 3);
     auto cell_at = [&](int i) -> int { return listed ? __builtin_amdgcn_readfirstlane(a.cell_list[i]) : i; };
-    int st_s = 0, st_max = 0, st_ord[5] = {0, 0, 0, 0, 0}, st_sq = 0, st_cells = 0, st_t16 = 0;
+    int st_s = 0, st_max = 0, st_ord[5] = {0, 0, 0, 0, 0}, st_sq = 0, st_cells = 0, st_t16 = 0, st_q = 0;
     bool any_bad = false;
     Strip<NT> Uprev;
     strip_zero(Uprev);
@@ -782,7 +809,13 @@
             auto fetch_next = [&](int sk, int r) { if (sk == 1 && r == 0) fa.issue(); };
             if constexpr (T16) {
                 s = 0; bad = false;
-                const bool ok16 = expm_t16_cell<NT, true>(smem, wave, lane, U, store_prev, fetch_next);
+                bool ok16;
+                if constexpr (NT == 4) {
+                    const bool q = a.splan != nullptr && (__builtin_amdgcn_readfirstlane(a.splan[cell]) & T16_PLAN_Q) != 0;
+                    if (q) { ok16 = expm_t16_cell<NT, true, true>(smem, wave, lane, U, store_prev, fetch_next); st_q += 1; }
+                    else ok16 = expm_t16_cell<NT, true>(smem, wave, lane, U, store_prev, fetch_next);
+                } else
+                    ok16 = expm_t16_cell<NT, true>(smem, wave, lane, U, store_prev, fetch_next);
                 if (tid == 0 && a.cellflag) a.cellflag[cell] = ok16 ? 0 : 1;
                 if (ok16) st_t16 += 1;
                 else if (tid == 0) a.cell_list[atomicAdd(&a.flags[4], 1)] = cell;
@@ -838,6 +871,7 @@
         if (st_max > 0) atomicMax(&a.flags[1], st_max);
         unsigned long long mi = (unsigned long long)st_cells * (T16 ? (SYM ? T16Count<NT>::CELL : T16Count<NT>::CELL_NOSYM) : SYM ? T18Count<NT>::CELL : T18Count<NT>::CELL_GENERAL)
                                 + (unsigned long long)st_sq * T18Count<NT>::GP;
+        mi -= (unsigned long long)st_q * (T18Count<NT>::GP - T18Count<NT>::SQH);
         if constexpr (T16) {
             stat_add(a.stats, 15, (unsigned long long)st_t16);
             atomicAdd(&a.flags[5], st_cells);
diff --git a/grape.jl_amd/csrc/grape_t18_coeffs.h b/grape.jl_amd/csrc/grape_t18_coeffs.h
--- a/grape.jl_amd/csrc/grape_t18_coeffs.h
+++ b/grape.jl_amd/csrc/grape_t18_coeffs.h
@@ -61,3 +61,20 @@
 #define T16_C14 0.32660098775353450156
 #define T16_C15 0.9999999999999999025
 #define T16_C16 0.99999999999999991128
+#define T16Q_THETA 1.11
+#define T16Q_C1 0.00051563001890111433182
+#define T16Q_C2 0.0
+#define T16Q_C3 0.0023030158800575477112
+#define T16Q_C4 0.57294486810438500817
+#define T16Q_C5 0.039952426348918349803
+#define T16Q_C6 9.9345037093649872503
+#define T16Q_C7 0.12383410213207938471
+#define T16Q_C8 -0.036677532080650709165
+#define T16Q_C9 -0.38874283651186037534
+#define T16Q_C10 -8.4588053279285115744
+#define T16Q_C11 0.2598977251233012689
+#define T16Q_C12 8.3944945060272534018
+#define T16Q_C13 -19.297513921073804518
+#define T16Q_C14 -0.43849131113914585078
+#define T16Q_C15 0.99999999999999703594
+#define T16Q_C16 1.0000000000000000038
```

Measured after the change: 59.06 (median of 6 runs). 5.8% higher.
